# yvette256/nerfstudio-thermal

Hardware: AMD Instinct MI355X
Metric: train rays/sec (4096-ray batch, 96 samples/ray) (higher is better)
Workload: dtype f32; 1 GPU; thermal-nerfacto density_mode=shared train step (pixel sampling+raygen+fwd+losses+bwd+allreduce+Adam), 4096 rays/GPU, 256/96 proposal + 48 field samples, hash 16x2^19x2 + 2x(5x2^17x2), 8 cameras (4 RGB + 4 thermal); rays_per_gpu=4096, parallelism=dp1, grad_scaler=device-side (optim.DeviceGradScaler)

## Files before the change

### nerfstudio-thermal_amd/csrc/tn_common.h

```cpp
#pragma once
#include <hip/hip_runtime.h>
#include <stdint.h>
#include <math.h>
#include "../../include/thermal_nerf_hip.h"

#define TN_WAVE 64

void tn_set_error(const char* fmt, ...);
#define TN_REQUIRE(cond, ...)        \
  do {                               \
    if (!(cond)) {                   \
      tn_set_error(__VA_ARGS__);     \
      return TN_EINVAL;              \
    }                                \
  } while (0)
#define TN_CHECK_LAUNCH(name)                                         \
  do {                                                                \
    hipError_t e__ = hipGetLastError();                               \
    if (e__ != hipSuccess) {                                          \
      tn_set_error("%s: %s", name, hipGetErrorString(e__));           \
      return TN_ELAUNCH;                                              \
    }                                                                 \
  } while (0)

// ... 261 lines not shown
__device__ __forceinline__ float tn_wave_max(float v) {
#pragma unroll
  for (int o = 32; o > 0; o >>= 1) v = fmaxf(v, __shfl_xor(v, o, 64));
  return v;
}
__device__ __forceinline__ double tn_wave_incl_scan_d(double v, int lane) {
#pragma unroll
  for (int o = 1; o < 64; o <<= 1) {
    double t = __shfl_up(v, o, 64);
    if (lane >= o) v += t;
  }
  return v;
}
__device__ __forceinline__ double tn_excl_from_incl_d(double incl, int lane) {
  double t = __shfl_up(incl, 1, 64);
  return lane == 0 ? 0.0 : t;
}
__device__ __forceinline__ float tn_rexcl_from_incl(float incl, int lane) {
  float t = __shfl_down(incl, 1, 64);
  return lane == 63 ? 0.0f : t;
}
__device__ __forceinline__ float tn_wave_incl_rscan(float v, int lane) {
#pragma unroll
  for (int o = 1; o < 64; o <<= 1) {
    float t = __shfl_down(v, o, 64);
    if (lane + o < 64) v += t;
  }
  return v;
}

__device__ __forceinline__ void tn_patch_order(int64_t i, int64_t N, int S, int64_t& ray, int& s) {
  int64_t per = 4 * (int64_t)S;
  int64_t g = tn_div_index(i, per, N * (int64_t)S);
  int w = (int)(i - g * per);
  int64_t r0 = g * 4;
  int nr = (N - r0) < 4 ? (int)(N - r0) : 4;
  s = nr == 4 ? (w >> 2) : w / nr;
  ray = r0 + (w - s * nr);
}

#define TN_SCATTER_SCRATCH_BYTES (64ll << 20)
#ifndef TN_BIN_SLICE_LOG2
#define TN_BIN_SLICE_LOG2 12
#endif
#define TN_BIN_MAX_SLICES 256
#define TN_BIN_COUNT_STRIDE 16
static inline int64_t tn_bin_level_records(int64_t P) { return 16 * P + TN_BIN_MAX_SLICES * 1032; }
static inline int64_t tn_bin_bytes(int64_t P, int num_levels) {
  return 256 + (int64_t)num_levels * TN_BIN_MAX_SLICES * 4 * TN_BIN_COUNT_STRIDE + (int64_t)num_levels * tn_bin_level_records(P) * (2 + 8);
}
static inline int64_t tn_scatter_scratch_bytes(int64_t P, int num_levels) {
  int64_t b = tn_bin_bytes(P, num_levels);
  return ((b > TN_SCATTER_SCRATCH_BYTES ? b : TN_SCATTER_SCRATCH_BYTES) + 255) / 256 * 256;
}
enum { TN_REP_NONE = 0, TN_REP_DENSE = 1 };
struct ReplicaK {
  float2* rep;
  uint32_t total;
  uint32_t kinds;
  uint32_t n[TN_MAX_LEVELS];
  uint32_t off[TN_MAX_LEVELS];
  uint32_t first[TN_MAX_LEVELS];
  uint8_t R[TN_MAX_LEVELS];
};
#define TN_LD_LEVEL_MAJOR (-1)
struct TnNextSamplingHost {
  const TnPropNet *prop0, *prop1;
  const float* pose; const uint8_t* frozen; int num_cameras;
  const float *rays_o, *rays_d; const int64_t* cam;
  const float *nears, *fars, *jit0, *jit1, *jit2, *lin0, *lin1, *lin2;
  float anneal;
  int S0, S1, S2;
  int64_t N;
  float* out;
  int64_t off[16];
  int save_enc;
};
int tn_adam_step_ranges_amp_update_cw(float* params, const float* grads, float* exp_avg, float* exp_avg_sq, int32_t num_ranges, const int64_t* offsets,
                                      const int64_t* counts, const int32_t* steps, const double* lrs, const double* lr_finals,
                                      const int32_t* sched_max_steps, int32_t sched_step, double beta1, double beta2, double eps, const float* inv_scale,
                                      float* found_inf, const int32_t* flag_index, int32_t num_flags, int32_t* skipped, int32_t lag_index,
                                      int32_t count_skip, int32_t zero_grads, float* scale, int32_t* growth_tracker, uint32_t* done_counter,
                                      double growth_factor, double backoff_factor, int32_t growth_interval, const TnSampleRays* next, bool* next_taken,
                                      tn_stream_t stream, const TnNextSamplingHost* chain = nullptr, bool su_update = true);
static inline bool tn_next_sampling_supported(int S0, int S1, int S2) { return S0 > 128 && S0 <= 256 && S1 > 64 && S1 <= 128 && S2 >= 1 && S2 <= 256; }
int tn_render_fwd_ex(const float* e_bins, const float* density, const float* rgb, int64_t N, int32_t S, int32_t C, int32_t training, float* weights,
                     float* comp, float* accumulation, float* depth_median, float* depth_expected, float* scratch, bool launch_clip, int* clip_nblk,
                     tn_stream_t stream);
int tn_train_losses_clip(const float* s_bins_fine, const float* weights_fine, int32_t S_fine, int32_t num_props, const float* const* s_bins_prop,
                         const float* const* weights_prop, const int32_t* S_prop, float* const* d_weights_prop, int64_t N, float distortion_mult,
                         float interlevel_mult, float* d_weights_fine, const float* pred_rgb, int32_t rgb_stride, const float* pred_thermal,
                         int32_t thermal_stride, const float* image, const float* is_thermal, float thermal_mult, float tv_mult, float cross_mult,
                         float* d_pred_rgb, float* d_pred_thermal, float* loss_lines, float* depth_expected, const float* scratch, int clip_nblk,
                         tn_stream_t stream);
struct DposArgs;
struct PoseFinishArgs;
int tn_grid_scatter_launch(const TnGrid& grid, const float* origins, const float* directions, const float* e_bins, const float* g_enc, int ld,
                           int64_t N, int S, float* d_origins, float* d_directions, void* scratch, hipStream_t stream, float* dense_sum = nullptr,
                           bool counters_zeroed = false, const DposArgs* cowork = nullptr, const PoseFinishArgs* fold_cowork = nullptr);
bool tn_grid_scatter_takes_cowork(const TnGrid& grid, int64_t P, void* scratch);
int tn_field_bwd_phase_ex(const TnField* field, const float* origins, const float* directions, const int64_t* camera_indices, const float* e_bins,
                          const float* d_density, const float* d_rgb, int64_t N, int32_t S, void* workspace, int64_t workspace_bytes, float* d_origins,
                          float* d_directions, int32_t phases, int32_t level_begin, int32_t level_end, const PoseFinishArgs* fold_cowork,
                          bool* fold_cowork_taken, tn_stream_t stream);
int tn_pose_finish_args(const float* pose_adjustment, const uint8_t* frozen, const int64_t* camera_indices, const float* directions_in,
                        const float* d_origins, const float* d_directions, int64_t N, int32_t num_cameras, float* grad_pose, const float* loss_lines,
                        float* losses16, float trans_pen, float rot_pen, float scale, float* reg_out, const float* grads, int32_t num_ranges,
                        const int64_t* offsets, const int64_t* counts, const int32_t* flag_index, int32_t num_flags, float* found_inf, int32_t pose_flag,
                        PoseFinishArgs& a);
void tn_grid_scatter_counters(const TnGrid& grid, int64_t P, void* scratch, uint32_t** ptr, int* words);
__device__ __forceinline__ void tn_zero_words(uint32_t* __restrict__ p, int words) {
  if (blockIdx.x == 0 && blockIdx.y == 0)
    for (int i = threadIdx.x; i < words; i += blockDim.x) p[i] = 0u;
}
bool tn_grid_scatter_is_binned(const TnGrid& grid, int64_t P, const void* scratch);
int tn_grid_scatter_bin(const TnGrid& grid, const float* origins, const float* directions, const float* e_bins, const float* g_enc, int ld, int64_t N,
                        int S, float* d_origins, float* d_directions, void* scratch, hipStream_t stream, bool counters_zeroed = false,
                        const DposArgs* cowork = nullptr);
int tn_grid_scatter_fold(const TnGrid& grid, int64_t P, void* scratch, int level_begin, int level_end, hipStream_t stream,
                         const PoseFinishArgs* cowork = nullptr);
int64_t tn_grid_dense_count(const TnGrid& grid, int64_t P);
int tn_grid_dense_fold(const TnGrid& grid, int64_t P, const float* dense_sum, hipStream_t stream);
```

### nerfstudio-thermal_amd/csrc/tn_field.hip

```cpp
#include "tn_common.h"
#include "tn_field_dpos.h"
#include <stdlib.h>

typedef float f32x16 __attribute__((ext_vector_type(16)));
typedef float v4f_t __attribute__((ext_vector_type(4)));
#ifndef FRAG_NT
#define FRAG_NT 1
#endif

#define TILE 32
#define FRAG 64

__host__ __device__ __forceinline__ constexpr int RROW(int r, int h) { return (r & 3) + 8 * (r >> 2) + 4 * h; }

struct LayerGeom { int mo, ti; };
__host__ __device__ __forceinline__ constexpr int layer_mo(int l) { return (l == 0 || l == 2 || l == 3) ? 2 : 1; }
__host__ __device__ __forceinline__ constexpr int layer_ti(int l) { return l == 0 ? 1 : 2; }
__host__ __device__ __forceinline__ constexpr int layer_frags(int l) { return layer_mo(l) * layer_ti(l) * 16; }
__host__ __device__ __forceinline__ constexpr int fwd_off(int l) {
  int o = 0;
  for (int i = 0; i < l; ++i) o += layer_frags(i) * FRAG;
  return o;
}
#define PACK_FWD_FLOATS (fwd_off(5))
// ... 1162 lines not shown
                    int64_t zero_bytes, tn_stream_t stream) {
  if (N == 0) return TN_OK;
  int rc = check_field(field, "tn_field_fwd", false);
  if (rc) return rc;
  TN_REQUIRE(origins && directions && camera_indices && e_bins && workspace && density && rgb, "tn_field_fwd: null pointer");
  TN_REQUIRE(N >= 0 && S >= 1 && S <= TN_MAX_SAMPLES, "tn_field_fwd: bad N=%lld S=%d", (long long)N, S);
  if (N == 0) return TN_OK;
  int64_t P = N * (int64_t)S;
  FieldWs ws = ws_layout(workspace, P, training);
  TN_REQUIRE((2 * ws.PT + P) * 8 < (1ll << 32), "tn_field_fwd: batch too large for the 32-bit lane offsets of the level-major loads");
  TN_REQUIRE(workspace_bytes >= ws.bytes, "tn_field_fwd: workspace of %lld bytes, tn_field_workspace_bytes(%lld, %d) = %lld", (long long)workspace_bytes,
             (long long)P, training, (long long)ws.bytes);
  TN_REQUIRE(zero == nullptr || (((uintptr_t)zero % 16) == 0 && zero_bytes % 16 == 0), "tn_field_fwd: the buffer to clear must be 16-byte aligned and sized");
  TN_REQUIRE(!training || field->num_images <= FIELD_MAX_IMAGES, "tn_field_fwd: %d cameras, the per-camera tables of the training path are sized for %d",
             field->num_images, FIELD_MAX_IMAGES);
  rc = launch_encode(field, origins, directions, e_bins, N, S, ws, stream, FieldPrepExtra{pack_first != 0, zero, zero_bytes});
  if (rc) return rc;
  const size_t shmem = PACK_FWD_TOTAL * sizeof(float);
  const int grid = (int)std::max<int64_t>(1, std::min<int64_t>(tn_cdiv(tn_cdiv(P, TILE), FWD_THREADS / 64), 512));
  const int L = field->grid.num_levels;
#define FWD_LAUNCH(TRAIN_, BF3_, ...)                                                                                                          \
  {                                                                                                                                            \
    (void)hipFuncSetAttribute(reinterpret_cast<const void*>(&k_field_mlp_fwd<TRAIN_, BF3_>), hipFuncAttributeMaxDynamicSharedMemorySize, (int)shmem); \
    hipLaunchKernelGGL((k_field_mlp_fwd<TRAIN_, BF3_>), dim3(grid), dim3(FWD_THREADS), shmem, tn_s(stream), ws.pack, ws.enc, L, ws.PT, ws.sel, ws.sh, \
                       camera_indices, field->emb, field->num_images, TRAIN_ ? 1 : 0, N, S, field->num_channels, density, rgb, density_pre, __VA_ARGS__); \
  }
  const bool bf3 = tn_head_bf16x3();
  if (training) {
    if (bf3) FWD_LAUNCH(true, true, ws.h1, ws.hin, ws.hh1, ws.hh2, ws.y) else FWD_LAUNCH(true, false, ws.h1, ws.hin, ws.hh1, ws.hh2, ws.y)
  } else {
    if (bf3) FWD_LAUNCH(false, true, nullptr, nullptr, nullptr, nullptr, nullptr) else FWD_LAUNCH(false, false, nullptr, nullptr, nullptr, nullptr, nullptr)
  }
#undef FWD_LAUNCH
  TN_CHECK_LAUNCH("tn_field_fwd");
  return TN_OK;
}

extern "C" int tn_field_density_fwd(const TnField* field, const float* origins, const float* directions, const float* e_bins, int64_t N, int32_t S,
                                    int32_t training, void* workspace, int64_t workspace_bytes, float* density, tn_stream_t stream) {
  if (N == 0) return TN_OK;
  int rc = check_field(field, "tn_field_density_fwd", false);
  if (rc) return rc;
  TN_REQUIRE(origins && directions && e_bins && workspace && density, "tn_field_density_fwd: null pointer");
  TN_REQUIRE(N >= 0 && S >= 1 && S <= TN_MAX_SAMPLES, "tn_field_density_fwd: bad N=%lld S=%d", (long long)N, S);
  int64_t P = N * (int64_t)S;
  FieldWs ws = ws_layout(workspace, P, training ? 1 : 0);
  TN_REQUIRE((2 * ws.PT + P) * 8 < (1ll << 32), "tn_field_density_fwd: batch too large for the 32-bit lane offsets of the level-major loads");
  TN_REQUIRE(workspace_bytes >= ws.bytes, "tn_field_density_fwd: workspace of %lld bytes, tn_field_workspace_bytes(%lld, %d) = %lld", (long long)workspace_bytes,
             (long long)P, training ? 1 : 0, (long long)ws.bytes);
  rc = launch_encode(field, origins, directions, e_bins, N, S, ws, stream);
  if (rc) return rc;
  size_t shmem = PACK_FWD_TOTAL * sizeof(float);
  if (training) {
    (void)hipFuncSetAttribute(reinterpret_cast<const void*>(&k_field_density_only<true>), hipFuncAttributeMaxDynamicSharedMemorySize, (int)shmem);
    hipLaunchKernelGGL(k_field_density_only<true>, dim3(mlp_grid(P)), dim3(256), shmem, tn_s(stream), ws.pack, ws.enc, field->grid.num_levels, ws.PT, ws.sel, P, density, ws.h1, ws.hin);
  } else {
    (void)hipFuncSetAttribute(reinterpret_cast<const void*>(&k_field_density_only<false>), hipFuncAttributeMaxDynamicSharedMemorySize, (int)shmem);
    hipLaunchKernelGGL(k_field_density_only<false>, dim3(mlp_grid(P)), dim3(256), shmem, tn_s(stream), ws.pack, ws.enc, field->grid.num_levels, ws.PT, ws.sel, P, density, nullptr, nullptr);
  }
  TN_CHECK_LAUNCH("tn_field_density_fwd");
  return TN_OK;
}

static TnGrid level_range_grid(const TnGrid& g, int level_begin, int level_end) {
  TnGrid sub = g;
  const int64_t T2 = 2ll << g.log2_hashmap_size;
  sub.table = g.table + level_begin * T2;
  sub.table_grad = g.table_grad ? g.table_grad + level_begin * T2 : nullptr;
  sub.num_levels = level_end - level_begin;
  for (int i = 0; i < TN_MAX_LEVELS; ++i) sub.res[i] = (level_begin + i < g.num_levels) ? g.res[level_begin + i] : 0.0f;
  return sub;
}

extern "C" int tn_field_bwd_phase(const TnField* field, const float* origins, const float* directions, const int64_t* camera_indices,
                                  const float* e_bins, const float* d_density, const float* d_rgb, int64_t N, int32_t S, void* workspace,
                                  int64_t workspace_bytes, float* d_origins, float* d_directions, int32_t phases, int32_t level_begin, int32_t level_end,
                                  tn_stream_t stream) {
  return tn_field_bwd_phase_ex(field, origins, directions, camera_indices, e_bins, d_density, d_rgb, N, S, workspace, workspace_bytes, d_origins, d_directions,
                               phases, level_begin, level_end, nullptr, nullptr, stream);
}
int tn_field_bwd_phase_ex(const TnField* field, const float* origins, const float* directions, const int64_t* camera_indices, const float* e_bins,
                          const float* d_density, const float* d_rgb, int64_t N, int32_t S, void* workspace, int64_t workspace_bytes, float* d_origins,
                          float* d_directions, int32_t phases, int32_t level_begin, int32_t level_end, const PoseFinishArgs* fold_cowork,
                          bool* fold_cowork_taken, tn_stream_t stream) {
  if (fold_cowork_taken) *fold_cowork_taken = false;
  if (N == 0) return TN_OK;
  int rc = check_field(field, "tn_field_bwd", true);
  if (rc) return rc;
  TN_REQUIRE(origins && directions && camera_indices && e_bins && d_density && workspace, "tn_field_bwd: null pointer");
  const bool dens_only = d_rgb == nullptr;
  TN_REQUIRE((d_origins == nullptr) == (d_directions == nullptr), "tn_field_bwd: d_origins and d_directions must both be given or both NULL");
  TN_REQUIRE(N >= 0 && S >= 1 && S <= TN_MAX_SAMPLES, "tn_field_bwd: bad N=%lld S=%d", (long long)N, S);
  TN_REQUIRE((phases & ~(TN_BWD_MLP | TN_BWD_SCATTER | TN_BWD_JOIN | TN_BWD_SCATTER_BIN | TN_BWD_SCATTER_FOLD | TN_BWD_FORK_DPOS | TN_BWD_COUNTERS_CLEAN)) == 0 && phases != 0,
             "tn_field_bwd: bad phase set %d", phases);
  TN_REQUIRE(!((phases & TN_BWD_SCATTER) && (phases & (TN_BWD_SCATTER_BIN | TN_BWD_SCATTER_FOLD))), "tn_field_bwd: TN_BWD_SCATTER and its two halves exclude each other");
  if (phases & (TN_BWD_SCATTER | TN_BWD_SCATTER_FOLD))
    TN_REQUIRE(level_begin >= 0 && level_begin < level_end && level_end <= field->grid.num_levels, "tn_field_bwd: bad level range [%d, %d)", level_begin,
               level_end);
  int64_t P = N * (int64_t)S;
  FieldWs ws = ws_layout(workspace, P, 1);
  TN_REQUIRE(workspace_bytes >= ws.bytes, "tn_field_bwd: workspace of %lld bytes, tn_field_workspace_bytes(%lld, 1) = %lld", (long long)workspace_bytes, (long long)P,
             (long long)ws.bytes);
  TN_REQUIRE((2 * ws.PT + P) * 8 < (1ll << 32), "tn_field_bwd: batch too large for the 32-bit lane offsets of the level-major loads");
  hipStream_t st = tn_s(stream);
  const int C = field->num_channels;
  TN_REQUIRE(dens_only || !(phases & TN_BWD_MLP) || field->num_images <= FIELD_MAX_IMAGES,
             "tn_field_bwd: %d cameras, the per-camera sums of the appearance embedding's gradient are sized for %d", field->num_images, FIELD_MAX_IMAGES);
  DposArgs dpos_args{};
  bool dpos_cowork = false;
  if (phases & TN_BWD_MLP) {
    const size_t shmem = FB_LDS_FLOATS * sizeof(float);
    const int grid = (int)std::max<int64_t>(1, std::min<int64_t>(tn_cdiv(tn_cdiv(P, TILE), 4), 256));
    FusedGrads G{field->gw0, field->gb0, field->gw1, field->gb1, field->ghw0, field->ghb0, field->ghw1, field->ghb1, field->ghw2, field->ghb2, field->gemb};
    uint32_t* zp;
    int zw;
    tn_grid_scatter_counters(field->grid, P, ws.scatter, &zp, &zw);
    if (dens_only) {
      (void)hipFuncSetAttribute(reinterpret_cast<const void*>(&k_field_bwd_fused<true, false>), hipFuncAttributeMaxDynamicSharedMemorySize, (int)shmem);
      hipLaunchKernelGGL((k_field_bwd_fused<true, false>), dim3(grid), dim3(256), shmem, st, ws.pack, ws.sel, ws.y, d_rgb, d_density, camera_indices, field->num_images, P, S,
                         C, ws.sh, field->emb, ws.cam_bias, field->grid.num_levels, ws.PT, ws.enc, ws.h1, ws.hin, ws.hh1, ws.hh2, ws.g_enc, G, zp, zw);
    } else if (tn_head_bf16x3()) {
      (void)hipFuncSetAttribute(reinterpret_cast<const void*>(&k_field_bwd_fused<false, true>), hipFuncAttributeMaxDynamicSharedMemorySize, (int)shmem);
      hipLaunchKernelGGL((k_field_bwd_fused<false, true>), dim3(grid), dim3(256), shmem, st, ws.pack, ws.sel, ws.y, d_rgb, d_density, camera_indices, field->num_images, P,
                         S, C, ws.sh, field->emb, ws.cam_bias, field->grid.num_levels, ws.PT, ws.enc, ws.h1, ws.hin, ws.hh1, ws.hh2, ws.g_enc, G, zp, zw);
    } else {
      (void)hipFuncSetAttribute(reinterpret_cast<const void*>(&k_field_bwd_fused<false, false>), hipFuncAttributeMaxDynamicSharedMemorySize, (int)shmem);
      hipLaunchKernelGGL((k_field_bwd_fused<false, false>), dim3(grid), dim3(256), shmem, st, ws.pack, ws.sel, ws.y, d_rgb, d_density, camera_indices, field->num_images, P,
                         S, C, ws.sh, field->emb, ws.cam_bias, field->grid.num_levels, ws.PT, ws.enc, ws.h1, ws.hin, ws.hh1, ws.hh2, ws.g_enc, G, zp, zw);
    }
    if (!dens_only && d_origins == nullptr)
      hipLaunchKernelGGL(k_field_emb_finish, dim3(std::min(field->num_images + 8, 1024)), dim3(256), 0, st, ws.cam_bias,
                         reinterpret_cast<uint32_t*>(ws.cam_bias + (int64_t)FIELD_MAX_IMAGES * 64), field->hw0, field->emb, field->gemb, field->ghw0,
                         field->num_images);
    TN_CHECK_LAUNCH("tn_field_bwd(mlp + weight gradients)");
    if (d_origins != nullptr) {
      dpos_args = DposArgs{origins, directions, e_bins, ws.g_enc, ws.jac, N, S, field->grid.num_levels, ws.PT, d_origins, d_directions,
                           dens_only ? nullptr : ws.cam_bias, reinterpret_cast<uint32_t*>(ws.cam_bias + (int64_t)FIELD_MAX_IMAGES * 64), field->hw0, field->emb,
                           field->gemb, field->ghw0, field->num_images};
      const char* cwe = getenv("TN_DPOS_COWORK");
      dpos_cowork = (phases & TN_BWD_SCATTER) && level_begin == 0 && level_end == field->grid.num_levels && !(cwe && cwe[0] == '0') &&
                    tn_grid_scatter_takes_cowork(field->grid, P, ws.scatter);
      if (!dpos_cowork) {
        hipStream_t side = (phases & TN_BWD_FORK_DPOS) ? tn_fork(st) : nullptr;
        const int64_t tiles = tn_cdiv(P, 32);
        hipLaunchKernelGGL(k_field_dpos, dim3((unsigned)std::min<int64_t>(tn_cdiv(tiles, 4), 256 * 8)), dim3(256), 0, side ? side : st, dpos_args);
      }
      TN_CHECK_LAUNCH("tn_field_bwd(d position)");
    }
  }
  float* sc_do = nullptr;
  float* sc_dd = nullptr;
  if (phases & TN_BWD_SCATTER) {
    TnGrid sub = level_range_grid(field->grid, level_begin, level_end);
    const bool cz = (phases & (TN_BWD_MLP | TN_BWD_COUNTERS_CLEAN)) && level_begin == 0 && level_end == field->grid.num_levels;
    const PoseFinishArgs* fcw = (fold_cowork != nullptr && dpos_cowork) ? fold_cowork : nullptr;
    rc = tn_grid_scatter_launch(sub, origins, directions, e_bins, ws.g_enc + (int64_t)level_begin * 2 * P, TN_LD_LEVEL_MAJOR, N, S, sc_do, sc_dd, ws.scatter, st,
                                nullptr, cz, dpos_cowork ? &dpos_args : nullptr, fcw);
    if (fold_cowork_taken && rc == TN_OK) *fold_cowork_taken = fcw != nullptr;
  }
  if (phases & (TN_BWD_SCATTER_BIN | TN_BWD_SCATTER_FOLD)) {
    TN_REQUIRE(tn_grid_scatter_is_binned(field->grid, P, ws.scatter), "tn_field_bwd: the two-step scatter needs a record-based path (TN_SCATTER_MODE=2 or 1 -- not 0 --, a scatter workspace, table <= 2^20 slots)");
    if (phases & TN_BWD_SCATTER_BIN)
      rc = tn_grid_scatter_bin(field->grid, origins, directions, e_bins, ws.g_enc, TN_LD_LEVEL_MAJOR, N, S, sc_do, sc_dd, ws.scatter, st,
                               (phases & (TN_BWD_MLP | TN_BWD_COUNTERS_CLEAN)) != 0);
    if (rc == TN_OK && (phases & TN_BWD_SCATTER_FOLD)) rc = tn_grid_scatter_fold(field->grid, P, ws.scatter, level_begin, level_end, st);
  }
  if (phases & TN_BWD_JOIN) tn_join_all(st);
  return rc;
}

extern "C" int tn_field_bwd(const TnField* field, const float* origins, const float* directions, const int64_t* camera_indices, const float* e_bins,
                            const float* d_density, const float* d_rgb, int64_t N, int32_t S, void* workspace, int64_t workspace_bytes, float* d_origins,
                            float* d_directions, tn_stream_t stream) {
  if (field == nullptr) return check_field(field, "tn_field_bwd", true);
  return tn_field_bwd_phase(field, origins, directions, camera_indices, e_bins, d_density, d_rgb, N, S, workspace, workspace_bytes, d_origins, d_directions,
                            TN_BWD_MLP | TN_BWD_SCATTER | TN_BWD_JOIN, 0, field->grid.num_levels, stream);
}

extern "C" int64_t tn_field_dense_count(const TnField* field, int64_t num_points, int32_t level_begin, int32_t level_end) {
  if (field == nullptr || level_begin < 0 || level_begin >= level_end || level_end > field->grid.num_levels) return 0;
  return tn_grid_dense_count(level_range_grid(field->grid, level_begin, level_end), num_points);
}

extern "C" int tn_field_bwd_scatter_dense(const TnField* field, const float* origins, const float* directions, const float* e_bins, int64_t N, int32_t S,
                                          void* workspace, int64_t workspace_bytes, float* d_origins, float* d_directions, int32_t level_begin,
                                          int32_t level_end, float* dense_sum, tn_stream_t stream) {
  if (N == 0) return TN_OK;
  int rc = check_field(field, "tn_field_bwd_scatter_dense", true);
  if (rc) return rc;
  TN_REQUIRE(origins && directions && e_bins && workspace && dense_sum, "tn_field_bwd_scatter_dense: null pointer");
  TN_REQUIRE((d_origins == nullptr) == (d_directions == nullptr), "tn_field_bwd_scatter_dense: d_origins and d_directions must both be given or both NULL");
  TN_REQUIRE(N > 0 && S >= 1 && S <= TN_MAX_SAMPLES, "tn_field_bwd_scatter_dense: bad N=%lld S=%d", (long long)N, S);
  TN_REQUIRE(level_begin >= 0 && level_begin < level_end && level_end <= field->grid.num_levels, "tn_field_bwd_scatter_dense: bad level range [%d, %d)",
             level_begin, level_end);
  FieldWs ws = ws_layout(workspace, N * (int64_t)S, 1);
  TN_REQUIRE(workspace_bytes >= ws.bytes, "tn_field_bwd_scatter_dense: workspace of %lld bytes, needs %lld", (long long)workspace_bytes, (long long)ws.bytes);
  return tn_grid_scatter_launch(level_range_grid(field->grid, level_begin, level_end), origins, directions, e_bins,
                                ws.g_enc + (int64_t)level_begin * 2 * N * S, TN_LD_LEVEL_MAJOR, N, S, nullptr, nullptr, ws.scatter, tn_s(stream), dense_sum);
}

extern "C" int tn_field_dense_fold(const TnField* field, int64_t num_points, int32_t level_begin, int32_t level_end, const float* dense_sum,
                                   tn_stream_t stream) {
  int rc = check_field(field, "tn_field_dense_fold", true);
  if (rc) return rc;
  TN_REQUIRE(level_begin >= 0 && level_begin < level_end && level_end <= field->grid.num_levels && num_points > 0, "tn_field_dense_fold: bad arguments");
  return tn_grid_dense_fold(level_range_grid(field->grid, level_begin, level_end), num_points, dense_sum, tn_s(stream));
}
```

### nerfstudio-thermal_amd/csrc/tn_misc.hip

```cpp
#include "tn_common.h"
#include "tn_pose_finish.h"
#include <algorithm>
#include "tn_pixel_loss.h"
#include <stdlib.h>
#include <stdarg.h>
#include <stdio.h>
#include <string.h>

static thread_local char g_err[512] = "";
void tn_set_error(const char* fmt, ...) {
  va_list ap;
  va_start(ap, fmt);
  vsnprintf(g_err, sizeof(g_err), fmt, ap);
  va_end(ap);
}
extern "C" const char* tn_last_error(void) { return g_err; }
#include <map>
#include <mutex>
namespace {
struct Companion {
  hipStream_t side = nullptr;
  hipEvent_t fork_ev = nullptr, join_ev = nullptr;
  bool forked = false;
};
// ... 738 lines not shown
    r.bc2_sqrt[n] = (float)sqrt(bc2);
    max_n4 = std::max<int64_t>(max_n4, counts[k] / 4);
    ++n;
  }
  if (n == 0) return TN_OK;
  int grid = (int)std::max<int64_t>(1, std::min<int64_t>(tn_cdiv(max_n4, 256), 256 * 16));
  hipLaunchKernelGGL(k_adam_ranges, dim3(grid, n), dim3(256), 0, tn_s(stream), params, grads, exp_avg, exp_avg_sq, r, (float)beta1, (float)beta2,
                     (float)(1.0 - beta1), (float)(1.0 - beta2), (float)eps);
  TN_CHECK_LAUNCH("tn_adam_step_ranges");
  return TN_OK;
}

__global__ void __launch_bounds__(256) k_grad_nonfinite(const float4* __restrict__ g, int64_t n4, const float* __restrict__ gt, int tail,
                                                         float* __restrict__ found_inf) {
  typedef float v4f __attribute__((ext_vector_type(4)));
  bool bad = false;
  for (int64_t i = blockIdx.x * (int64_t)blockDim.x + threadIdx.x; i < n4; i += (int64_t)gridDim.x * blockDim.x) {
    const v4f v = reinterpret_cast<const v4f*>(g)[i];
    const float t = (v.x - v.x) + (v.y - v.y) + (v.z - v.z) + (v.w - v.w);
    bad = bad || (t != 0.0f);
  }
  if (blockIdx.x == 0 && (int)threadIdx.x < tail) { const float x = gt[threadIdx.x]; bad = bad || ((x - x) != 0.0f); }
  if (__any(bad) && (threadIdx.x & 63) == 0) *found_inf = 1.0f;
}
extern "C" int tn_grad_nonfinite(const float* grads, int64_t count, float* found_inf, tn_stream_t stream) {
  if (count == 0) return TN_OK;
  TN_REQUIRE(grads && found_inf && count > 0, "tn_grad_nonfinite: bad argument");
  TN_REQUIRE(((uintptr_t)grads % 16) == 0, "tn_grad_nonfinite: grads must be 16-byte aligned");
  const int64_t n4 = count / 4;
  const int grid = (int)std::max<int64_t>(1, std::min<int64_t>(tn_cdiv(n4, 256 * 4), 256 * 8));
  hipLaunchKernelGGL(k_grad_nonfinite, dim3(grid), dim3(256), 0, tn_s(stream), reinterpret_cast<const float4*>(grads), n4, grads + n4 * 4, (int)(count - n4 * 4),
                     found_inf);
  TN_CHECK_LAUNCH("tn_grad_nonfinite");
  return TN_OK;
}
struct NonfiniteRanges { int64_t off[TN_ADAM_MAX_RANGES], cnt[TN_ADAM_MAX_RANGES]; int32_t flag[TN_ADAM_MAX_RANGES]; };
__global__ void __launch_bounds__(256) k_grad_nonfinite_ranges(const float* __restrict__ g, NonfiniteRanges r, float* __restrict__ found_inf) {
  typedef float v4f __attribute__((ext_vector_type(4)));
  const int k = blockIdx.y;
  const int64_t n = r.cnt[k], n4 = n / 4;
  if ((int64_t)blockIdx.x * blockDim.x >= n4 && blockIdx.x != 0) return;
  const float* base = g + r.off[k];
  bool bad = false;
  for (int64_t i = blockIdx.x * (int64_t)blockDim.x + threadIdx.x; i < n4; i += (int64_t)gridDim.x * blockDim.x) {
    const v4f v = reinterpret_cast<const v4f*>(base)[i];
    const float t = (v.x - v.x) + (v.y - v.y) + (v.z - v.z) + (v.w - v.w);
    bad = bad || (t != 0.0f);
  }
  if (blockIdx.x == 0 && (int64_t)threadIdx.x < n - n4 * 4) { const float x = base[n4 * 4 + threadIdx.x]; bad = bad || ((x - x) != 0.0f); }
  if (__any(bad) && (threadIdx.x & 63) == 0) found_inf[r.flag[k]] = 1.0f;
}
extern "C" int tn_grad_nonfinite_ranges(const float* grads, int32_t num_ranges, const int64_t* offsets, const int64_t* counts, const int32_t* flag_index,
                                        int32_t num_flags, float* found_inf, tn_stream_t stream) {
  if (num_ranges == 0) return TN_OK;
  TN_REQUIRE(grads && offsets && counts && found_inf && num_ranges > 0 && num_ranges <= TN_ADAM_MAX_RANGES && num_flags >= 1,
             "tn_grad_nonfinite_ranges: bad argument");
  TN_REQUIRE(((uintptr_t)grads % 16) == 0, "tn_grad_nonfinite_ranges: grads must be 16-byte aligned");
  NonfiniteRanges r{};
  int64_t max_n4 = 0;
  int n = 0;
  for (int k = 0; k < num_ranges; ++k) {
    const int fl = flag_index ? flag_index[k] : 0;
    TN_REQUIRE(offsets[k] >= 0 && offsets[k] % 4 == 0 && counts[k] >= 0 && fl >= 0 && fl < num_flags, "tn_grad_nonfinite_ranges: bad range %d", k);
    if (counts[k] == 0) continue;
    r.off[n] = offsets[k]; r.cnt[n] = counts[k]; r.flag[n] = fl;
    max_n4 = std::max<int64_t>(max_n4, counts[k] / 4);
    ++n;
  }
  if (n == 0) return TN_OK;
  const int grid = (int)std::max<int64_t>(1, std::min<int64_t>(tn_cdiv(max_n4, 256 * 4), 256 * 8));
  hipLaunchKernelGGL(k_grad_nonfinite_ranges, dim3(grid, n), dim3(256), 0, tn_s(stream), grads, r, found_inf);
  TN_CHECK_LAUNCH("tn_grad_nonfinite_ranges");
  return TN_OK;
}

struct AdamRangesAmp {
  int64_t off[TN_ADAM_MAX_RANGES], cnt[TN_ADAM_MAX_RANGES];
  int32_t step[TN_ADAM_MAX_RANGES], flag[TN_ADAM_MAX_RANGES];
  double lr[TN_ADAM_MAX_RANGES];
  double lr_final[TN_ADAM_MAX_RANGES];
  int32_t max_steps[TN_ADAM_MAX_RANGES];
  int32_t sched_step;
  int32_t num_flags, lag_index;
};
struct ScalerUpdate {
  float* scale;
  int32_t* growth_tracker;
  uint32_t* done;
  float growth_factor, backoff_factor;
  int32_t growth_interval;
};
__device__ __forceinline__ void scaler_update_body(float* scale, int32_t* growth_tracker, float* found_inf, int num_flags, int32_t* lag, float growth_factor,
                                                   float backoff_factor, int growth_interval, int clear) {
  bool any = false;
  for (int i = 0; i < num_flags; ++i) {
    any = any || (found_inf[i] != 0.0f);
    if (clear) found_inf[i] = 0.0f;
  }
  if (any) {
    *scale = *scale * backoff_factor;
    *growth_tracker = 0;
    if (lag != nullptr) *lag += 1;
  } else {
    const int successful = *growth_tracker + 1;
    if (successful == growth_interval) {
      const float ns = *scale * growth_factor;
      if ((ns - ns) == 0.0f) *scale = ns;
      *growth_tracker = 0;
    } else {
      *growth_tracker = successful;
    }
  }
}
#define TN_DONE_WORDS (65 * 16)
__device__ __forceinline__ void adam_block_done(const ScalerUpdate& su, float* found_inf, int num_flags, int32_t* skipped, int lag_index) {
  if (su.scale == nullptr) return;
  __syncthreads();
  if (threadIdx.x == 0) {
    const uint32_t total = gridDim.x * gridDim.y, lb = blockIdx.y * gridDim.x + blockIdx.x, line = lb & 63u;
    const uint32_t expect = total / 64u + ((line < (total & 63u)) ? 1u : 0u);
    if (__hip_atomic_fetch_add(su.done + line * 16u, 1u, __ATOMIC_RELAXED, __HIP_MEMORY_SCOPE_AGENT) + 1u == expect) {
      __hip_atomic_store(su.done + line * 16u, 0u, __ATOMIC_RELAXED, __HIP_MEMORY_SCOPE_AGENT);
      const uint32_t lines = total < 64u ? total : 64u;
      if (__hip_atomic_fetch_add(su.done + 64u * 16u, 1u, __ATOMIC_RELAXED, __HIP_MEMORY_SCOPE_AGENT) + 1u == lines) {
        __hip_atomic_store(su.done + 64u * 16u, 0u, __ATOMIC_RELAXED, __HIP_MEMORY_SCOPE_AGENT);
        scaler_update_body(su.scale, su.growth_tracker, found_inf, num_flags, (skipped != nullptr && lag_index >= 0) ? skipped + lag_index : nullptr,
                           su.growth_factor, su.backoff_factor, su.growth_interval, 1);
      }
    }
  }
}
struct SampleCoWork { SamplePixelsArgs a; RaygenArgs g; int blocks; };
#include "tn_next_sampling.h"
__device__ __forceinline__ void adam_range_body(float* __restrict__ p, const float* __restrict__ g, float* __restrict__ m, float* __restrict__ v,
                                                const AdamRangesAmp& r, double beta1, double beta2, float eps, const float* __restrict__ inv_scale,
                                                float* __restrict__ found_inf, int32_t* __restrict__ skipped, int count_skip, int zero_g, int k, int bid,
                                                int nblk) {
  const int fl = r.flag[k];
  float* gz = const_cast<float*>(g);
  const int lag = (skipped != nullptr && r.lag_index >= 0) ? skipped[r.lag_index] : 0;
  const int64_t off = r.off[k], n = r.cnt[k], n4 = n / 4;
  const int64_t stride = (int64_t)nblk * blockDim.x;
  if (found_inf != nullptr && found_inf[fl] != 0.0f) {
    if (count_skip && skipped != nullptr && bid == 0 && threadIdx.x == 0) {
      bool first = true;
      for (int j = 0; j < k; ++j) first = first && r.flag[j] != fl;
      if (first) atomicAdd(&skipped[fl], 1);
    }
    if (zero_g) {
      for (int64_t i = bid * (int64_t)blockDim.x + threadIdx.x; i < n4; i += stride)
        reinterpret_cast<float4*>(gz + off)[i] = make_float4(0.f, 0.f, 0.f, 0.f);
      if (bid == 0 && (int64_t)threadIdx.x < n - n4 * 4) gz[off + n4 * 4 + threadIdx.x] = 0.0f;
    }
    return;
  }
  if ((int64_t)bid * blockDim.x >= n4 && bid != 0) return;
  __shared__ float s_ns, s_bc;
  __syncthreads();
  if (threadIdx.x == 0) {
    const int sk = skipped ? skipped[fl] : 0;
    const int eff = r.step[k] - sk;
    const double bc1 = 1.0 - pow(beta1, (double)(eff < 1 ? 1 : eff)), bc2 = 1.0 - pow(beta2, (double)(eff < 1 ? 1 : eff));
    double lr = r.lr[k];
    if (r.max_steps[k] > 0) {
      double t = (double)(r.sched_step - lag) / (double)r.max_steps[k];
      t = t < 0.0 ? 0.0 : (t > 1.0 ? 1.0 : t);
      lr = exp(log(r.lr[k]) * (1.0 - t) + log(r.lr_final[k]) * t);
    }
    s_ns = (float)(-(lr / bc1));
    s_bc = (float)sqrt(bc2);
  }
  __syncthreads();
  const float neg_step = s_ns, bc2_sqrt = s_bc, b1 = (float)beta1, b2 = (float)beta2, omb1 = (float)(1.0 - beta1), omb2 = (float)(1.0 - beta2);
  const float is = inv_scale ? *inv_scale : 1.0f;
  float4* p4 = reinterpret_cast<float4*>(p + off);
  const float4* g4 = reinterpret_cast<const float4*>(g + off);
  float4* m4 = reinterpret_cast<float4*>(m + off);
  float4* v4 = reinterpret_cast<float4*>(v + off);
#define ADAM1(P, G, M, V)                         \
  {                                               \
    float g_ = inv_scale ? (G) * is : (G);        \
    float m_new_ = M * b1 + g_ * omb1;            \
    float v_new_ = V * b2 + (omb2 * g_) * g_;     \
    float den_ = sqrtf(v_new_) / bc2_sqrt + eps;  \
    P = P + neg_step * (m_new_ / den_);           \
    M = m_new_;                                   \
    V = v_new_;                                   \
  }
  typedef float v4f __attribute__((ext_vector_type(4)));
  typedef uint32_t v4u __attribute__((ext_vector_type(4)));
#define ADAM4(I, GG, MM, VV)                                                                                           \
  {                                                                                                                    \
    const v4u zb = __builtin_bit_cast(v4u, GG) | __builtin_bit_cast(v4u, MM) | __builtin_bit_cast(v4u, VV);          \
    if ((zb.x | zb.y | zb.z | zb.w) != 0u) {                                                                           \
      float4 pp = p4[I];                                                                                               \
      ADAM1(pp.x, GG.x, MM.x, VV.x)                                                                                    \
      ADAM1(pp.y, GG.y, MM.y, VV.y)                                                                                    \
      ADAM1(pp.z, GG.z, MM.z, VV.z)                                                                                    \
      ADAM1(pp.w, GG.w, MM.w, VV.w)                                                                                    \
      p4[I] = pp;                                                                                                      \
      __builtin_nontemporal_store(MM, reinterpret_cast<v4f*>(m4) + (I));                                               \
      __builtin_nontemporal_store(VV, reinterpret_cast<v4f*>(v4) + (I));                                               \
      if (zero_g) { const v4f z = {0.f, 0.f, 0.f, 0.f}; __builtin_nontemporal_store(z, reinterpret_cast<v4f*>(gz + off) + (I)); } \
    }                                                                                                                  \
  }
  int64_t i0 = bid * (int64_t)blockDim.x + threadIdx.x;
  for (; i0 < n4; i0 += stride) {
    v4f gg = __builtin_nontemporal_load(reinterpret_cast<const v4f*>(g4) + i0);
    v4f mm4 = __builtin_nontemporal_load(reinterpret_cast<const v4f*>(m4) + i0);
    v4f vv4 = __builtin_nontemporal_load(reinterpret_cast<const v4f*>(v4) + i0);
    ADAM4(i0, gg, mm4, vv4)
  }
#undef ADAM4
  const int tail = (int)(n - n4 * 4);
  if (bid == 0 && (int)threadIdx.x < tail) {
    const int64_t i = off + n4 * 4 + threadIdx.x;
    float pp = p[i], gg = g[i], mm = m[i], vv = v[i];
    ADAM1(pp, gg, mm, vv)
    p[i] = pp; m[i] = mm; v[i] = vv;
    if (zero_g) gz[i] = 0.0f;
  }
#undef ADAM1
}
__global__ void k_adam_ranges_amp(float* __restrict__ p, const float* __restrict__ g, float* __restrict__ m, float* __restrict__ v, AdamRangesAmp r,
                                  double beta1, double beta2, float eps, const float* __restrict__ inv_scale, float* __restrict__ found_inf,
                                  int32_t* __restrict__ skipped, int count_skip, int zero_g, ScalerUpdate su, SampleCoWork cw) {
  int k = blockIdx.y;
  if (cw.blocks > 0) {
    if (k == 0) {
      if (blockIdx.x < (unsigned)cw.blocks) sample_rays_body(cw.a, cw.g, blockIdx.x, (unsigned)cw.blocks);
      adam_block_done(su, found_inf, r.num_flags, skipped, r.lag_index);
      return;
    }
    --k;
  }
  adam_range_body(p, g, m, v, r, beta1, beta2, eps, inv_scale, found_inf, skipped, count_skip, zero_g, k, (int)blockIdx.x, (int)gridDim.x);
  adam_block_done(su, found_inf, r.num_flags, skipped, r.lag_index);
}
template <bool FUSED>
__global__ void __launch_bounds__(256, 4) k_adam_ranges_amp_next(float* __restrict__ p, const float* __restrict__ g, float* __restrict__ m, float* __restrict__ v,
                                                                 AdamRangesAmp r, double beta1, double beta2, float eps, const float* __restrict__ inv_scale,
                                                                 float* __restrict__ found_inf, int32_t* __restrict__ skipped, int count_skip, int zero_g,
                                                                 ScalerUpdate su, NextSamplingArgs ns, FusedAdam fa) {
  __shared__ __attribute__((aligned(16))) float ns_lds[NS_LDS_FLOATS];
  __shared__ __attribute__((aligned(16))) float fa_stage[FUSED ? 4 * FA_STAGE_FLOATS : 4];
  __shared__ float fa_scal[4];
  if (blockIdx.y == 0) {
    if (blockIdx.x < (unsigned)ns.blocks) next_sampling_body<FUSED>(ns, blockIdx.x, (unsigned)ns.blocks, ns_lds, &fa, fa_stage, fa_scal);
  } else {
    adam_range_body(p, g, m, v, r, beta1, beta2, eps, inv_scale, found_inf, skipped, count_skip, zero_g, (int)blockIdx.y - 1, (int)blockIdx.x, (int)gridDim.x);
  }
  adam_block_done(su, found_inf, r.num_flags, skipped, r.lag_index);
}
__global__ void __launch_bounds__(256, 4) k_next_sampling(NextSamplingArgs ns) {
  __shared__ __attribute__((aligned(16))) float ns_lds[NS_LDS_FLOATS];
  next_sampling_body(ns, blockIdx.x, gridDim.x, ns_lds);
}
static int adam_ranges_amp_impl(float* params, const float* grads, float* exp_avg, float* exp_avg_sq, int32_t num_ranges, const int64_t* offsets,
                               const int64_t* counts, const int32_t* steps, const double* lrs, const double* lr_finals,
                               const int32_t* sched_max_steps, int32_t sched_step, double beta1, double beta2, double eps,
                               const float* inv_scale, const float* found_inf, const int32_t* flag_index, int32_t num_flags, int32_t* skipped,
                               int32_t lag_index, int32_t count_skip, int32_t zero_grads, ScalerUpdate su, tn_stream_t stream,
                               const TnSampleRays* next = nullptr, bool* next_taken = nullptr, const TnNextSamplingHost* chain = nullptr) {
  if (next_taken) *next_taken = false;
  if (num_ranges == 0) return TN_OK;
  TN_REQUIRE(params && grads && exp_avg && exp_avg_sq && offsets && counts && steps && lrs, "tn_adam_step_ranges_amp: null pointer");
  TN_REQUIRE(num_ranges > 0 && num_ranges <= TN_ADAM_MAX_RANGES, "tn_adam_step_ranges_amp: %d ranges (at most %d)", num_ranges, TN_ADAM_MAX_RANGES);
  TN_REQUIRE(((uintptr_t)params % 16 == 0) && ((uintptr_t)grads % 16 == 0) && ((uintptr_t)exp_avg % 16 == 0) && ((uintptr_t)exp_avg_sq % 16 == 0),
             "tn_adam_step_ranges_amp: arena pointers must be 16-byte aligned");
  TN_REQUIRE(num_flags >= 1 && num_flags <= 64 && lag_index >= -1 && lag_index <= 64, "tn_adam_step_ranges_amp: bad num_flags / lag_index");
  AdamRangesAmp r{};
  int64_t max_n4 = 0;
  int n = 0;
  for (int k = 0; k < num_ranges; ++k) {
    TN_REQUIRE(offsets[k] >= 0 && offsets[k] % 4 == 0 && counts[k] >= 0 && steps[k] >= 1, "tn_adam_step_ranges_amp: bad range %d (offset %lld count %lld step %d)",
               k, (long long)offsets[k], (long long)counts[k], steps[k]);
    const int fl = flag_index ? flag_index[k] : 0;
    TN_REQUIRE(fl >= 0 && fl < num_flags, "tn_adam_step_ranges_amp: flag index %d of range %d outside [0, %d)", fl, k, num_flags);
    if (counts[k] == 0) continue;
    r.off[n] = offsets[k]; r.cnt[n] = counts[k]; r.step[n] = steps[k]; r.lr[n] = lrs[k]; r.flag[n] = fl;
    r.lr_final[n] = lr_finals ? lr_finals[k] : lrs[k];
    r.max_steps[n] = (lr_finals && sched_max_steps) ? sched_max_steps[k] : 0;
    max_n4 = std::max<int64_t>(max_n4, counts[k] / 4);
    ++n;
  }
  if (n == 0) return TN_OK;
  r.sched_step = sched_step;
  r.num_flags = num_flags;
  r.lag_index = lag_index;
  int grid = (int)std::max<int64_t>(1, std::min<int64_t>(tn_cdiv(max_n4, 256), 256 * 16));
  SampleCoWork cw{};
  if (next != nullptr && next->num_rays > 0) {
    int rc = sample_rays_build("tn_train_step(next_sample)", next, cw.a, cw.g);
    if (rc) return rc;
    grid = std::max(grid, (int)std::min<int64_t>(tn_cdiv(next->num_rays * 4, 256), 256));
    cw.blocks = (int)std::min<int64_t>(tn_cdiv(next->num_rays * 4, 256), grid);
    if (next_taken) *next_taken = true;
  }
  if (chain != nullptr) {
    TN_REQUIRE(next == nullptr, "tn_train_step(next_sampling): the launch that carries the chain does not sample the batch");
    TN_REQUIRE(chain->N > 0 && chain->N % 4 == 0 && chain->N < (1ll << 30), "tn_train_step(next_sampling): %lld rays (a multiple of 4 is needed)", (long long)chain->N);
    TN_REQUIRE(tn_next_sampling_supported(chain->S0, chain->S1, chain->S2), "tn_train_step(next_sampling): unsupported sample counts (%d, %d, %d)", chain->S0,
               chain->S1, chain->S2);
    TN_REQUIRE(chain->prop0 && chain->prop1 && chain->pose && chain->nears && chain->fars && chain->lin0 && chain->lin1 && chain->lin2 && chain->out &&
                   chain->rays_o && chain->rays_d && chain->cam && chain->num_cameras >= 1,
               "tn_train_step(next_sampling): null pointer");
    TN_REQUIRE(chain->prop0->grid.num_levels == PL && chain->prop1->grid.num_levels == PL && chain->prop0->grid.log2_hashmap_size >= 1 &&
                   chain->prop0->grid.log2_hashmap_size <= 24 && chain->prop1->grid.log2_hashmap_size >= 1 && chain->prop1->grid.log2_hashmap_size <= 24,
               "tn_train_step(next_sampling): proposal grids are built for %d levels", PL);
    NextSamplingArgs ns{};
    auto prop = [](const TnPropNet* q) {
      NsProp o{};
      o.table = reinterpret_cast<const float2*>(q->grid.table);
      o.tsize = 1u << q->grid.log2_hashmap_size; o.mask = o.tsize - 1u;
      for (int l = 0; l < PL; ++l) o.res[l] = q->grid.res[l];
      o.w0 = q->w0; o.b0 = q->b0; o.w1 = q->w1; o.b1 = q->b1;
      return o;
    };
    TN_REQUIRE(chain->prop0->grid.table && chain->prop0->w0 && chain->prop0->b0 && chain->prop0->w1 && chain->prop0->b1 && chain->prop1->grid.table &&
                   chain->prop1->w0 && chain->prop1->b0 && chain->prop1->w1 && chain->prop1->b1, "tn_train_step(next_sampling): null parameter pointer");
    ns.p0 = prop(chain->prop0); ns.p1 = prop(chain->prop1);
    ns.pose = chain->pose; ns.frozen = chain->frozen; ns.num_cameras = chain->num_cameras;
    ns.rays_o = chain->rays_o; ns.rays_d = chain->rays_d; ns.cam = chain->cam;
    ns.nears = chain->nears; ns.fars = chain->fars;
    ns.jit0 = chain->jit0; ns.jit1 = chain->jit1; ns.jit2 = chain->jit2;
    ns.lin0 = chain->lin0; ns.lin1 = chain->lin1; ns.lin2 = chain->lin2;
    ns.anneal = chain->anneal;
    ns.S0 = chain->S0; ns.S1 = chain->S1; ns.S2 = chain->S2; ns.N = (int)chain->N;
    ns.out = chain->out;
    for (int k = 0; k < NS_SLOTS; ++k) {
      TN_REQUIRE(chain->off[k] >= 0 && chain->off[k] < (1ll << 32), "tn_train_step(next_sampling): forward buffer region %d out of range", k);
      ns.off[k] = (uint32_t)chain->off[k];
    }
    ns.save_enc = chain->save_enc;
    grid = std::max(grid, (int)std::min<int64_t>(chain->N / 4, 1024));
    ns.blocks = (int)std::min<int64_t>(chain->N / 4, grid);
    const char* mode = getenv("TN_NEXT_SAMPLING");
    if (mode && mode[0] == '3') {
      hipStream_t side = tn_fork_n(tn_s(stream), 3);
      hipLaunchKernelGGL(k_next_sampling, dim3(ns.blocks), dim3(256), 0, side ? side : tn_s(stream), ns);
      TN_CHECK_LAUNCH("tn_next_sampling");
      SampleCoWork none{};
      hipLaunchKernelGGL(k_adam_ranges_amp, dim3(grid, n), dim3(256), 0, tn_s(stream), params, grads, exp_avg, exp_avg_sq, r, beta1, beta2, (float)eps, inv_scale,
                         const_cast<float*>(found_inf), skipped, (int)count_skip, (int)zero_grads, su, none);
      TN_CHECK_LAUNCH("tn_adam_step_ranges_amp");
      return TN_OK;
    }
    if (mode && mode[0] == '2') {
      SampleCoWork none{};
      hipLaunchKernelGGL(k_adam_ranges_amp, dim3(grid, n), dim3(256), 0, tn_s(stream), params, grads, exp_avg, exp_avg_sq, r, beta1, beta2, (float)eps, inv_scale,
                         const_cast<float*>(found_inf), skipped, (int)count_skip, (int)zero_grads, su, none);
      TN_CHECK_LAUNCH("tn_adam_step_ranges_amp");
      hipLaunchKernelGGL(k_next_sampling, dim3(ns.blocks), dim3(256), 0, tn_s(stream), ns);
      TN_CHECK_LAUNCH("tn_next_sampling");
      return TN_OK;
    }
    FusedAdam fa{};
    if (mode && mode[0] == '4' && n == 1 && inv_scale == nullptr) {
      const int64_t nb = r.cnt[0] / 256, W = (int64_t)ns.blocks * 4, trips = tn_cdiv(chain->N, W);
      const char* fs = getenv("TN_FUSED_SITES");
      const int64_t per_ray = fs ? std::max(1, atoi(fs)) : FA_SITES_PER_RAY;
      const int64_t take = std::min<int64_t>(nb - 1, per_ray * trips * W);
      if (take >= W) {
        fa.p = params + r.off[0]; fa.g = grads + r.off[0]; fa.m = exp_avg + r.off[0]; fa.v = exp_avg_sq + r.off[0];
        fa.batches = (uint32_t)take;
        fa.flag = r.flag[0]; fa.step = r.step[0]; fa.max_steps = r.max_steps[0]; fa.sched_step = r.sched_step; fa.lag_index = r.lag_index;
        fa.zero_g = (int)zero_grads;
        fa.beta1 = beta1; fa.beta2 = beta2; fa.lr = r.lr[0]; fa.lr_final = r.lr_final[0]; fa.eps = (float)eps;
        fa.found_inf = found_inf; fa.skipped = skipped;
        r.off[0] += take * 256; r.cnt[0] -= take * 256;
      }
    }
    if (fa.batches > 0)
      hipLaunchKernelGGL(k_adam_ranges_amp_next<true>, dim3(grid, n + 1), dim3(256), 0, tn_s(stream), params, grads, exp_avg, exp_avg_sq, r, beta1, beta2, (float)eps,
                         inv_scale, const_cast<float*>(found_inf), skipped, (int)count_skip, (int)zero_grads, su, ns, fa);
    else
      hipLaunchKernelGGL(k_adam_ranges_amp_next<false>, dim3(grid, n + 1), dim3(256), 0, tn_s(stream), params, grads, exp_avg, exp_avg_sq, r, beta1, beta2, (float)eps,
                         inv_scale, const_cast<float*>(found_inf), skipped, (int)count_skip, (int)zero_grads, su, ns, fa);
    TN_CHECK_LAUNCH("tn_adam_step_ranges_amp(next_sampling)");
    return TN_OK;
  }
  hipLaunchKernelGGL(k_adam_ranges_amp, dim3(grid, n + (cw.blocks > 0 ? 1 : 0)), dim3(256), 0, tn_s(stream), params, grads, exp_avg, exp_avg_sq, r, beta1, beta2,
                     (float)eps, inv_scale, const_cast<float*>(found_inf), skipped, (int)count_skip, (int)zero_grads, su, cw);
  TN_CHECK_LAUNCH("tn_adam_step_ranges_amp");
  return TN_OK;
}
extern "C" int tn_adam_step_ranges_amp(float* params, const float* grads, float* exp_avg, float* exp_avg_sq, int32_t num_ranges, const int64_t* offsets,
                                       const int64_t* counts, const int32_t* steps, const double* lrs, const double* lr_finals,
                                       const int32_t* sched_max_steps, int32_t sched_step, double beta1, double beta2, double eps,
                                       const float* inv_scale, const float* found_inf, const int32_t* flag_index, int32_t num_flags, int32_t* skipped,
                                       int32_t lag_index, int32_t count_skip, int32_t zero_grads, tn_stream_t stream) {
  return adam_ranges_amp_impl(params, grads, exp_avg, exp_avg_sq, num_ranges, offsets, counts, steps, lrs, lr_finals, sched_max_steps, sched_step, beta1, beta2,
                              eps, inv_scale, found_inf, flag_index, num_flags, skipped, lag_index, count_skip, zero_grads, ScalerUpdate{}, stream);
}
extern "C" int tn_adam_step_ranges_amp_update(float* params, const float* grads, float* exp_avg, float* exp_avg_sq, int32_t num_ranges, const int64_t* offsets,
                                              const int64_t* counts, const int32_t* steps, const double* lrs, const double* lr_finals,
                                              const int32_t* sched_max_steps, int32_t sched_step, double beta1, double beta2, double eps,
                                              const float* inv_scale, float* found_inf, const int32_t* flag_index, int32_t num_flags, int32_t* skipped,
                                              int32_t lag_index, int32_t count_skip, int32_t zero_grads, float* scale, int32_t* growth_tracker,
                                              uint32_t* done_counter, double growth_factor, double backoff_factor, int32_t growth_interval,
                                              tn_stream_t stream) {
  TN_REQUIRE(found_inf && scale && growth_tracker && done_counter && growth_interval >= 1, "tn_adam_step_ranges_amp_update: bad scaler arguments");
  TN_REQUIRE(num_ranges > 0, "tn_adam_step_ranges_amp_update: the fused scale update needs at least one range (use tn_grad_scaler_update otherwise)");
  ScalerUpdate su{scale, growth_tracker, done_counter, (float)growth_factor, (float)backoff_factor, (int32_t)growth_interval};
  return adam_ranges_amp_impl(params, grads, exp_avg, exp_avg_sq, num_ranges, offsets, counts, steps, lrs, lr_finals, sched_max_steps, sched_step, beta1, beta2,
                              eps, inv_scale, found_inf, flag_index, num_flags, skipped, lag_index, count_skip, zero_grads, su, stream);
}

int tn_adam_step_ranges_amp_update_cw(float* params, const float* grads, float* exp_avg, float* exp_avg_sq, int32_t num_ranges, const int64_t* offsets,
                                      const int64_t* counts, const int32_t* steps, const double* lrs, const double* lr_finals,
                                      const int32_t* sched_max_steps, int32_t sched_step, double beta1, double beta2, double eps, const float* inv_scale,
                                      float* found_inf, const int32_t* flag_index, int32_t num_flags, int32_t* skipped, int32_t lag_index,
                                      int32_t count_skip, int32_t zero_grads, float* scale, int32_t* growth_tracker, uint32_t* done_counter,
                                      double growth_factor, double backoff_factor, int32_t growth_interval, const TnSampleRays* next, bool* next_taken,
                                      tn_stream_t stream, const TnNextSamplingHost* chain, bool su_update) {
  TN_REQUIRE(found_inf && scale && growth_tracker && done_counter && growth_interval >= 1, "tn_adam_step_ranges_amp_update: bad scaler arguments");
  TN_REQUIRE(num_ranges > 0, "tn_adam_step_ranges_amp_update: the fused scale update needs at least one range (use tn_grad_scaler_update otherwise)");
  ScalerUpdate su{scale, growth_tracker, done_counter, (float)growth_factor, (float)backoff_factor, (int32_t)growth_interval};
  return adam_ranges_amp_impl(params, grads, exp_avg, exp_avg_sq, num_ranges, offsets, counts, steps, lrs, lr_finals, sched_max_steps, sched_step, beta1, beta2,
                              eps, inv_scale, found_inf, flag_index, num_flags, skipped, lag_index, count_skip, zero_grads, su_update ? su : ScalerUpdate{}, stream,
                              next, next_taken, chain);
}

__global__ void k_grad_scaler_update(float* scale, int32_t* growth_tracker, float* found_inf, int num_flags, int32_t* lag, float growth_factor,
                                     float backoff_factor, int growth_interval, int clear) {
  scaler_update_body(scale, growth_tracker, found_inf, num_flags, lag, growth_factor, backoff_factor, growth_interval, clear);
}
extern "C" int tn_grad_scaler_update(float* scale, int32_t* growth_tracker, float* found_inf, int32_t num_flags, int32_t* lag,
                                     double growth_factor, double backoff_factor, int32_t growth_interval, int32_t clear_found_inf, tn_stream_t stream) {
  TN_REQUIRE(scale && growth_tracker && found_inf && num_flags >= 1 && growth_interval >= 1, "tn_grad_scaler_update: bad argument");
  hipLaunchKernelGGL(k_grad_scaler_update, dim3(1), dim3(1), 0, tn_s(stream), scale, growth_tracker, found_inf, (int)num_flags, lag, (float)growth_factor,
                     (float)backoff_factor, (int)growth_interval, (int)clear_found_inf);
  TN_CHECK_LAUNCH("tn_grad_scaler_update");
  return TN_OK;
}
```

### nerfstudio-thermal_amd/csrc/tn_pipeline.hip

```cpp
#include "tn_common.h"
#include "tn_pose_finish.h"

namespace {
struct EvalWs {
  float *s0, *e0, *d0, *w0, *s1, *e1, *d1, *w1, *s2, *e2, *w2, *rgb_s, *scratch;
  void* field_ws;
  int64_t bytes;
};
EvalWs eval_layout(void* base, int64_t N, int S0, int S1, int S2, int C) {
  EvalWs w;
  char* p = reinterpret_cast<char*>(base);
  int64_t off = 0;
  auto take = [&](int64_t floats) {
    float* r = reinterpret_cast<float*>(p + off);
    off += ((floats * 4 + 255) / 256) * 256;
    return r;
  };
  w.s0 = take(N * (S0 + 1)); w.e0 = take(N * (S0 + 1)); w.d0 = take(N * S0); w.w0 = take(N * S0);
  w.s1 = take(N * (S1 + 1)); w.e1 = take(N * (S1 + 1)); w.d1 = take(N * S1); w.w1 = take(N * S1);
  w.s2 = take(N * (S2 + 1)); w.e2 = take(N * (S2 + 1)); w.w2 = take(N * S2);
  w.rgb_s = take(N * (int64_t)S2 * C);
  w.scratch = take(TN_RENDER_SCRATCH_FLOATS);
  w.field_ws = p + off;
  off += tn_field_workspace_bytes(N * (int64_t)S2, 0);
  w.bytes = off;
  return w;
}
}

extern "C" int64_t tn_render_rays_eval_workspace_bytes(int64_t num_rays, int32_t S0, int32_t S1, int32_t S2, int32_t C) {
  if (num_rays < 0 || S0 < 1 || S1 < 1 || S2 < 1 || S0 > TN_MAX_SAMPLES || S1 > TN_MAX_SAMPLES || S2 > TN_MAX_SAMPLES || C < 1 || C > 4) return TN_EINVAL;
  return eval_layout(nullptr, num_rays, S0, S1, S2, C).bytes;
}

extern "C" int tn_render_rays_eval(const TnPropNet* prop0, const TnPropNet* prop1, const TnField* field, const float* origins,
                                   const float* directions, const int64_t* camera_indices, const float* nears, const float* fars, int64_t N,
                                   int32_t S0, int32_t S1, int32_t S2, float anneal, const float* lin_spaced0, const float* lin_pdf1,
                                   const float* lin_pdf2, void* workspace, int64_t workspace_bytes, float* rgb, float* accumulation, float* depth_median,
                                   float* depth_expected, float* prop_depth0, float* prop_depth1, float* density, float* e_bins_out,
                                   float* rgb_samples_out, tn_stream_t stream) {
  if (N == 0) return TN_OK;
  TN_REQUIRE(prop0 && prop1 && field && origins && directions && camera_indices && nears && fars && lin_spaced0 && lin_pdf1 && lin_pdf2 &&
                 workspace && rgb && density,
             "tn_render_rays_eval: null pointer");
  TN_REQUIRE(N > 0 && S0 >= 1 && S1 >= 1 && S2 >= 1 && S0 <= TN_MAX_SAMPLES && S1 <= TN_MAX_SAMPLES && S2 <= TN_MAX_SAMPLES,
             "tn_render_rays_eval: bad N=%lld S=(%d, %d, %d)", (long long)N, S0, S1, S2);
  TN_REQUIRE(((uintptr_t)workspace % 256) == 0, "tn_render_rays_eval: workspace must be 256-byte aligned");
  const int C = field->num_channels;
  EvalWs w = eval_layout(workspace, N, S0, S1, S2, C);
  TN_REQUIRE(workspace_bytes >= w.bytes, "tn_render_rays_eval: workspace of %lld bytes, tn_render_rays_eval_workspace_bytes = %lld", (long long)workspace_bytes,
             (long long)w.bytes);
  const int64_t field_ws_bytes = tn_field_workspace_bytes(N * (int64_t)S2, 0);
  float* e2 = e_bins_out ? e_bins_out : w.e2;
  float* rgb_s = rgb_samples_out ? rgb_samples_out : w.rgb_s;
  int rc;
  if ((rc = tn_spaced_bins(lin_spaced0, nullptr, nears, fars, N, S0, w.s0, w.e0, stream))) return rc;
  if ((rc = tn_prop_density_fwd(prop0, origins, directions, w.e0, N, S0, w.d0, stream))) return rc;
  if ((rc = tn_weights_resample(w.e0, w.d0, w.s0, S0, anneal, lin_pdf1, nullptr, nears, fars, N, S1, w.w0, prop_depth0, w.s1, w.e1, stream))) return rc;
  if ((rc = tn_prop_density_fwd(prop1, origins, directions, w.e1, N, S1, w.d1, stream))) return rc;
  if ((rc = tn_weights_resample(w.e1, w.d1, w.s1, S1, anneal, lin_pdf2, nullptr, nears, fars, N, S2, w.w1, prop_depth1, w.s2, e2, stream))) return rc;
  if ((rc = tn_field_fwd_ex(field, origins, directions, camera_indices, e2, N, S2, 0, w.field_ws, field_ws_bytes, density, rgb_s, nullptr, 1, nullptr, 0, stream)))
    return rc;
  return tn_render_fwd(e2, density, rgb_s, N, S2, C, 0, w.w2, rgb, accumulation, depth_median, depth_expected, w.scratch, stream);
}

enum {
  TRO_ORIGINS = 0, TRO_DIRECTIONS,
  TRO_S0, TRO_E0, TRO_D0, TRO_W0, TRO_M0,
  TRO_S1, TRO_E1, TRO_D1, TRO_W1, TRO_M1,
  TRO_S2, TRO_E2, TRO_D2, TRO_W2,
  TRO_RGB_SAMPLES, TRO_COMP, TRO_ACC, TRO_DEPTH, TRO_EXPECTED, TRO_SCRATCH,
  TRO_PENC0, TRO_PENC1,
  TRO_END,
  TRO_COUNT
};
static void train_layout(int64_t N, int S0, int S1, int S2, int C, int64_t* off) {
  int64_t o = 0;
  auto take = [&](int slot, int64_t floats) { off[slot] = o; o += (floats + 63) / 64 * 64; };
  take(TRO_ORIGINS, N * 3); take(TRO_DIRECTIONS, N * 3);
  take(TRO_S0, N * (S0 + 1)); take(TRO_E0, N * (S0 + 1)); take(TRO_D0, N * S0); take(TRO_W0, N * S0); take(TRO_M0, N);
  take(TRO_S1, N * (S1 + 1)); take(TRO_E1, N * (S1 + 1)); take(TRO_D1, N * S1); take(TRO_W1, N * S1); take(TRO_M1, N);
  take(TRO_S2, N * (S2 + 1)); take(TRO_E2, N * (S2 + 1)); take(TRO_D2, N * S2); take(TRO_W2, N * S2);
  take(TRO_RGB_SAMPLES, N * (int64_t)S2 * C); take(TRO_COMP, N * C); take(TRO_ACC, N); take(TRO_DEPTH, N); take(TRO_EXPECTED, N);
  take(TRO_SCRATCH, TN_RENDER_SCRATCH_FLOATS);
// ... 10 lines not shown
}

static int render_rays_train_impl(const TnPropNet* prop0, const TnPropNet* prop1, const TnField* field, const float* pose_adjustment,
                                  const uint8_t* frozen, int32_t num_cameras, const float* origins_in, const float* directions_in,
                                  const int64_t* camera_indices, const float* nears, const float* fars, int64_t N, int32_t S0, int32_t S1,
                                  int32_t S2, float anneal, const float* jitter0, const float* jitter1, const float* jitter2,
                                  const float* lin_spaced0, const float* lin_pdf1, const float* lin_pdf2, void* field_workspace,
                                  int64_t field_workspace_bytes, float* out, void* wait_event_before_field, void* zero_fill, int64_t zero_fill_bytes,
                                  int32_t save_prop_enc, int with_render, int* clip_nblk, tn_stream_t stream, bool sampling_done = false) {
  if (clip_nblk) *clip_nblk = 0;
  if (N == 0) return TN_OK;
  TN_REQUIRE(prop0 && prop1 && field && origins_in && directions_in && camera_indices && nears && fars && lin_spaced0 && lin_pdf1 && lin_pdf2 &&
                 field_workspace && out,
             "tn_render_rays_train: null pointer");
  TN_REQUIRE(N > 0 && S0 >= 1 && S1 >= 1 && S2 >= 1 && S0 <= TN_MAX_SAMPLES && S1 <= TN_MAX_SAMPLES && S2 <= TN_MAX_SAMPLES,
             "tn_render_rays_train: bad N=%lld S=(%d, %d, %d)", (long long)N, S0, S1, S2);
  TN_REQUIRE(((uintptr_t)out % 256) == 0, "tn_render_rays_train: the output buffer must be 256-byte aligned");
  const int C = field->num_channels;
  int64_t off[TRO_COUNT];
  train_layout(N, S0, S1, S2, C, off);
  auto at = [&](int slot) { return out + off[slot]; };
  const float* o = origins_in;
  const float* d = directions_in;
  int rc;
  if (sampling_done) {
    if (pose_adjustment != nullptr) { o = at(TRO_ORIGINS); d = at(TRO_DIRECTIONS); }
  } else {
    if (pose_adjustment != nullptr) {
      TN_REQUIRE(num_cameras >= 1, "tn_render_rays_train: bad num_cameras=%d", num_cameras);
      if ((rc = tn_pose_spaced_bins(pose_adjustment, frozen, camera_indices, origins_in, directions_in, N, num_cameras, at(TRO_ORIGINS), at(TRO_DIRECTIONS),
                                    lin_spaced0, jitter0, nears, fars, S0, at(TRO_S0), at(TRO_E0), stream)))
        return rc;
      o = at(TRO_ORIGINS);
      d = at(TRO_DIRECTIONS);
    } else if ((rc = tn_spaced_bins(lin_spaced0, jitter0, nears, fars, N, S0, at(TRO_S0), at(TRO_E0), stream))) {
      return rc;
    }
    if ((rc = tn_prop_density_fwd_ex(prop0, o, d, at(TRO_E0), N, S0, at(TRO_D0), save_prop_enc ? at(TRO_PENC0) : nullptr, stream))) return rc;
    if ((rc = tn_weights_resample(at(TRO_E0), at(TRO_D0), at(TRO_S0), S0, anneal, lin_pdf1, jitter1, nears, fars, N, S1, at(TRO_W0), at(TRO_M0), at(TRO_S1),
                                  at(TRO_E1), stream)))
      return rc;
    if ((rc = tn_prop_density_fwd_ex(prop1, o, d, at(TRO_E1), N, S1, at(TRO_D1), save_prop_enc ? at(TRO_PENC1) : nullptr, stream))) return rc;
    if ((rc = tn_weights_resample(at(TRO_E1), at(TRO_D1), at(TRO_S1), S1, anneal, lin_pdf2, jitter2, nears, fars, N, S2, at(TRO_W1), at(TRO_M1), at(TRO_S2),
                                  at(TRO_E2), stream)))
      return rc;
  }
  if (wait_event_before_field != nullptr) {
    hipError_t e = hipStreamWaitEvent(tn_s(stream), reinterpret_cast<hipEvent_t>(wait_event_before_field), 0);
    TN_REQUIRE(e == hipSuccess, "tn_render_rays_train: hipStreamWaitEvent failed: %s", hipGetErrorString(e));
  }
  if ((rc = tn_field_fwd_ex(field, o, d, camera_indices, at(TRO_E2), N, S2, 1, field_workspace, field_workspace_bytes, at(TRO_D2), at(TRO_RGB_SAMPLES), nullptr, 1,
                            zero_fill, zero_fill_bytes, stream)))
    return rc;
  if (!with_render) return TN_OK;
  return tn_render_fwd_ex(at(TRO_E2), at(TRO_D2), at(TRO_RGB_SAMPLES), N, S2, C, 1, at(TRO_W2), at(TRO_COMP), at(TRO_ACC), at(TRO_DEPTH), at(TRO_EXPECTED),
                          at(TRO_SCRATCH), with_render == 1, clip_nblk, stream);
}
extern "C" int tn_render_rays_train(const TnPropNet* prop0, const TnPropNet* prop1, const TnField* field, const float* pose_adjustment,
                                    const uint8_t* frozen, int32_t num_cameras, const float* origins_in, const float* directions_in,
                                    const int64_t* camera_indices, const float* nears, const float* fars, int64_t N, int32_t S0, int32_t S1,
                                    int32_t S2, float anneal, const float* jitter0, const float* jitter1, const float* jitter2,
                                    const float* lin_spaced0, const float* lin_pdf1, const float* lin_pdf2, void* field_workspace,
                                    int64_t field_workspace_bytes, float* out, void* wait_event_before_field, void* zero_fill, int64_t zero_fill_bytes,
                                    int32_t save_prop_enc, tn_stream_t stream) {
  return render_rays_train_impl(prop0, prop1, field, pose_adjustment, frozen, num_cameras, origins_in, directions_in, camera_indices, nears, fars, N, S0, S1, S2,
                                anneal, jitter0, jitter1, jitter2, lin_spaced0, lin_pdf1, lin_pdf2, field_workspace, field_workspace_bytes, out,
                                wait_event_before_field, zero_fill, zero_fill_bytes, save_prop_enc, 1, nullptr, stream);
}

__global__ void k_add_inplace(float* __restrict__ a, const float* __restrict__ b, int64_t n) {
  for (int64_t i = blockIdx.x * (int64_t)blockDim.x + threadIdx.x; i < n; i += (int64_t)gridDim.x * blockDim.x) a[i] += b[i];
}
extern "C" int64_t tn_render_rays_train_bwd_tmp_floats(int64_t N, int32_t S0, int32_t S1, int32_t S2, int32_t C) {
  if (N < 0 || S0 < 1 || S1 < 1 || S2 < 1 || C < 1 || C > 4) return TN_EINVAL;
  auto up = [](int64_t x) { return (x + 63) / 64 * 64; };
  return up(N * (int64_t)S2 * C) + up(N * (int64_t)S2) + up(N * (int64_t)S0) + up(N * (int64_t)S1);
}
static int render_rays_train_bwd_impl(const TnPropNet* prop0, const TnPropNet* prop1, const TnField* field, const float* origins,
                                      const float* directions, const int64_t* camera_indices, int64_t N, int32_t S0, int32_t S1, int32_t S2,
                                      const float* fwd_out, const float* d_comp, const float* d_weights0,
                                      const float* d_weights1, const float* d_weights2, const float* d_density_extra, void* field_workspace,
                                      int64_t field_workspace_bytes, void* prop_workspace0, int64_t prop_workspace_bytes0, void* prop_workspace1,
                                      int64_t prop_workspace_bytes1, float* tmp, float* d_origins, float* d_directions, int32_t prop_enc_saved,
                                      bool render_bwd_done, const PoseFinishArgs* fold_cowork, bool* fold_cowork_taken, tn_stream_t stream) {
  if (fold_cowork_taken) *fold_cowork_taken = false;
  if (N == 0) return TN_OK;
  TN_REQUIRE(field && origins && directions && camera_indices && fwd_out && d_comp && d_weights2 && field_workspace && tmp,
             "tn_render_rays_train_bwd: null pointer");
  TN_REQUIRE((d_weights0 == nullptr) == (d_weights1 == nullptr), "tn_render_rays_train_bwd: d_weights0 and d_weights1 come together (or not at all)");
  const bool prop_grad = d_weights0 != nullptr;
  if (prop_grad) TN_REQUIRE(prop0 && prop1 && prop_workspace0 && prop_workspace1, "tn_render_rays_train_bwd: proposal networks / workspaces missing");
  TN_REQUIRE(N > 0 && S0 >= 1 && S1 >= 1 && S2 >= 1 && S0 <= TN_MAX_SAMPLES && S1 <= TN_MAX_SAMPLES && S2 <= TN_MAX_SAMPLES,
             "tn_render_rays_train_bwd: bad N=%lld S=(%d, %d, %d)", (long long)N, S0, S1, S2);
  TN_REQUIRE((d_origins == nullptr) == (d_directions == nullptr), "tn_render_rays_train_bwd: d_origins and d_directions must both be given or both NULL");
  const int C = field->num_channels;
  int64_t off[TRO_COUNT];
  train_layout(N, S0, S1, S2, C, off);
  auto at = [&](int slot) { return fwd_out + off[slot]; };
  auto up = [](int64_t x) { return (x + 63) / 64 * 64; };
  float* d_rgb = tmp;
  float* d_dens = d_rgb + up(N * (int64_t)S2 * C);
  float* dd0 = d_dens + up(N * (int64_t)S2);
  float* dd1 = dd0 + up(N * (int64_t)S0);
  const float* o = origins;
  const float* d = directions;
  hipStream_t st = tn_s(stream);
  int rc;
  if (!render_bwd_done && (rc = tn_render_bwd(at(TRO_E2), at(TRO_D2), at(TRO_RGB_SAMPLES), at(TRO_W2), d_comp, d_weights2, N, S2, C, d_rgb, d_dens, stream)))
    return rc;
  if (d_density_extra != nullptr) {
    const int64_t n = N * (int64_t)S2;
    hipLaunchKernelGGL(k_add_inplace, dim3((unsigned)std::min<int64_t>(tn_cdiv(n, 256), 4096)), dim3(256), 0, st, d_dens, d_density_extra, n);
    TN_CHECK_LAUNCH("tn_render_rays_train_bwd(add)");
  }
  int rc0 = TN_OK, rc1 = TN_OK;
  if (prop_grad) {
    hipStream_t s0 = tn_fork_n(st, 1), s1 = tn_fork_n(st, 2);
    tn_stream_t t0 = s0 ? (tn_stream_t)s0 : stream, t1 = s1 ? (tn_stream_t)s1 : stream;
    rc0 = tn_weights_bwd(at(TRO_E0), at(TRO_D0), at(TRO_W0), d_weights0, N, S0, dd0, t0);
    if (!rc0)
      rc0 = tn_prop_density_bwd_ex(prop0, o, d, at(TRO_E0), dd0, N, S0, prop_workspace0, prop_workspace_bytes0, d_origins, d_directions,
                                   prop_enc_saved ? at(TRO_PENC0) : nullptr, t0);
    rc1 = tn_weights_bwd(at(TRO_E1), at(TRO_D1), at(TRO_W1), d_weights1, N, S1, dd1, t1);
    if (!rc1)
      rc1 = tn_prop_density_bwd_ex(prop1, o, d, at(TRO_E1), dd1, N, S1, prop_workspace1, prop_workspace_bytes1, d_origins, d_directions,
                                   prop_enc_saved ? at(TRO_PENC1) : nullptr, t1);
  }
  rc = tn_field_bwd_phase_ex(field, o, d, camera_indices, at(TRO_E2), d_dens, d_rgb, N, S2, field_workspace, field_workspace_bytes, d_origins, d_directions,
                             TN_BWD_MLP | TN_BWD_SCATTER | TN_BWD_JOIN | (prop_grad ? TN_BWD_FORK_DPOS : 0), 0, field->grid.num_levels,
                             prop_grad ? nullptr : fold_cowork, fold_cowork_taken, stream);
  if (prop_grad) { tn_join_n(st, 1); tn_join_n(st, 2); }
  return rc ? rc : (rc0 ? rc0 : rc1);
}
extern "C" int tn_render_rays_train_bwd(const TnPropNet* prop0, const TnPropNet* prop1, const TnField* field, const float* origins,
                                        const float* directions, const int64_t* camera_indices, int64_t N, int32_t S0, int32_t S1, int32_t S2,
                                        const float* fwd_out, const float* d_comp, const float* d_weights0,
                                        const float* d_weights1, const float* d_weights2, const float* d_density_extra, void* field_workspace,
                                        int64_t field_workspace_bytes, void* prop_workspace0, int64_t prop_workspace_bytes0, void* prop_workspace1,
                                        int64_t prop_workspace_bytes1, float* tmp, float* d_origins, float* d_directions, int32_t prop_enc_saved,
                                        tn_stream_t stream) {
  return render_rays_train_bwd_impl(prop0, prop1, field, origins, directions, camera_indices, N, S0, S1, S2, fwd_out, d_comp, d_weights0, d_weights1, d_weights2,
                                    d_density_extra, field_workspace, field_workspace_bytes, prop_workspace0, prop_workspace_bytes0, prop_workspace1,
                                    prop_workspace_bytes1, tmp, d_origins, d_directions, prop_enc_saved, false, nullptr, nullptr, stream);
}


extern "C" int tn_train_step(const TnTrainStep* a, tn_stream_t stream) {
  TN_REQUIRE(a != nullptr, "tn_train_step: null argument block");
  tn_join_n(tn_s(stream), 3);
  if (a->next_sample_taken) *a->next_sample_taken = 0;
  if (a->N == 0) return TN_OK;
  TN_REQUIRE(a->prop0 && a->prop1 && a->field && a->origins_in && a->directions_in && a->camera_indices && a->image && a->is_thermal && a->nears &&
                 a->fars && a->fwd_out && a->bwd_tmp && a->acc && a->losses16 && a->loss_lines && a->d_comp && a->d_weights2,
             "tn_train_step: null pointer");
  TN_REQUIRE(a->pose_adjustment && a->grad_pose && a->d_origins && a->d_directions && a->num_cameras >= 1,
             "tn_train_step: this entry point is the iteration WITH a camera optimiser (pose_adjustment, grad_pose, d_origins, d_directions)");
  TN_REQUIRE(a->prop_grad == 0 || (a->d_weights0 && a->d_weights1 && a->prop_workspace0 && a->prop_workspace1),
             "tn_train_step: prop_grad needs d_weights0 / d_weights1 and both proposal workspaces");
  TN_REQUIRE(a->num_check >= 0 && a->num_check <= TN_TRAIN_STEP_MAX_RANGES && a->num_ranges >= 0 && a->num_ranges <= TN_TRAIN_STEP_MAX_RANGES,
             "tn_train_step: at most %d ranges", TN_TRAIN_STEP_MAX_RANGES);
  TN_REQUIRE(a->found_inf && a->num_flags >= 1 && a->scale && a->growth_tracker && a->done_counter && a->skipped,
             "tn_train_step: the GradScaler state is part of the iteration (found_inf, scale, growth_tracker, done_counter, skipped)");
  TN_REQUIRE(a->num_ranges == 0 || (a->params && a->grads && a->exp_avg && a->exp_avg_sq), "tn_train_step: null arena pointer");
  const int C = a->field->num_channels;
  TN_REQUIRE(C == 4, "tn_train_step: the shared-density model renders RGB + thermal from one field (4 channels), got %d", C);
  TN_REQUIRE(a->N > 0 && a->S0 >= 1 && a->S1 >= 1 && a->S2 >= 1 && a->S0 <= TN_MAX_SAMPLES && a->S1 <= TN_MAX_SAMPLES && a->S2 <= TN_MAX_SAMPLES,
             "tn_train_step: bad N=%lld S=(%d, %d, %d)", (long long)a->N, a->S0, a->S1, a->S2);
  TN_REQUIRE(((uintptr_t)a->fwd_out % 256) == 0, "tn_train_step: the forward's buffer must be 256-byte aligned");
  TN_REQUIRE(((uintptr_t)a->acc % 16) == 0 && a->acc_bytes >= 0 && a->acc_bytes % 16 == 0, "tn_train_step: the accumulator block must be 16-byte aligned and sized");
  TN_REQUIRE(a->lin_spaced0 && a->lin_pdf1 && a->lin_pdf2 && a->field_workspace, "tn_train_step: null sampler table / field workspace");
  {
    const int64_t need_f = tn_field_workspace_bytes(a->N * (int64_t)a->S2, 1);
    TN_REQUIRE(a->field_workspace_bytes >= need_f, "tn_train_step: field workspace of %lld bytes, tn_field_workspace_bytes(%lld, 1) = %lld",
               (long long)a->field_workspace_bytes, (long long)(a->N * (int64_t)a->S2), (long long)need_f);
    if (a->prop_grad) {
      const int64_t need0 = tn_prop_workspace_bytes(a->N * (int64_t)a->S0), need1 = tn_prop_workspace_bytes(a->N * (int64_t)a->S1);
      TN_REQUIRE(a->prop_workspace_bytes0 >= need0 && a->prop_workspace_bytes1 >= need1,
                 "tn_train_step: proposal workspaces of %lld / %lld bytes, tn_prop_workspace_bytes = %lld / %lld", (long long)a->prop_workspace_bytes0,
                 (long long)a->prop_workspace_bytes1, (long long)need0, (long long)need1);
    }
  }
  if (a->next_sampling_taken) *a->next_sampling_taken = 0;
  if (a->next_sample != nullptr && a->num_ranges > 0) {
    const TnSampleRays* s = a->next_sample;
    TN_REQUIRE(s->num_rays >= 0 && s->num_images >= 1 && s->patch_size >= 1 && s->patch_size <= 8, "tn_train_step(next_sample): bad num_rays=%lld num_images=%d patch_size=%d",
               (long long)s->num_rays, s->num_images, s->patch_size);
    if (s->num_rays > 0) {
      const int64_t pp = (int64_t)s->patch_size * s->patch_size, per = ((s->num_rays / s->num_images) / pp) * pp, last = s->num_rays - (int64_t)(s->num_images - 1) * per;
      TN_REQUIRE(last > 0 && last % pp == 0, "tn_train_step(next_sample): %lld rays over %d images do not split into whole patches", (long long)s->num_rays, s->num_images);
      TN_REQUIRE(s->images && s->image_offsets && s->heights && s->widths && s->is_thermal && s->image_idx && s->u && s->ray_indices && s->image &&
                     s->is_thermal_out && s->c2w && s->fx && s->fy && s->cx && s->cy && s->origins && s->directions && s->num_cameras >= 1,
                 "tn_train_step(next_sample): null pointer / bad camera arguments");
    }
  }
  if (a->next_sampling != nullptr) TN_REQUIRE(a->next_sampling->fwd_out != nullptr && ((uintptr_t)a->next_sampling->fwd_out % 256) == 0,
                                              "tn_train_step(next_sampling): the next forward buffer must be given and 256-byte aligned");
  int64_t off[TRO_COUNT];
  train_layout(a->N, a->S0, a->S1, a->S2, C, off);
  int rc;
  const char* fr = getenv("TN_FUSE_RENDER");
  const bool fuse_render = fr && fr[0] == '1' && a->N % 4 == 0;
  int clip_nblk = 0;
  if ((rc = render_rays_train_impl(a->prop0, a->prop1, a->field, a->pose_adjustment, a->frozen, a->num_cameras, a->origins_in, a->directions_in,
                                   a->camera_indices, a->nears, a->fars, a->N, a->S0, a->S1, a->S2, a->anneal, a->jitter0, a->jitter1, a->jitter2,
                                   a->lin_spaced0, a->lin_pdf1, a->lin_pdf2, a->field_workspace, a->field_workspace_bytes, a->fwd_out, nullptr, a->acc,
                                   a->acc_bytes, a->prop_grad ? 1 : 0, fuse_render ? 0 : 2, &clip_nblk, stream, a->sampling_done != 0)))
    return rc;
  float* out = a->fwd_out;
  const float* sprop[2] = {out + off[TRO_S0], out + off[TRO_S1]};
  const float* wprop[2] = {out + off[TRO_W0], out + off[TRO_W1]};
  const int32_t Sprop[2] = {a->S0, a->S1};
  float* dwprop[2] = {a->prop_grad ? a->d_weights0 : nullptr, a->prop_grad ? a->d_weights1 : nullptr};
  const float* comp = out + off[TRO_COMP];
  if (fuse_render) {
    float* d_rgb = a->bwd_tmp;
    float* d_dens = d_rgb + (a->N * (int64_t)a->S2 * C + 63) / 64 * 64;
    if ((rc = tn_render_losses_bwd(out + off[TRO_E2], out + off[TRO_D2], out + off[TRO_RGB_SAMPLES], a->N, a->S2, C, out + off[TRO_W2], out + off[TRO_COMP],
                                   out + off[TRO_ACC], out + off[TRO_DEPTH], out + off[TRO_EXPECTED], out + off[TRO_SCRATCH], out + off[TRO_S2], 2, sprop, wprop,
                                   Sprop, dwprop, a->distortion_mult, a->interlevel_mult, a->d_weights2, a->image, a->is_thermal, a->thermal_mult, a->tv_mult,
                                   a->cross_mult, a->d_comp, a->loss_lines, d_rgb, d_dens, 1, stream)))
      return rc;
  } else if ((rc = tn_train_losses_clip(out + off[TRO_S2], out + off[TRO_W2], a->S2, 2, sprop, wprop, Sprop, dwprop, a->N, a->distortion_mult,
                                        a->interlevel_mult, a->d_weights2, comp, C, comp + 3, C, a->image, a->is_thermal, a->thermal_mult, a->tv_mult,
                                        a->cross_mult, a->d_comp, a->d_comp + 3, a->loss_lines, out + off[TRO_EXPECTED], out + off[TRO_SCRATCH], clip_nblk,
                                        stream))) {
    return rc;
  }
  PoseFinishArgs pf;
  bool pf_taken = false;
  const char* pfe = getenv("TN_POSE_FINISH_COWORK");
  const bool pf_cowork = !a->prop_grad && !(pfe && pfe[0] == '0');
  if (pf_cowork &&
      (rc = tn_pose_finish_args(a->pose_adjustment, a->frozen, a->camera_indices, a->directions_in, a->d_origins, a->d_directions, a->N, a->num_cameras,
                                a->grad_pose, a->loss_lines, a->losses16, a->trans_pen, a->rot_pen, a->pen_scale, a->losses16 + 11, a->grads, a->num_check,
                                a->check_offsets, a->check_counts, a->check_flags, a->num_flags, a->found_inf, a->pose_flag, pf)))
    return rc;
  if ((rc = render_rays_train_bwd_impl(a->prop_grad ? a->prop0 : nullptr, a->prop_grad ? a->prop1 : nullptr, a->field, out + off[TRO_ORIGINS],
                                       out + off[TRO_DIRECTIONS], a->camera_indices, a->N, a->S0, a->S1, a->S2, out, a->d_comp,
                                       a->prop_grad ? a->d_weights0 : nullptr, a->prop_grad ? a->d_weights1 : nullptr, a->d_weights2, nullptr,
                                       a->field_workspace, a->field_workspace_bytes, a->prop_grad ? a->prop_workspace0 : nullptr,
                                       a->prop_grad ? a->prop_workspace_bytes0 : 0, a->prop_grad ? a->prop_workspace1 : nullptr,
                                       a->prop_grad ? a->prop_workspace_bytes1 : 0, a->bwd_tmp, a->d_origins, a->d_directions, a->prop_grad ? 1 : 0,
                                       fuse_render, pf_cowork ? &pf : nullptr, &pf_taken, stream)))
    return rc;
  if (!pf_taken) {
    if ((rc = tn_pose_bwd_finish_check(a->pose_adjustment, a->frozen, a->camera_indices, a->directions_in, a->d_origins, a->d_directions, a->N,
                                       a->num_cameras, a->grad_pose, a->loss_lines, a->losses16, a->trans_pen, a->rot_pen, a->pen_scale, a->losses16 + 11,
                                       a->grads, a->num_check, a->check_offsets, a->check_counts, a->check_flags, a->num_flags, a->found_inf, a->pose_flag,
                                       stream)))
      return rc;
  }
  if (a->num_ranges == 0) return TN_OK;
  bool taken = false;
  const TnNextSampling* nx = a->next_sampling;
  const char* nse = getenv("TN_NEXT_SAMPLING");
  bool chain = nx != nullptr && a->next_sample != nullptr && a->next_sample->num_rays == a->N && a->next_sample->camera_indices != nullptr && a->N % 4 == 0 &&
               tn_next_sampling_supported(a->S0, a->S1, a->S2) && !(nse && nse[0] == '0');
  int first[TN_TRAIN_STEP_MAX_RANGES], nfirst = 0, rest[TN_TRAIN_STEP_MAX_RANGES], nrest = 0;
  if (chain) {
    const float* reads[] = {a->prop0->grid.table, a->prop0->w0, a->prop0->b0, a->prop0->w1, a->prop0->b1, a->prop1->grid.table, a->prop1->w0,
                            a->prop1->b0, a->prop1->w1, a->prop1->b1, a->pose_adjustment};
    for (int k = 0; k < a->num_ranges; ++k) {
      const float *lo = a->params + a->offsets[k], *hi = lo + a->counts[k];
      bool hit = false;
      for (const float* q : reads) hit = hit || (q >= lo && q < hi);
      if (hit) first[nfirst++] = k; else if (a->counts[k] > 0) rest[nrest++] = k;
    }
    chain = nrest > 0 && nfirst > 0;
  }
  if (!chain) {
    rc = tn_adam_step_ranges_amp_update_cw(a->params, a->grads, a->exp_avg, a->exp_avg_sq, a->num_ranges, a->offsets, a->counts, a->steps, a->lrs, a->lr_finals,
                                           a->sched_max_steps, a->sched_step, a->beta1, a->beta2, a->eps, nullptr, a->found_inf, a->flag_index, a->num_flags,
                                           a->skipped, a->lag_index, 1, 1, a->scale, a->growth_tracker, a->done_counter, a->growth_factor, a->backoff_factor,
                                           a->growth_interval, a->next_sample, &taken, stream);
  } else {
    auto sub = [&](const int* idx, int n, int64_t* o, int64_t* c, int32_t* s, double* l, double* lf, int32_t* ms, int32_t* fl) {
      for (int i = 0; i < n; ++i) {
        const int k = idx[i];
        o[i] = a->offsets[k]; c[i] = a->counts[k]; s[i] = a->steps[k]; l[i] = a->lrs[k]; lf[i] = a->lr_finals[k]; ms[i] = a->sched_max_steps[k]; fl[i] = a->flag_index[k];
      }
    };
    int64_t o[TN_TRAIN_STEP_MAX_RANGES], c[TN_TRAIN_STEP_MAX_RANGES];
    int32_t s[TN_TRAIN_STEP_MAX_RANGES], ms[TN_TRAIN_STEP_MAX_RANGES], fl[TN_TRAIN_STEP_MAX_RANGES];
    double l[TN_TRAIN_STEP_MAX_RANGES], lf[TN_TRAIN_STEP_MAX_RANGES];
    rc = TN_OK;
    sub(first, nfirst, o, c, s, l, lf, ms, fl);
    rc = tn_adam_step_ranges_amp_update_cw(a->params, a->grads, a->exp_avg, a->exp_avg_sq, nfirst, o, c, s, l, lf, ms, a->sched_step, a->beta1, a->beta2, a->eps,
                                           nullptr, a->found_inf, fl, a->num_flags, a->skipped, a->lag_index, 1, 1, a->scale, a->growth_tracker, a->done_counter,
                                           a->growth_factor, a->backoff_factor, a->growth_interval, a->next_sample, &taken, stream, nullptr, false);
    if (!rc && !taken) rc = tn_sample_rays_args(a->next_sample, stream);
    if (!rc) {
      taken = true;
      TnNextSamplingHost h{};
      h.prop0 = a->prop0; h.prop1 = a->prop1; h.pose = a->pose_adjustment; h.frozen = a->frozen; h.num_cameras = a->num_cameras;
      h.rays_o = a->next_sample->origins; h.rays_d = a->next_sample->directions; h.cam = a->next_sample->camera_indices;
      h.nears = a->nears; h.fars = a->fars; h.jit0 = nx->jitter0; h.jit1 = nx->jitter1; h.jit2 = nx->jitter2;
      h.lin0 = a->lin_spaced0; h.lin1 = a->lin_pdf1; h.lin2 = a->lin_pdf2; h.anneal = nx->anneal;
      h.S0 = a->S0; h.S1 = a->S1; h.S2 = a->S2; h.N = a->N;
      h.out = nx->fwd_out;
      const int slots[16] = {TRO_ORIGINS, TRO_DIRECTIONS, TRO_S0, TRO_E0, TRO_D0, TRO_W0, TRO_M0, TRO_S1, TRO_E1, TRO_D1, TRO_W1, TRO_M1, TRO_S2, TRO_E2, TRO_PENC0,
                             TRO_PENC1};
      for (int k = 0; k < 16; ++k) h.off[k] = off[slots[k]];
      h.save_enc = nx->prop_grad ? 1 : 0;
      sub(rest, nrest, o, c, s, l, lf, ms, fl);
      rc = tn_adam_step_ranges_amp_update_cw(a->params, a->grads, a->exp_avg, a->exp_avg_sq, nrest, o, c, s, l, lf, ms, a->sched_step, a->beta1, a->beta2, a->eps,
                                             nullptr, a->found_inf, fl, a->num_flags, a->skipped, a->lag_index, 1, 1, a->scale, a->growth_tracker, a->done_counter,
                                             a->growth_factor, a->backoff_factor, a->growth_interval, nullptr, nullptr, stream, &h, true);
      if (!rc && a->next_sampling_taken) *a->next_sampling_taken = 1;
    }
  }
  if (a->next_sample_taken) *a->next_sample_taken = taken ? 1 : 0;
  return rc;
}
```

### nerfstudio-thermal_amd/csrc/tn_scatter.hip

```cpp
#include "tn_common.h"
#include "tn_field_dpos.h"
#include "tn_pose_finish.h"
#include <stdlib.h>
#include <stdio.h>
#include <vector>
#include <algorithm>

__device__ __forceinline__ float seg_sum4(float v, int start, int lane) {
  int sl = lane >> 2;
#pragma unroll
  for (int o = 1; o < 16; o <<= 1) {
    float t = __shfl_up(v, 4 * o, 64);
    if (sl - o >= start) v += t;
  }
  return v;
}

__global__ void __launch_bounds__(256) k_grid_scatter(GridK g, const float* __restrict__ origins, const float* __restrict__ directions,
                                                      const float* __restrict__ e_bins, const float* __restrict__ g_enc, int ld, int64_t N, int S,
                                                      float* __restrict__ d_origins, float* __restrict__ d_directions, int level_groups, ReplicaK rk) {
  const bool want_dpos = d_origins != nullptr;
  const int lane = tn_lane();
  const int q = lane & 3, xc = q >> 1, ft = q & 1;
  const int64_t P = N * (int64_t)S;
  const int64_t stride = (int64_t)gridDim.x * (blockDim.x >> 2);
  const int64_t iters = tn_cdiv(P, stride);
  for (int64_t it = 0; it < iters; ++it) {
    int64_t i = it * stride + (int64_t)blockIdx.x * (blockDim.x >> 2) + (threadIdx.x >> 2);
    const bool live = i < P;
    if (!live) i = P - 1;
    int64_t ray;
    int s;
    tn_patch_order(i, N, S, ray, s);
    const int64_t p = ray * S + s;
    const float* o = origins + ray * 3;
    const float* d = directions + ray * 3;
    const float* eb = e_bins + ray * (S + 1) + s;
    const float st = eb[0], en = eb[1];
    const Contracted c = tn_contract(o[0], o[1], o[2], d[0], d[1], d[2], st, en);
    float dpx = 0.f, dpy = 0.f, dpz = 0.f;
    float gvs[TN_MAX_LEVELS];
#pragma unroll
    for (int li = 0; li < TN_MAX_LEVELS; ++li) {
      int l = blockIdx.y + li * level_groups;
      gvs[li] = (live && l < g.L) ? g_enc[ld > 0 ? p * ld + 2 * l + ft : (int64_t)l * 2 * P + 2 * p + ft] : 0.0f;
    }
    if (want_dpos) {
#pragma unroll 1
      for (int li = 0; li < TN_MAX_LEVELS; ++li) {
        int l = blockIdx.y + li * level_groups;
        if (l >= g.L) break;
        float gv = gvs[li];
        const float res = g.res[l];
        const uint32_t level_off = (uint32_t)l * g.tsize;
        float sx = c.px * res, sy = c.py * res, sz = c.pz * res;
        float fxf = floorf(sx), fyf = floorf(sy), fzf = floorf(sz);
        uint32_t fx = (uint32_t)(int)fxf, fy = (uint32_t)(int)fyf, fz = (uint32_t)(int)fzf;
        uint32_t cx = (uint32_t)(int)ceilf(sx), cy = (uint32_t)(int)ceilf(sy), cz = (uint32_t)(int)ceilf(sz);
        float ox = sx - fxf, oy = sy - fyf, oz = sz - fzf;
        float ux = 1.0f - ox, uy = 1.0f - oy, uz = 1.0f - oz;
        uint32_t xi = xc ? cx : fx;
        float wxv = xc ? ox : ux;
        uint32_t hcy = cy * TN_PRIME_Y, hfy = fy * TN_PRIME_Y, hcz = cz * TN_PRIME_Z, hfz = fz * TN_PRIME_Z;
        const uint32_t hy[4] = {hcy, hfy, hcy, hfy};
        const uint32_t hz[4] = {hcz, hcz, hfz, hfz};
        const float wy[4] = {oy, uy, oy, uy};
        const float wz[4] = {oz, oz, uz, uz};
        float a = 0.f, b = 0.f, cc = 0.f;
#pragma unroll
        for (int k = 0; k < 4; ++k) {
          uint32_t idx = ((xi ^ hy[k] ^ hz[k]) & g.mask) + level_off;
          float2 t = g.table[idx];
          float tv = ft ? t.y : t.x;
          a += wy[k] * wz[k] * tv;
          b += ((k & 1) ? -1.0f : 1.0f) * wz[k] * tv;
          cc += wy[k] * ((k & 2) ? -1.0f : 1.0f) * tv;
        }
        dpx += (xc ? 1.0f : -1.0f) * a * gv * res;
        dpy += wxv * b * gv * res;
        dpz += wxv * cc * gv * res;
      }
    }
#pragma unroll 1
    for (int li = 0; li < TN_MAX_LEVELS; ++li) {
      int l = blockIdx.y + li * level_groups;
// ... 461 lines not shown
  const bool store = g.grad_zero && raw_count <= bk.cap;
  const uint32_t begin = ch * chunk;
  if (begin >= count) return;
  if (bk.trace && threadIdx.x == 0) bk.trace[16 * blk] = wall_clock64();
  const uint32_t end = min(count, begin + chunk);
  const bool split = count > chunk;
  const int tid = threadIdx.x, lane = tid & 63, wave = tid >> 6;
  const uint32_t slots = 1u << bk.slice_log2;
  const size_t base = (size_t)l * bk.level_stride + (size_t)sl * bk.cap;
  const uint16_t* ip = bk.idx + base;
  const float2* vp = bk.val + base;
  const uint32_t mine = wave * 512 + 2 * lane;
  double* ax = reinterpret_cast<double*>(s_mem);
  double* ay = ax + slots;
#define FOLD_FIRE(REC)                                                                      \
  _Pragma("unroll") for (int j = 0; j < 8; ++j) {                                             \
    if (((REC).ok >> j) & 1u) {                                                               \
      const uint32_t id = (REC).id(j);                                                        \
      if ((REC).vals[j].x != 0.0f) unsafeAtomicAdd(&ax[id], (double)(REC).vals[j].x);         \
      if ((REC).vals[j].y != 0.0f) unsafeAtomicAdd(&ay[id], (double)(REC).vals[j].y);         \
    }                                                                                         \
  }
  FoldRecs cur, nxt;
  fold_load(ip, vp, begin + mine, end, cur);
  {
    float4* z = reinterpret_cast<float4*>(s_mem);
    for (uint32_t t = tid; t < slots; t += FOLD_THREADS) z[t] = make_float4(0.f, 0.f, 0.f, 0.f);
  }
  __syncthreads();
  if (bk.trace && threadIdx.x == 0) bk.trace[16 * blk + 1] = wall_clock64();
  for (uint32_t blk = begin + wave * 512; blk < end; blk += FOLD_THREADS * 8) {
    nxt.ok = 0;
    if (blk + FOLD_THREADS * 8 < end) fold_load(ip, vp, blk + FOLD_THREADS * 8 + 2 * lane, end, nxt);
    FOLD_FIRE(cur)
    cur = nxt;
  }
#undef FOLD_FIRE
  __syncthreads();
  if (bk.trace && threadIdx.x == 0) bk.trace[16 * blk + 2] = wall_clock64();
  float2* dst = g.grad + (size_t)l * g.tsize + ((size_t)sl << bk.slice_log2);
  for (uint32_t t0 = 0; t0 < slots; t0 += FOLD_THREADS * 8) {
    float2 v[8], cv[8];
    bool nz[8];
#pragma unroll
    for (int u = 0; u < 8; ++u) {
      const uint32_t t = t0 + u * FOLD_THREADS + tid;
      nz[u] = false;
      if (t < slots) {
        v[u] = make_float2((float)ax[t], (float)ay[t]);
        nz[u] = v[u].x != 0.0f || v[u].y != 0.0f;
        if (nz[u] && !split) cv[u] = store ? make_float2(0.f, 0.f) : dst[t];
      }
    }
#pragma unroll
    for (int u = 0; u < 8; ++u) {
      const uint32_t t = t0 + u * FOLD_THREADS + tid;
      if (!nz[u]) continue;
      if (!split) {
        const float2 r = make_float2(cv[u].x + v[u].x, cv[u].y + v[u].y);
        dst[t] = r;
        if (g.nonfinite != nullptr && ((r.x - r.x) + (r.y - r.y)) != 0.0f) *g.nonfinite = 1.0f;
      } else {
        if (v[u].x != 0.0f) unsafeAtomicAdd(reinterpret_cast<float*>(dst + t), v[u].x);
        if (v[u].y != 0.0f) unsafeAtomicAdd(reinterpret_cast<float*>(dst + t) + 1, v[u].y);
        if (g.nonfinite != nullptr && ((v[u].x - v[u].x) + (v[u].y - v[u].y)) != 0.0f) *g.nonfinite = 1.0f;
      }
    }
  }
  if (bk.trace) {
    __syncthreads();
    if (threadIdx.x == 0) bk.trace[16 * blk + 3] = wall_clock64();
  }
}

struct SegK {
  uint16_t* idx;
  float2* val;
  uint32_t* hdr;
  uint32_t NB;
  int slice_log2, nslices;
  uint32_t merge_mask;
  uint32_t segc;
  uint32_t chunks;
};
#define SEG_CAP (BIN_THREADS * 8)
#define SEG_REGION (SEG_CAP + TN_BIN_MAX_SLICES)
#ifndef SEG_FOLD_ABLATE
#define SEG_FOLD_ABLATE 0
#endif

template <bool WANT_DPOS>
__global__ void __launch_bounds__(BIN_THREADS, 4) k_seg_bin(GridK g, const float* __restrict__ origins, const float* __restrict__ directions,
                                                         const float* __restrict__ e_bins, const float* __restrict__ g_enc, int ld, int64_t N, int S,
                                                         float* __restrict__ d_origins, float* __restrict__ d_directions, int level_groups, SegK sk,
                                                         DposArgs cw, int cw_blocks) {
  __shared__ uint32_t s_cnt[TN_BIN_MAX_SLICES];
  __shared__ uint32_t s_off[TN_BIN_MAX_SLICES + 1];
  __shared__ __attribute__((aligned(16))) uint16_t s_i16[SEG_REGION];
  __shared__ __attribute__((aligned(16))) float2 s_val[SEG_REGION];
  const unsigned bx = blockIdx.x;
  if (!WANT_DPOS && bx >= sk.NB) {
    field_dpos_body(cw, blockIdx.y * (unsigned)cw_blocks + (bx - sk.NB), (unsigned)cw_blocks * gridDim.y, reinterpret_cast<float*>(s_val),
                    reinterpret_cast<int*>(s_cnt));
    return;
  }
  const int lane = tn_lane();
  const int tid = threadIdx.x, wv = tid >> 6;
  const int ns = sk.nslices;
  const int64_t P = N * (int64_t)S;
  int64_t i = (int64_t)bx * BIN_THREADS + tid;
  const bool live = i < P;
  if (!live) i = P - 1;
  int64_t ray;
  int s;
  tn_patch_order(i, N, S, ray, s);
  const int64_t p = ray * S + s;
  const float* o = origins + ray * 3;
  const float* d = directions + ray * 3;
  const float* eb = e_bins + ray * (S + 1) + s;
  const float st = eb[0], en = eb[1];
  const Contracted c = tn_contract(o[0], o[1], o[2], d[0], d[1], d[2], st, en);
  const int nlev = (g.L - (int)blockIdx.y + level_groups - 1) / level_groups;
  constexpr int GVP = WANT_DPOS ? 0 : 5;
  float2 gvp[GVP + 1];
#pragma unroll
  for (int li = 0; li < GVP; ++li) {
    const int l = blockIdx.y + li * level_groups;
    gvp[li] = (live && li < nlev) ? *reinterpret_cast<const float2*>(ld > 0 ? g_enc + p * ld + 2 * l : g_enc + (int64_t)l * 2 * P + 2 * p) : make_float2(0.f, 0.f);
  }
  for (int t = tid; t < ns; t += BIN_THREADS) s_cnt[t] = 0;
  __syncthreads();
  const uint32_t smask = (1u << sk.slice_log2) - 1u;
  float dpx = 0.f, dpy = 0.f, dpz = 0.f;
#pragma unroll 1
  for (int li = 0; li < nlev; ++li) {
    const int l = blockIdx.y + li * level_groups;
    const float res = g.res[l];
    const bool merge = (sk.merge_mask >> l) & 1u;
    BinLevel b;
    bin_level(c, res, g.mask, merge, live, lane, b);
    if (b.emit) {
#pragma unroll
      for (int k = 0; k < 8; ++k) b.idx[k] |= atomicAdd(&s_cnt[b.idx[k] >> sk.slice_log2], 1u) << 20;
    }
    __syncthreads();
    if (wv == (li & (BIN_THREADS / 64 - 1))) {
      uint32_t run = 0;
      uint32_t* hdr = sk.hdr + ((size_t)l * ns) * sk.NB + bx;
      for (int base = 0; base < ns; base += 64) {
        const int sl = base + lane;
        const uint32_t cnt = sl < ns ? s_cnt[sl] : 0u;
        const uint32_t ce = (cnt + 1u) & ~1u;
        uint32_t inc = ce;
#pragma unroll
        for (int o2 = 1; o2 < 64; o2 <<= 1) {
          const uint32_t t = __shfl_up(inc, o2, 64);
          if (lane >= o2) inc += t;
        }
        if (sl < ns) {
          const uint32_t off = run + inc - ce;
          s_off[sl] = off;
          s_cnt[sl] = 0u;
          hdr[(size_t)sl * sk.NB] = off | (cnt << 16);
        }
        run += __shfl(inc, 63, 64);
      }
      if (lane == 0) s_off[ns] = run;
    }
    float2 gv = make_float2(0.f, 0.f);
    if (li < GVP) {
#pragma unroll
      for (int q = 0; q < GVP; ++q)
        if (q == li) gv = gvp[q];
    } else if (live) {
      gv = *reinterpret_cast<const float2*>(ld > 0 ? g_enc + p * ld + 2 * l : g_enc + (int64_t)l * 2 * P + 2 * p);
    }
    if (WANT_DPOS) {
      const float2* tb = g.table + (size_t)l * g.tsize;
      float sk8[8];
#pragma unroll
      for (int k = 0; k < 8; ++k) {
        const float2 t = tb[b.idx[k] & 0xfffffu];
        sk8[k] = gv.x * t.x + gv.y * t.y;
      }
      float ax = 0.f, ay = 0.f, az = 0.f;
#pragma unroll
      for (int v = 0; v < 2; ++v)
#pragma unroll
        for (int u = 0; u < 2; ++u) {
          ax += b.wy[u] * b.wz[v] * (sk8[1 + 2 * u + 4 * v] - sk8[0 + 2 * u + 4 * v]);
          ay += b.wx[u] * b.wz[v] * (sk8[u + 2 + 4 * v] - sk8[u + 0 + 4 * v]);
          az += b.wx[u] * b.wy[v] * (sk8[u + 2 * v + 4] - sk8[u + 2 * v + 0]);
        }
      dpx += ax * res;
      dpy += ay * res;
      dpz += az * res;
    }
    float vx[8], vy[8];
#pragma unroll
    for (int k = 0; k < 8; ++k) {
      const float w = b.wx[k & 1] * b.wy[(k >> 1) & 1] * b.wz[k >> 2];
      vx[k] = w * gv.x;
      vy[k] = w * gv.y;
    }
    if (merge && b.maxlen > 1) bin_run_sums(vx, vy, lane, b);
    __syncthreads();
    if (b.emit) {
#pragma unroll
      for (int k = 0; k < 8; ++k) {
        const uint32_t pos = s_off[(b.idx[k] & 0xfffffu) >> sk.slice_log2] + (b.idx[k] >> 20);
        s_i16[pos] = (uint16_t)(b.idx[k] & smask);
        s_val[pos] = make_float2(vx[k], vy[k]);
      }
    }
    __syncthreads();
    const uint32_t total = s_off[ns];
    const size_t reg = ((size_t)l * sk.NB + bx) * SEG_REGION;
    {
      float4* __restrict__ dv = reinterpret_cast<float4*>(sk.val + reg);
      const float4* sv = reinterpret_cast<const float4*>(s_val);
      for (uint32_t j = tid; j < (total + 1) / 2; j += BIN_THREADS) dv[j] = sv[j];
      uint4* __restrict__ di = reinterpret_cast<uint4*>(sk.idx + reg);
      const uint4* si = reinterpret_cast<const uint4*>(s_i16);
      for (uint32_t j = tid; j < (total + 7) / 8; j += BIN_THREADS) di[j] = si[j];
    }
  }
  if (WANT_DPOS) {
    float wxg, wyg, wzg;
    tn_contract_bwd(c, dpx, dpy, dpz, wxg, wyg, wzg);
    if (!live) { wxg = wyg = wzg = 0.0f; }
    const float tm = (st + en) / 2.0f;
    float v[6] = {wxg, wyg, wzg, wxg * tm, wyg * tm, wzg * tm};
    const int r32 = (int)ray;
    const int lead = __shfl(r32, lane & 3, 64);
    if (__all(r32 == lead)) {
#pragma unroll
      for (int k = 0; k < 6; ++k) {
        float r = v[k];
        r += __shfl_xor(r, 4, 64);
        r += __shfl_xor(r, 8, 64);
        r += __shfl_xor(r, 16, 64);
        r += __shfl_xor(r, 32, 64);
        if (lane < 4 && r != 0.0f) atomicAdd((k < 3 ? d_origins : d_directions) + ray * 3 + (k % 3), r);
      }
    } else {
#pragma unroll
      for (int k = 0; k < 6; ++k)
        if (v[k] != 0.0f) atomicAdd((k < 3 ? d_origins : d_directions) + ray * 3 + (k % 3), v[k]);
    }
  }
}

__global__ void __launch_bounds__(FOLD_THREADS, 8) k_seg_fold(GridK g, SegK sk, uint32_t level_begin, uint32_t grad_zero_promise, PoseFinishArgs pf,
                                                           uint32_t pf_blocks) {
  extern __shared__ __attribute__((aligned(16))) float s_mem[];
  if (blockIdx.x < pf_blocks) {
    if ((int)blockIdx.x < pf.total_blocks) pose_finish_body(pf, (int)blockIdx.x);
    return;
  }
  const uint32_t fb = blockIdx.x - pf_blocks;
  const int tid = threadIdx.x, lane = tid & 63, wave = tid >> 6;
  const uint32_t ns = (uint32_t)sk.nslices, per_level = ns * sk.chunks;
  const uint32_t l = level_begin + fb / per_level, rel = fb % per_level;
  const uint32_t ch = rel / ns, p = rel % ns;
  const uint32_t sl = (ns % 32u == 0u) ? ((p >> 5) << 5) + ((p & 7u) << 2) + ((p >> 3) & 3u) : p;
  const uint32_t slots = 1u << sk.slice_log2;
  double* ax = reinterpret_cast<double*>(s_mem);
  double* ay = ax + slots;
  uint32_t* s_h = reinterpret_cast<uint32_t*>(s_mem + 4 * slots);
  uint32_t* s_pre = s_h + sk.segc;
  uint32_t* s_tot = s_pre + sk.segc;
  const uint32_t b0 = ch * sk.segc, nseg = min(sk.segc, sk.NB - b0);
  const uint32_t my_h = (uint32_t)tid < nseg ? sk.hdr[((size_t)l * ns + sl) * sk.NB + b0 + tid] : 0u;
  {
    float4* z = reinterpret_cast<float4*>(s_mem);
    for (uint32_t t = tid; t < slots; t += FOLD_THREADS) z[t] = make_float4(0.f, 0.f, 0.f, 0.f);
  }
  {
    const uint32_t c = ((my_h >> 16) + 1u) >> 1;
    uint32_t inc = c;
#pragma unroll
    for (int o = 1; o < 64; o <<= 1) {
      const uint32_t up = __shfl_up(inc, o, 64);
      if (lane >= o) inc += up;
    }
    if ((uint32_t)tid < nseg) { s_h[tid] = my_h; s_pre[tid] = inc - c; }
    if (lane == 63) s_tot[wave] = inc;
  }
  __syncthreads();
  uint32_t total = 0;
#pragma unroll
  for (int w = 0; w < FOLD_THREADS / 64; ++w) total += s_tot[w];
  if (total == 0) return;
  const bool split = sk.chunks > 1;
  const bool store = grad_zero_promise && !split;
  const uint32_t avg = 2u * total / nseg;
  const int gw_log2 = avg >= 256 ? 6 : (avg >= 96 ? 5 : 4);
  const uint32_t gw = 1u << gw_log2, ngroups = FOLD_THREADS >> gw_log2;
  const uint32_t share = (((total + ngroups - 1) / ngroups) + gw - 1) & ~(gw - 1);
  const uint32_t r_begin = ((uint32_t)tid >> gw_log2) * share, r_end = min(total, r_begin + share);
  uint32_t rr = r_begin + ((uint32_t)tid & (gw - 1));
  const size_t lvl_base = (size_t)l * sk.NB + b0;
  uint32_t sg = 0, t = 0, cnt = 0, cnt_rec = 0;
  size_t base = 0;
  auto open_seg = [&]() {
    const uint32_t h = s_h[sg];
    cnt_rec = h >> 16;
    cnt = (cnt_rec + 1u) >> 1;
    base = (lvl_base + sg) * SEG_REGION + (h & 0xffffu);
  };
  if (r_begin < total) {
    uint32_t before = 0, w = 0;
#pragma unroll
    for (int i = 0; i < FOLD_THREADS / 64; ++i) {
      const uint32_t c = s_tot[i];
      if (i == (int)w && r_begin >= before + c) { before += c; ++w; }
    }
    const uint32_t want = r_begin - before;
    uint32_t lo = w * 64, hi = min(nseg, lo + 64);
    while (hi - lo > 1) {
      const uint32_t mid = (lo + hi) >> 1;
      if (s_pre[mid] <= want) lo = mid; else hi = mid;
    }
    sg = lo;
    open_seg();
    t = want - s_pre[sg] + ((uint32_t)tid & (gw - 1));
  }
  struct FoldRec { uint32_t idp; float4 v; bool ok; };
  auto fetch = [&](FoldRec& r) {
    r.ok = rr < r_end;
    r.idp = 0;
    r.v = make_float4(0.f, 0.f, 0.f, 0.f);
    if (r.ok) {
      while (t >= cnt) {
        t -= cnt;
        ++sg;
        open_seg();
      }
#if SEG_FOLD_ABLATE & 2
      r.idp = ((uint32_t)(base + 2 * t) & (slots - 1)) * 0x10001u;
      r.v = make_float4(1.0f, 1.0f, 1.0f, 1.0f);
#else
      r.idp = *reinterpret_cast<const uint32_t*>(sk.idx + base + 2 * (size_t)t);
      r.v = *reinterpret_cast<const float4*>(sk.val + base + 2 * (size_t)t);
#endif
      if (2u * t + 1u >= cnt_rec) { r.idp &= 0xffffu; r.v.z = 0.0f; r.v.w = 0.0f; }
    }
    t += gw;
    rr += gw;
  };
#ifndef SEG_FOLD_D
#define SEG_FOLD_D 4
#endif
  constexpr int FOLD_D = SEG_FOLD_D;
  FoldRec q[FOLD_D];
#pragma unroll
  for (int d = 0; d < FOLD_D; ++d) fetch(q[d]);
  while (__any(q[0].ok)) {
#pragma unroll
    for (int d = 0; d < FOLD_D; ++d) {
      const FoldRec c = q[d];
      fetch(q[d]);
#if SEG_FOLD_ABLATE & 1
      if (c.ok && c.v.x == 123.456f && c.idp == 77u) ax[c.idp & 0xffffu] = (double)c.v.y;
#else
      if (c.ok && ((c.v.x != 0.0f) | (c.v.y != 0.0f) | (c.v.z != 0.0f) | (c.v.w != 0.0f))) {
        const uint32_t i0 = c.idp & 0xffffu, i1 = c.idp >> 16;
        unsafeAtomicAdd(&ax[i0], (double)c.v.x);
        unsafeAtomicAdd(&ay[i0], (double)c.v.y);
        unsafeAtomicAdd(&ax[i1], (double)c.v.z);
        unsafeAtomicAdd(&ay[i1], (double)c.v.w);
      }
#endif
    }
  }
  __syncthreads();
#if SEG_FOLD_ABLATE & 4
  if (total != 0xffffffffu) return;
#endif
  float2* dst = g.grad + (size_t)l * g.tsize + ((size_t)sl << sk.slice_log2);
  for (uint32_t tt = 0; tt < slots; tt += FOLD_THREADS * 8) {
    float2 w[8], cv[8];
    bool nz[8];
#pragma unroll
    for (int u = 0; u < 8; ++u) {
      const uint32_t t = tt + u * FOLD_THREADS + tid;
      nz[u] = false;
      if (t < slots) {
        w[u] = make_float2((float)ax[t], (float)ay[t]);
        nz[u] = w[u].x != 0.0f || w[u].y != 0.0f;
        if (nz[u] && !split) cv[u] = store ? make_float2(0.f, 0.f) : dst[t];
      }
    }
#pragma unroll
    for (int u = 0; u < 8; ++u) {
      const uint32_t t = tt + u * FOLD_THREADS + tid;
      if (!nz[u]) continue;
      if (!split) {
        const float2 r = make_float2(cv[u].x + w[u].x, cv[u].y + w[u].y);
        dst[t] = r;
        if (g.nonfinite != nullptr && ((r.x - r.x) + (r.y - r.y)) != 0.0f) *g.nonfinite = 1.0f;
      } else {
        if (w[u].x != 0.0f) unsafeAtomicAdd(reinterpret_cast<float*>(dst + t), w[u].x);
        if (w[u].y != 0.0f) unsafeAtomicAdd(reinterpret_cast<float*>(dst + t) + 1, w[u].y);
        if (g.nonfinite != nullptr && ((w[u].x - w[u].x) + (w[u].y - w[u].y)) != 0.0f) *g.nonfinite = 1.0f;
      }
    }
  }
}

static int env_int(const char* name, int dflt, int lo, int hi) {
  const char* e = getenv(name);
  int v = e ? atoi(e) : dflt;
  return v < lo ? lo : (v > hi ? hi : v);
}
static int dense_replicas() { static int r = env_int("TN_SCATTER_REPLICAS", 16, 0, 64); return r; }

static int64_t plan_replicas(const TnGrid& grid, int64_t P, ReplicaK& rk) {
  const int64_t cap = TN_SCATTER_SCRATCH_BYTES / (int64_t)sizeof(float2);
  const int64_t T = 1ll << grid.log2_hashmap_size;
  int64_t used = 0, total = 0;
  if (dense_replicas() <= 0) return 0;
  for (int l = 0; l < grid.num_levels; ++l) {
    float r = grid.res[l];
    int64_t n = 0;
    int kind = TN_REP_NONE, R = 0;
    if (r >= 1.0f && r <= 62.0f) {
      int64_t r1 = (int64_t)ceilf(r) + 1;
      n = r1 * r1 * r1;
      R = dense_replicas();
      if (n <= T && n <= 4 * P && used + n * R <= cap) kind = TN_REP_DENSE;
    }
    if (kind == TN_REP_NONE) break;
    rk.kinds |= (uint32_t)kind << (2 * l);
    rk.n[l] = (uint32_t)n;
    rk.off[l] = (uint32_t)used;
    rk.first[l] = (uint32_t)total;
    rk.R[l] = (uint8_t)R;
    used += n * R;
    total += n;
  }
  rk.total = (uint32_t)total;
  return used;
}

static int scatter_mode() { return env_int("TN_SCATTER_MODE", 2, 0, 2); }
static bool seg_mode() { return scatter_mode() == 2; }
static int merge_res();

static int seg_plan(const TnGrid& grid, int64_t P, void* scratch, SegK& sk) {
  const int L = grid.num_levels;
  sk = SegK{};
  sk.slice_log2 = std::min(TN_BIN_SLICE_LOG2, grid.log2_hashmap_size);
  sk.nslices = 1 << (grid.log2_hashmap_size - sk.slice_log2);
  TN_REQUIRE(sk.nslices <= TN_BIN_MAX_SLICES, "tn_grid_scatter: table too large for the segmented path");
  const int64_t NB = tn_cdiv(P, BIN_THREADS);
  sk.NB = (uint32_t)NB;
  const int64_t recs = (int64_t)L * NB * SEG_REGION;
  char* base = reinterpret_cast<char*>(scratch) + 256;
  sk.val = reinterpret_cast<float2*>(base);
  sk.idx = reinterpret_cast<uint16_t*>(base + recs * 8);
  sk.hdr = reinterpret_cast<uint32_t*>(base + recs * 10);
  TN_REQUIRE(256 + recs * 10 + (int64_t)L * sk.nslices * NB * 4 <= tn_scatter_scratch_bytes(P, L), "tn_grid_scatter: segmented layout exceeds the scatter scratch");
  for (int l = 0; l < L; ++l)
    if (grid.res[l] <= (float)merge_res()) sk.merge_mask |= 1u << l;
  int64_t segc = (int64_t)L * sk.nslices >= 1024 ? 1024 : std::max<int64_t>(64, std::min<int64_t>(1024, 8 * sk.nslices));
  segc = std::min<int64_t>(segc, NB);
  segc = tn_cdiv(NB, tn_cdiv(NB, segc));
  sk.segc = (uint32_t)segc;
  sk.chunks = (uint32_t)tn_cdiv(NB, segc);
  return TN_OK;
}
static int fold_chunk_sparse() { static int r = env_int("TN_SCATTER_SPARSE_CHUNK", 16384, 1024, 32768) & ~1023; return r; }
static int merge_res() { static int r = env_int("TN_SCATTER_MERGE_RES", 1 << 20, 0, 1 << 20); return r; }

static int bin_plan(const TnGrid& grid, int64_t P, void* scratch, BinK& bk, uint32_t& nblk) {
  const int L = grid.num_levels;
  bk = BinK{};
  bk.slice_log2 = std::min(TN_BIN_SLICE_LOG2, grid.log2_hashmap_size);
  bk.nslices = 1 << (grid.log2_hashmap_size - bk.slice_log2);
  TN_REQUIRE(bk.nslices <= TN_BIN_MAX_SLICES, "tn_grid_scatter: table too large for the binned path");
  const int64_t cap = (tn_bin_level_records(P) / bk.nslices) & ~7ll;
  TN_REQUIRE(cap * bk.nslices < (1ll << 32), "tn_grid_scatter: batch too large for the binned path");
  bk.cap = (uint32_t)cap;
  bk.level_stride = (uint32_t)(cap * bk.nslices);
  char* base = reinterpret_cast<char*>(scratch);
  bk.count = reinterpret_cast<uint32_t*>(base);
  bk.cstride = 1;
  const int64_t cnt_bytes = 256 + (int64_t)L * TN_BIN_MAX_SLICES * 4 * TN_BIN_COUNT_STRIDE;
  bk.val = reinterpret_cast<float2*>(base + cnt_bytes);
  bk.idx = reinterpret_cast<uint16_t*>(base + cnt_bytes + (int64_t)L * tn_bin_level_records(P) * 8);
  nblk = 0;
  for (int l = 0; l < L; ++l) {
    if (grid.res[l] <= (float)merge_res()) bk.merge_mask |= 1u << l;
    const double r1 = ceil((double)grid.res[l]) + 1.0;
    const double T = (double)(1ll << grid.log2_hashmap_size), live = std::min(r1 * r1 * r1, T);
    const bool sparse = r1 * r1 * r1 < 0.5 * T || 8.0 * (double)P > 16.0 * live;
    bk.chunk[l] = sparse ? (uint32_t)fold_chunk_sparse() : 32768u;
    bk.blk0[l] = nblk;
    nblk += (uint32_t)(bk.nslices * tn_cdiv(bk.cap, bk.chunk[l]));
  }
  bk.blk0[L] = nblk;
  return TN_OK;
}

void tn_grid_scatter_counters(const TnGrid& grid, int64_t P, void* scratch, uint32_t** ptr, int* words) {
  *ptr = nullptr;
  *words = 0;
  if (P <= 0 || !tn_grid_scatter_is_binned(grid, P, scratch)) return;
  if (seg_mode()) return;
  BinK bk;
  uint32_t nblk;
  if (bin_plan(grid, P, scratch, bk, nblk) != TN_OK) return;
  *ptr = bk.count;
  *words = grid.num_levels * bk.nslices * (int)bk.cstride;
}

int tn_grid_scatter_bin(const TnGrid& grid, const float* origins, const float* directions, const float* e_bins, const float* g_enc, int ld, int64_t N,
                        int S, float* d_origins, float* d_directions, void* scratch, hipStream_t stream, bool counters_zeroed, const DposArgs* cowork) {
  const int64_t P = N * (int64_t)S;
  const int L = grid.num_levels;
  if (seg_mode()) {
    SegK sk;
    int rc = seg_plan(grid, P, scratch, sk);
    if (rc) return rc;
    GridK gk = make_gridk(grid);
    const int blocks = (int)sk.NB;
    int level_groups = 1;
    while (level_groups < L && (int64_t)blocks * level_groups < 256 * 6) level_groups *= 2;
    level_groups = std::min(level_groups, L);
    TN_REQUIRE(cowork == nullptr || d_origins == nullptr, "tn_grid_scatter: co-work only beside a bin pass without a d position path of its own");
    if (d_origins != nullptr) {
      hipLaunchKernelGGL(k_seg_bin<true>, dim3(blocks, level_groups), dim3(BIN_THREADS), 0, stream, gk, origins, directions, e_bins, g_enc, ld, N, S, d_origins,
                         d_directions, level_groups, sk, DposArgs{}, 0);
    } else {
      int cw_blocks = 0;
      if (cowork != nullptr) {
        const int64_t tiles = tn_cdiv(cowork->N * (int64_t)cowork->S, 32);
        cw_blocks = (int)std::min<int64_t>(tn_cdiv(tn_cdiv(tiles, BIN_THREADS / 64), level_groups), 2048);
      }
      hipLaunchKernelGGL(k_seg_bin<false>, dim3(blocks + cw_blocks, level_groups), dim3(BIN_THREADS), 0, stream, gk, origins, directions, e_bins, g_enc, ld, N, S,
                         d_origins, d_directions, level_groups, sk, cowork ? *cowork : DposArgs{}, cw_blocks);
    }
    TN_CHECK_LAUNCH("tn_grid_scatter(bin, segmented)");
    return TN_OK;
  }
  TN_REQUIRE(cowork == nullptr, "tn_grid_scatter: co-work needs the segmented path (tn_grid_scatter_takes_cowork)");
  BinK bk;
  uint32_t nblk;
  int rc = bin_plan(grid, P, scratch, bk, nblk);
  if (rc) return rc;
  if (!counters_zeroed) {
    hipError_t e = hipMemsetAsync(bk.count, 0, (size_t)L * bk.nslices * 4 * bk.cstride, stream);
    TN_REQUIRE(e == hipSuccess, "tn_grid_scatter: memset failed: %s", hipGetErrorString(e));
  }
  GridK gk = make_gridk(grid);
  const int blocks = (int)tn_cdiv(P, BIN_THREADS);
  int level_groups = 1;
  while (level_groups < L && ((int64_t)blocks * level_groups < 256 * 6 || tn_cdiv(L, level_groups) * bk.nslices > BIN_MAX_COUNTERS)) level_groups *= 2;
  level_groups = std::min(level_groups, L);
  {
    static const int forced = env_int("TN_BIN_LEVEL_GROUPS", 0, 0, TN_MAX_LEVELS);
    if (forced > 0 && tn_cdiv(L, std::min(forced, L)) * bk.nslices <= BIN_MAX_COUNTERS) level_groups = std::min(forced, L);
  }
  if (d_origins != nullptr)
    hipLaunchKernelGGL(k_grid_bin<true>, dim3(blocks, level_groups), dim3(BIN_THREADS), 0, stream, gk, origins, directions, e_bins, g_enc, ld, N, S,
                       d_origins, d_directions, level_groups, bk);
  else
    hipLaunchKernelGGL(k_grid_bin<false>, dim3(blocks, level_groups), dim3(BIN_THREADS), 0, stream, gk, origins, directions, e_bins, g_enc, ld, N, S,
                       d_origins, d_directions, level_groups, bk);
  TN_CHECK_LAUNCH("tn_grid_scatter(bin)");
  return TN_OK;
}

int tn_grid_scatter_fold(const TnGrid& grid, int64_t P, void* scratch, int level_begin, int level_end, hipStream_t stream, const PoseFinishArgs* cowork) {
  const int L = grid.num_levels;
  TN_REQUIRE(level_begin >= 0 && level_begin < level_end && level_end <= L, "tn_grid_scatter_fold: bad level range");
  TN_REQUIRE(cowork == nullptr || seg_mode(), "tn_grid_scatter_fold: co-work needs the segmented path (tn_grid_scatter_takes_cowork)");
  if (seg_mode()) {
    SegK sk;
    int rc = seg_plan(grid, P, scratch, sk);
    if (rc) return rc;
    GridK gk = make_gridk(grid);
    const size_t shmem = (size_t)(2u << sk.slice_log2) * sizeof(double) + (size_t)sk.segc * 8 + (FOLD_THREADS / 64) * 4;
    (void)hipFuncSetAttribute(reinterpret_cast<const void*>(&k_seg_fold), hipFuncAttributeMaxDynamicSharedMemorySize,
                              (int)((2u << TN_BIN_SLICE_LOG2) * sizeof(double) + 1024 * 8 + (FOLD_THREADS / 64) * 4));
    const uint32_t nblk = (uint32_t)(level_end - level_begin) * (uint32_t)sk.nslices * sk.chunks;
    const uint32_t pfb = cowork ? ((uint32_t)cowork->total_blocks + 7u) & ~7u : 0u;
    hipLaunchKernelGGL(k_seg_fold, dim3(nblk + pfb), dim3(FOLD_THREADS), shmem, stream, gk, sk, (uint32_t)level_begin, (uint32_t)(gk.grad_zero ? 1 : 0),
                       cowork ? *cowork : PoseFinishArgs{}, pfb);
    TN_CHECK_LAUNCH("tn_grid_scatter(fold, segmented)");
    return TN_OK;
  }
  BinK bk;
  uint32_t nblk_all;
  int rc = bin_plan(grid, P, scratch, bk, nblk_all);
  if (rc) return rc;
  GridK gk = make_gridk(grid);
  const uint32_t first_block = bk.blk0[level_begin], nblk = bk.blk0[level_end] - bk.blk0[level_begin];
  const size_t shmem = (size_t)(2u << bk.slice_log2) * sizeof(double);
  (void)hipFuncSetAttribute(reinterpret_cast<const void*>(&k_grid_fold), hipFuncAttributeMaxDynamicSharedMemorySize,
                            (int)((2u << TN_BIN_SLICE_LOG2) * sizeof(double)));
  static int trace_on = env_int("TN_FOLD_TRACE", 0, 0, 1);
  static unsigned long long* trace_buf = nullptr;
  if (trace_on) {
    if (!trace_buf) (void)hipMalloc(&trace_buf, (size_t)1 << 22);
    (void)hipMemsetAsync(trace_buf, 0, (size_t)nblk_all * 128, stream);
    bk.trace = trace_buf;
  }
  hipLaunchKernelGGL(k_grid_fold, dim3(nblk), dim3(FOLD_THREADS), shmem, stream, gk, bk, first_block);
  if (trace_on) {
    std::vector<unsigned long long> h((size_t)nblk_all * 16);
    (void)hipStreamSynchronize(stream);
    (void)hipMemcpy(h.data(), trace_buf, h.size() * 8, hipMemcpyDeviceToHost);
    unsigned long long t0 = ~0ull, t1 = 0;
    for (uint32_t b = 0; b < nblk_all; ++b)
      if (h[16 * b]) { t0 = std::min(t0, h[16 * b]); t1 = std::max(t1, h[16 * b + 3]); }
    fprintf(stderr, "[fold trace] %u blocks, span %.1f us (wall clock 100 MHz)\n", nblk, (t1 - t0) / 100.0);
    if (const char* dump = getenv("TN_FOLD_TRACE_FILE")) {
      if (FILE* f = fopen(dump, "wb")) { fwrite(h.data(), 8, h.size(), f); fclose(f); }
    }
    for (int l = 0; l < L; ++l) {
      double a = 0, b2 = 0, c = 0, first = 1e30, last = 0; int n = 0;
      double st[9] = {0};
      for (uint32_t b = bk.blk0[l]; b < bk.blk0[l + 1]; ++b) {
        const unsigned long long* q = &h[16 * b];
        if (!q[0]) continue;
        ++n; a += (q[1] - q[0]) / 100.0; b2 += (q[2] - q[1]) / 100.0; c += (q[3] - q[2]) / 100.0;
        first = std::min(first, (q[0] - t0) / 100.0); last = std::max(last, (q[3] - t0) / 100.0);
        unsigned long long prev = q[1];
        for (int k = 0; k < 9; ++k) { if (q[4 + k]) { st[k] += (q[4 + k] - prev) / 100.0; prev = q[4 + k]; } }
      }
      if (n) fprintf(stderr, "  level %2d: %4d active blocks, mean us: setup %.1f passes %.1f flush %.1f; first start %.1f last end %.1f | 1st iteration: passes %.2f %.2f %.2f %.2f retries %.2f %.2f %.2f sync %.2f float-atomics %.2f\n", l, n, a / n, b2 / n, c / n, first, last,
                     st[0] / n, st[1] / n, st[2] / n, st[3] / n, st[4] / n, st[5] / n, st[6] / n, st[7] / n, st[8] / n);
    }
  }
  TN_CHECK_LAUNCH("tn_grid_scatter(fold)");
  return TN_OK;
}

bool tn_grid_scatter_is_binned(const TnGrid& grid, int64_t P, const void* scratch) {
  return scratch != nullptr && scatter_mode() >= 1 && grid.log2_hashmap_size - TN_BIN_SLICE_LOG2 <= 8 && P * 8 < (1ll << 31);
}

bool tn_grid_scatter_takes_cowork(const TnGrid& grid, int64_t P, void* scratch) { return seg_mode() && tn_grid_scatter_is_binned(grid, P, scratch); }

static int grid_scatter_binned(const TnGrid& grid, const float* origins, const float* directions, const float* e_bins, const float* g_enc, int ld,
                               int64_t N, int S, float* d_origins, float* d_directions, void* scratch, hipStream_t stream, bool counters_zeroed,
                               const DposArgs* cowork, const PoseFinishArgs* fold_cowork) {
  int rc = tn_grid_scatter_bin(grid, origins, directions, e_bins, g_enc, ld, N, S, d_origins, d_directions, scratch, stream, counters_zeroed, cowork);
  if (rc) return rc;
  return tn_grid_scatter_fold(grid, N * (int64_t)S, scratch, 0, grid.num_levels, stream, fold_cowork);
}

int tn_grid_scatter_launch(const TnGrid& grid, const float* origins, const float* directions, const float* e_bins, const float* g_enc, int ld,
                           int64_t N, int S, float* d_origins, float* d_directions, void* scratch, hipStream_t stream, float* dense_sum,
                           bool counters_zeroed, const DposArgs* cowork, const PoseFinishArgs* fold_cowork) {
  TN_REQUIRE(grid.table && grid.table_grad && origins && directions && e_bins && g_enc, "tn_grid_scatter: null pointer");
  TN_REQUIRE(grid.num_levels >= 1 && grid.num_levels <= TN_MAX_LEVELS && (ld >= 2 * grid.num_levels || ld == TN_LD_LEVEL_MAJOR),
             "tn_grid_scatter: bad level count / row stride");
  int64_t P = N * (int64_t)S;
  if (P == 0) return TN_OK;
  if (dense_sum == nullptr && tn_grid_scatter_is_binned(grid, P, scratch))
    return grid_scatter_binned(grid, origins, directions, e_bins, g_enc, ld, N, S, d_origins, d_directions, scratch, stream, counters_zeroed, cowork, fold_cowork);
  TN_REQUIRE(cowork == nullptr && fold_cowork == nullptr, "tn_grid_scatter: co-work needs the segmented path (tn_grid_scatter_takes_cowork)");
  int grid_dim = (int)std::min<int64_t>(tn_cdiv(P, 64), 256 * 32);
  int level_groups = 1;
  if (grid.num_levels >= 8) {
    double rounds = (double)grid_dim / 2048.0;
    if (rounds < 4.0 && (rounds - floor(rounds)) > 0.0 && (rounds - floor(rounds)) < 0.75) level_groups = 2;
  }
  ReplicaK rk{};
  int64_t used = 0;
  if (scratch != nullptr) {
    used = plan_replicas(grid, P, rk);
    rk.rep = reinterpret_cast<float2*>(scratch);
    if (rk.kinds) {
      hipError_t e = hipMemsetAsync(scratch, 0, (size_t)used * sizeof(float2), stream);
      TN_REQUIRE(e == hipSuccess, "tn_grid_scatter: memset failed: %s", hipGetErrorString(e));
    }
  }
  if (dense_sum != nullptr) {
    bool all_dense = scratch != nullptr;
    for (int l = 0; l < grid.num_levels; ++l) all_dense = all_dense && (((rk.kinds >> (2 * l)) & 3u) == TN_REP_DENSE);
    TN_REQUIRE(all_dense, "tn_grid_scatter: dense_sum wanted but not every level of the range is accumulated densely");
  }
  GridK gk = make_gridk(grid);
  hipLaunchKernelGGL(k_grid_scatter, dim3(grid_dim, level_groups), dim3(256), 0, stream, gk, origins, directions, e_bins, g_enc, ld, N, S, d_origins,
                     d_directions, level_groups, rk);
  TN_CHECK_LAUNCH("tn_grid_scatter");
  if (rk.kinds) {
    hipLaunchKernelGGL(k_replica_reduce, dim3((unsigned)tn_cdiv(rk.total, 256)), dim3(256), 0, stream, gk, rk, reinterpret_cast<float2*>(dense_sum));
    TN_CHECK_LAUNCH("tn_grid_scatter(reduce)");
  }
  return TN_OK;
}

int64_t tn_grid_dense_count(const TnGrid& grid, int64_t P) {
  if (P <= 0 || grid.num_levels < 1 || grid.num_levels > TN_MAX_LEVELS) return 0;
  ReplicaK rk{};
  (void)plan_replicas(grid, P, rk);
  for (int l = 0; l < grid.num_levels; ++l)
    if (((rk.kinds >> (2 * l)) & 3u) != TN_REP_DENSE) return 0;
  return (int64_t)rk.total;
}

__global__ void __launch_bounds__(256) k_dense_fold(GridK g, ReplicaK rk, const float2* __restrict__ dense_sum) {
  uint32_t e = blockIdx.x * blockDim.x + threadIdx.x;
  if (e >= rk.total) return;
  float2 v = dense_sum[e];
  if (v.x == 0.0f && v.y == 0.0f) return;
  int l = 0;
#pragma unroll 1
  for (int i = 0; i < g.L; ++i)
    if (rk.first[i] <= e) l = i;
  const uint32_t t = e - rk.first[l];
  const uint32_t r1 = (uint32_t)(int)ceilf(g.res[l]) + 1u;
  uint32_t x = t % r1, y = (t / r1) % r1, z = t / (r1 * r1);
  uint32_t idx = ((x ^ (y * TN_PRIME_Y) ^ (z * TN_PRIME_Z)) & g.mask) + (uint32_t)l * g.tsize;
  float* dst = reinterpret_cast<float*>(g.grad + idx);
  if (v.x != 0.0f) unsafeAtomicAdd(dst, v.x);
  if (v.y != 0.0f) unsafeAtomicAdd(dst + 1, v.y);
  if (g.nonfinite != nullptr && ((v.x - v.x) + (v.y - v.y)) != 0.0f) *g.nonfinite = 1.0f;
}
int tn_grid_dense_fold(const TnGrid& grid, int64_t P, const float* dense_sum, hipStream_t stream) {
  TN_REQUIRE(grid.table_grad && dense_sum, "tn_grid_dense_fold: null pointer");
  ReplicaK rk{};
  (void)plan_replicas(grid, P, rk);
  for (int l = 0; l < grid.num_levels; ++l)
    TN_REQUIRE(((rk.kinds >> (2 * l)) & 3u) == TN_REP_DENSE, "tn_grid_dense_fold: level %d of the range is not accumulated densely", l);
  hipLaunchKernelGGL(k_dense_fold, dim3((unsigned)tn_cdiv(rk.total, 256)), dim3(256), 0, stream, make_gridk(grid), rk, reinterpret_cast<const float2*>(dense_sum));
  TN_CHECK_LAUNCH("tn_grid_dense_fold");
  return TN_OK;
}

extern "C" int64_t tn_hash_scatter_workspace_bytes(int64_t num_points, int32_t num_levels) {
  if (num_points < 0 || num_levels < 1 || num_levels > TN_MAX_LEVELS) return TN_EINVAL;
  return tn_scatter_scratch_bytes(num_points, num_levels);
}

extern "C" int tn_hash_scatter(const TnGrid* grid, const float* origins, const float* directions, const float* e_bins, const float* g_enc, int32_t ld,
                               int64_t N, int32_t S, float* d_origins, float* d_directions, void* workspace, int64_t workspace_bytes, tn_stream_t stream) {
  if (N == 0) return TN_OK;
  TN_REQUIRE(grid != nullptr, "tn_hash_scatter: null grid");
  TN_REQUIRE(((uintptr_t)workspace % 256) == 0, "tn_hash_scatter: workspace must be 256-byte aligned");
  TN_REQUIRE((d_origins == nullptr) == (d_directions == nullptr), "tn_hash_scatter: d_origins and d_directions must both be given or both NULL");
  TN_REQUIRE(N >= 0 && S >= 1 && S <= TN_MAX_SAMPLES, "tn_hash_scatter: bad N=%lld S=%d", (long long)N, S);
  TN_REQUIRE(grid->log2_hashmap_size >= 1 && grid->log2_hashmap_size <= 24, "tn_hash_scatter: bad log2_hashmap_size");
// ... 7 lines not shown
```

Measured before the change: 5.980 million rays/s.

## Fuse Adam step for the hash table into the segmented scatter fold

Adds a path where the segmented grid-scatter fold kernel applies the Adam update directly to the hash-table parameters as it folds gradients. A prepare kernel checks the other gradient ranges for inf/nan first, and a state word records whether the fused step happened. The later range-based Adam kernel then skips that range when the word says fused. This avoids a separate pass that re-reads the large table gradient and Adam moments, at the cost of an extra small prepare launch and more complex fallback logic.

```diff
diff --git a/nerfstudio-thermal_amd/csrc/tn_adam.h b/nerfstudio-thermal_amd/csrc/tn_adam.h
--- /dev/null
+++ b/nerfstudio-thermal_amd/csrc/tn_adam.h
@@ -0,0 +1,60 @@
+#pragma once
+#include "tn_common.h"
+
+struct AdamCoef {
+  float neg_step, bc2_sqrt;
+  float b1, b2, omb1, omb2, eps;
+};
+__host__ __device__ __forceinline__ AdamCoef adam_coef(float neg_step, float bc2_sqrt, double beta1, double beta2, float eps) {
+  return AdamCoef{neg_step, bc2_sqrt, (float)beta1, (float)beta2, (float)(1.0 - beta1), (float)(1.0 - beta2), eps};
+}
+__device__ __forceinline__ void adam1(float& p, float g, float& m, float& v, const AdamCoef& c) {
+  const float m_new = m * c.b1 + g * c.omb1;
+  const float v_new = v * c.b2 + (c.omb2 * g) * g;
+  const float den = sqrtf(v_new) / c.bc2_sqrt + c.eps;
+  p = p + c.neg_step * (m_new / den);
+  m = m_new;
+  v = v_new;
+}
+#pragma clang fp contract(off)
+__device__ __forceinline__ double adam_bias_correction(double beta, int step, int skipped) {
+  const int eff = step - skipped;
+  return 1.0 - pow(beta, (double)(eff < 1 ? 1 : eff));
+}
+__device__ __forceinline__ double adam_sched_t(int max_steps, int sched_step, int lag) {
+  const double t = (double)(sched_step - lag) / (double)max_steps;
+  return t < 0.0 ? 0.0 : (t > 1.0 ? 1.0 : t);
+}
+__device__ __forceinline__ double adam_log_lr_term(double lr, double weight) { return log(lr) * weight; }
+__device__ __forceinline__ void adam_scalars_finish(double bc1, double bc2, double lr, float& neg_step, float& bc2_sqrt) {
+  neg_step = (float)(-(lr / bc1));
+  bc2_sqrt = (float)sqrt(bc2);
+}
+__device__ __forceinline__ void adam_step_scalars(int step, int skipped, double lr, double lr_final, int max_steps, int sched_step, int lag, double beta1,
+                                                  double beta2, float& neg_step, float& bc2_sqrt) {
+  const double bc1 = adam_bias_correction(beta1, step, skipped), bc2 = adam_bias_correction(beta2, step, skipped);
+  if (max_steps > 0) {
+    const double t = adam_sched_t(max_steps, sched_step, lag);
+    lr = exp(adam_log_lr_term(lr, 1.0 - t) + adam_log_lr_term(lr_final, t));
+  }
+  adam_scalars_finish(bc1, bc2, lr, neg_step, bc2_sqrt);
+}
+
+#define TN_FOLD_ADAM_STATE_SLOT 12
+#define TN_FOLD_ADAM_NONE 0.0f
+#define TN_FOLD_ADAM_FUSED 1.0f
+#define TN_FOLD_ADAM_FELL_BACK 2.0f
+struct FoldAdamHost {
+  float *p, *m, *v;
+  float* state;
+  float* found_inf;
+  int flag;
+  const int32_t* skipped;
+  int lag_index;
+  int step, max_steps, sched_step;
+  double lr, lr_final, beta1, beta2;
+  float eps;
+  const float* grads;
+  int ncheck;
+  int64_t check_off[TN_TRAIN_STEP_MAX_RANGES], check_cnt[TN_TRAIN_STEP_MAX_RANGES];
+};
diff --git a/nerfstudio-thermal_amd/csrc/tn_common.h b/nerfstudio-thermal_amd/csrc/tn_common.h
--- a/nerfstudio-thermal_amd/csrc/tn_common.h
+++ b/nerfstudio-thermal_amd/csrc/tn_common.h
@@ -367,7 +367,8 @@
                                       float* found_inf, const int32_t* flag_index, int32_t num_flags, int32_t* skipped, int32_t lag_index,
                                       int32_t count_skip, int32_t zero_grads, float* scale, int32_t* growth_tracker, uint32_t* done_counter,
                                       double growth_factor, double backoff_factor, int32_t growth_interval, const TnSampleRays* next, bool* next_taken,
-                                      tn_stream_t stream, const TnNextSamplingHost* chain = nullptr, bool su_update = true);
+                                      tn_stream_t stream, const TnNextSamplingHost* chain = nullptr, bool su_update = true,
+                                      const float* cond_word = nullptr, int cond_range = -1);
 static inline bool tn_next_sampling_supported(int S0, int S1, int S2) { return S0 > 128 && S0 <= 256 && S1 > 64 && S1 <= 128 && S2 >= 1 && S2 <= 256; }
 int tn_render_fwd_ex(const float* e_bins, const float* density, const float* rgb, int64_t N, int32_t S, int32_t C, int32_t training, float* weights,
                      float* comp, float* accumulation, float* depth_median, float* depth_expected, float* scratch, bool launch_clip, int* clip_nblk,
@@ -380,14 +381,17 @@
                          tn_stream_t stream);
 struct DposArgs;
 struct PoseFinishArgs;
+struct FoldAdamHost;
 int tn_grid_scatter_launch(const TnGrid& grid, const float* origins, const float* directions, const float* e_bins, const float* g_enc, int ld,
                            int64_t N, int S, float* d_origins, float* d_directions, void* scratch, hipStream_t stream, float* dense_sum = nullptr,
-                           bool counters_zeroed = false, const DposArgs* cowork = nullptr, const PoseFinishArgs* fold_cowork = nullptr);
+                           bool counters_zeroed = false, const DposArgs* cowork = nullptr, const PoseFinishArgs* fold_cowork = nullptr,
+                           const FoldAdamHost* fold_adam = nullptr);
 bool tn_grid_scatter_takes_cowork(const TnGrid& grid, int64_t P, void* scratch);
+bool tn_fold_adam_takes(const TnGrid& grid, int64_t P, void* scratch);
 int tn_field_bwd_phase_ex(const TnField* field, const float* origins, const float* directions, const int64_t* camera_indices, const float* e_bins,
                           const float* d_density, const float* d_rgb, int64_t N, int32_t S, void* workspace, int64_t workspace_bytes, float* d_origins,
                           float* d_directions, int32_t phases, int32_t level_begin, int32_t level_end, const PoseFinishArgs* fold_cowork,
-                          bool* fold_cowork_taken, tn_stream_t stream);
+                          bool* fold_cowork_taken, tn_stream_t stream, const FoldAdamHost* fold_adam = nullptr);
 int tn_pose_finish_args(const float* pose_adjustment, const uint8_t* frozen, const int64_t* camera_indices, const float* directions_in,
                         const float* d_origins, const float* d_directions, int64_t N, int32_t num_cameras, float* grad_pose, const float* loss_lines,
                         float* losses16, float trans_pen, float rot_pen, float scale, float* reg_out, const float* grads, int32_t num_ranges,
@@ -401,8 +405,8 @@
 bool tn_grid_scatter_is_binned(const TnGrid& grid, int64_t P, const void* scratch);
 int tn_grid_scatter_bin(const TnGrid& grid, const float* origins, const float* directions, const float* e_bins, const float* g_enc, int ld, int64_t N,
                         int S, float* d_origins, float* d_directions, void* scratch, hipStream_t stream, bool counters_zeroed = false,
-                        const DposArgs* cowork = nullptr);
+                        const DposArgs* cowork = nullptr, const FoldAdamHost* fold_adam = nullptr);
 int tn_grid_scatter_fold(const TnGrid& grid, int64_t P, void* scratch, int level_begin, int level_end, hipStream_t stream,
-                         const PoseFinishArgs* cowork = nullptr);
+                         const PoseFinishArgs* cowork = nullptr, const FoldAdamHost* fold_adam = nullptr);
 int64_t tn_grid_dense_count(const TnGrid& grid, int64_t P);
 int tn_grid_dense_fold(const TnGrid& grid, int64_t P, const float* dense_sum, hipStream_t stream);
diff --git a/nerfstudio-thermal_amd/csrc/tn_field.hip b/nerfstudio-thermal_amd/csrc/tn_field.hip
--- a/nerfstudio-thermal_amd/csrc/tn_field.hip
+++ b/nerfstudio-thermal_amd/csrc/tn_field.hip
@@ -1268,7 +1268,7 @@
 int tn_field_bwd_phase_ex(const TnField* field, const float* origins, const float* directions, const int64_t* camera_indices, const float* e_bins,
                           const float* d_density, const float* d_rgb, int64_t N, int32_t S, void* workspace, int64_t workspace_bytes, float* d_origins,
                           float* d_directions, int32_t phases, int32_t level_begin, int32_t level_end, const PoseFinishArgs* fold_cowork,
-                          bool* fold_cowork_taken, tn_stream_t stream) {
+                          bool* fold_cowork_taken, tn_stream_t stream, const FoldAdamHost* fold_adam) {
   if (fold_cowork_taken) *fold_cowork_taken = false;
   if (N == 0) return TN_OK;
   int rc = check_field(field, "tn_field_bwd", true);
@@ -1340,8 +1340,9 @@
     TnGrid sub = level_range_grid(field->grid, level_begin, level_end);
     const bool cz = (phases & (TN_BWD_MLP | TN_BWD_COUNTERS_CLEAN)) && level_begin == 0 && level_end == field->grid.num_levels;
     const PoseFinishArgs* fcw = (fold_cowork != nullptr && dpos_cowork) ? fold_cowork : nullptr;
+    const FoldAdamHost* fad = (fold_adam != nullptr && dpos_cowork) ? fold_adam : nullptr;
     rc = tn_grid_scatter_launch(sub, origins, directions, e_bins, ws.g_enc + (int64_t)level_begin * 2 * P, TN_LD_LEVEL_MAJOR, N, S, sc_do, sc_dd, ws.scatter, st,
-                                nullptr, cz, dpos_cowork ? &dpos_args : nullptr, fcw);
+                                nullptr, cz, dpos_cowork ? &dpos_args : nullptr, fcw, fad);
     if (fold_cowork_taken && rc == TN_OK) *fold_cowork_taken = fcw != nullptr;
   }
   if (phases & (TN_BWD_SCATTER_BIN | TN_BWD_SCATTER_FOLD)) {
diff --git a/nerfstudio-thermal_amd/csrc/tn_misc.hip b/nerfstudio-thermal_amd/csrc/tn_misc.hip
--- a/nerfstudio-thermal_amd/csrc/tn_misc.hip
+++ b/nerfstudio-thermal_amd/csrc/tn_misc.hip
@@ -844,6 +844,8 @@
   int32_t max_steps[TN_ADAM_MAX_RANGES];
   int32_t sched_step;
   int32_t num_flags, lag_index;
+  const float* cond_word;
+  int32_t cond_range;
 };
 struct ScalerUpdate {
   float* scale;
@@ -894,6 +896,7 @@
 }
 struct SampleCoWork { SamplePixelsArgs a; RaygenArgs g; int blocks; };
 #include "tn_next_sampling.h"
+#include "tn_adam.h"
 __device__ __forceinline__ void adam_range_body(float* __restrict__ p, const float* __restrict__ g, float* __restrict__ m, float* __restrict__ v,
                                                 const AdamRangesAmp& r, double beta1, double beta2, float eps, const float* __restrict__ inv_scale,
                                                 float* __restrict__ found_inf, int32_t* __restrict__ skipped, int count_skip, int zero_g, int k, int bid,
@@ -903,51 +906,37 @@
   const int lag = (skipped != nullptr && r.lag_index >= 0) ? skipped[r.lag_index] : 0;
   const int64_t off = r.off[k], n = r.cnt[k], n4 = n / 4;
   const int64_t stride = (int64_t)nblk * blockDim.x;
+  const bool stepped_by_fold = r.cond_word != nullptr && k == r.cond_range && *r.cond_word == TN_FOLD_ADAM_FUSED;
   if (found_inf != nullptr && found_inf[fl] != 0.0f) {
     if (count_skip && skipped != nullptr && bid == 0 && threadIdx.x == 0) {
       bool first = true;
       for (int j = 0; j < k; ++j) first = first && r.flag[j] != fl;
       if (first) atomicAdd(&skipped[fl], 1);
     }
-    if (zero_g) {
+    if (zero_g && !stepped_by_fold) {
       for (int64_t i = bid * (int64_t)blockDim.x + threadIdx.x; i < n4; i += stride)
         reinterpret_cast<float4*>(gz + off)[i] = make_float4(0.f, 0.f, 0.f, 0.f);
       if (bid == 0 && (int64_t)threadIdx.x < n - n4 * 4) gz[off + n4 * 4 + threadIdx.x] = 0.0f;
     }
     return;
   }
+  if (stepped_by_fold) return;
   if ((int64_t)bid * blockDim.x >= n4 && bid != 0) return;
   __shared__ float s_ns, s_bc;
   __syncthreads();
-  if (threadIdx.x == 0) {
-    const int sk = skipped ? skipped[fl] : 0;
-    const int eff = r.step[k] - sk;
-    const double bc1 = 1.0 - pow(beta1, (double)(eff < 1 ? 1 : eff)), bc2 = 1.0 - pow(beta2, (double)(eff < 1 ? 1 : eff));
-    double lr = r.lr[k];
-    if (r.max_steps[k] > 0) {
-      double t = (double)(r.sched_step - lag) / (double)r.max_steps[k];
-      t = t < 0.0 ? 0.0 : (t > 1.0 ? 1.0 : t);
-      lr = exp(log(r.lr[k]) * (1.0 - t) + log(r.lr_final[k]) * t);
-    }
-    s_ns = (float)(-(lr / bc1));
-    s_bc = (float)sqrt(bc2);
-  }
+  if (threadIdx.x == 0) adam_step_scalars(r.step[k], skipped ? skipped[fl] : 0, r.lr[k], r.lr_final[k], r.max_steps[k], r.sched_step, lag, beta1, beta2, s_ns, s_bc);
   __syncthreads();
-  const float neg_step = s_ns, bc2_sqrt = s_bc, b1 = (float)beta1, b2 = (float)beta2, omb1 = (float)(1.0 - beta1), omb2 = (float)(1.0 - beta2);
+  const AdamCoef coef = adam_coef(s_ns, s_bc, beta1, beta2, eps);
   const float is = inv_scale ? *inv_scale : 1.0f;
   float4* p4 = reinterpret_cast<float4*>(p + off);
   const float4* g4 = reinterpret_cast<const float4*>(g + off);
   float4* m4 = reinterpret_cast<float4*>(m + off);
   float4* v4 = reinterpret_cast<float4*>(v + off);
-#define ADAM1(P, G, M, V)                         \
-  {                                               \
-    float g_ = inv_scale ? (G) * is : (G);        \
-    float m_new_ = M * b1 + g_ * omb1;            \
-    float v_new_ = V * b2 + (omb2 * g_) * g_;     \
-    float den_ = sqrtf(v_new_) / bc2_sqrt + eps;  \
-    P = P + neg_step * (m_new_ / den_);           \
-    M = m_new_;                                   \
-    V = v_new_;                                   \
+#define ADAM1(P, G, M, V)                               \
+  {                                                     \
+    float p_ = P, m_ = M, v_ = V;                       \
+    adam1(p_, inv_scale ? (G) * is : (G), m_, v_, coef); \
+    P = p_; M = m_; V = v_;                             \
   }
   typedef float v4f __attribute__((ext_vector_type(4)));
   typedef uint32_t v4u __attribute__((ext_vector_type(4)));
@@ -1023,7 +1012,8 @@
                                const int32_t* sched_max_steps, int32_t sched_step, double beta1, double beta2, double eps,
                                const float* inv_scale, const float* found_inf, const int32_t* flag_index, int32_t num_flags, int32_t* skipped,
                                int32_t lag_index, int32_t count_skip, int32_t zero_grads, ScalerUpdate su, tn_stream_t stream,
-                               const TnSampleRays* next = nullptr, bool* next_taken = nullptr, const TnNextSamplingHost* chain = nullptr) {
+                               const TnSampleRays* next = nullptr, bool* next_taken = nullptr, const TnNextSamplingHost* chain = nullptr,
+                               const float* cond_word = nullptr, int cond_range = -1) {
   if (next_taken) *next_taken = false;
   if (num_ranges == 0) return TN_OK;
   TN_REQUIRE(params && grads && exp_avg && exp_avg_sq && offsets && counts && steps && lrs, "tn_adam_step_ranges_amp: null pointer");
@@ -1040,6 +1030,7 @@
     const int fl = flag_index ? flag_index[k] : 0;
     TN_REQUIRE(fl >= 0 && fl < num_flags, "tn_adam_step_ranges_amp: flag index %d of range %d outside [0, %d)", fl, k, num_flags);
     if (counts[k] == 0) continue;
+    if (cond_word != nullptr && k == cond_range) { r.cond_word = cond_word; r.cond_range = n; }
     r.off[n] = offsets[k]; r.cnt[n] = counts[k]; r.step[n] = steps[k]; r.lr[n] = lrs[k]; r.flag[n] = fl;
     r.lr_final[n] = lr_finals ? lr_finals[k] : lrs[k];
     r.max_steps[n] = (lr_finals && sched_max_steps) ? sched_max_steps[k] : 0;
@@ -1118,7 +1109,7 @@
       return TN_OK;
     }
     FusedAdam fa{};
-    if (mode && mode[0] == '4' && n == 1 && inv_scale == nullptr) {
+    if (mode && mode[0] == '4' && n == 1 && inv_scale == nullptr && r.cond_word == nullptr) {
       const int64_t nb = r.cnt[0] / 256, W = (int64_t)ns.blocks * 4, trips = tn_cdiv(chain->N, W);
       const char* fs = getenv("TN_FUSED_SITES");
       const int64_t per_ray = fs ? std::max(1, atoi(fs)) : FA_SITES_PER_RAY;
@@ -1175,13 +1166,13 @@
                                       float* found_inf, const int32_t* flag_index, int32_t num_flags, int32_t* skipped, int32_t lag_index,
                                       int32_t count_skip, int32_t zero_grads, float* scale, int32_t* growth_tracker, uint32_t* done_counter,
                                       double growth_factor, double backoff_factor, int32_t growth_interval, const TnSampleRays* next, bool* next_taken,
-                                      tn_stream_t stream, const TnNextSamplingHost* chain, bool su_update) {
+                                      tn_stream_t stream, const TnNextSamplingHost* chain, bool su_update, const float* cond_word, int cond_range) {
   TN_REQUIRE(found_inf && scale && growth_tracker && done_counter && growth_interval >= 1, "tn_adam_step_ranges_amp_update: bad scaler arguments");
   TN_REQUIRE(num_ranges > 0, "tn_adam_step_ranges_amp_update: the fused scale update needs at least one range (use tn_grad_scaler_update otherwise)");
   ScalerUpdate su{scale, growth_tracker, done_counter, (float)growth_factor, (float)backoff_factor, (int32_t)growth_interval};
   return adam_ranges_amp_impl(params, grads, exp_avg, exp_avg_sq, num_ranges, offsets, counts, steps, lrs, lr_finals, sched_max_steps, sched_step, beta1, beta2,
                               eps, inv_scale, found_inf, flag_index, num_flags, skipped, lag_index, count_skip, zero_grads, su_update ? su : ScalerUpdate{}, stream,
-                              next, next_taken, chain);
+                              next, next_taken, chain, cond_word, cond_range);
 }
 
 __global__ void k_grad_scaler_update(float* scale, int32_t* growth_tracker, float* found_inf, int num_flags, int32_t* lag, float growth_factor,
diff --git a/nerfstudio-thermal_amd/csrc/tn_pipeline.hip b/nerfstudio-thermal_amd/csrc/tn_pipeline.hip
--- a/nerfstudio-thermal_amd/csrc/tn_pipeline.hip
+++ b/nerfstudio-thermal_amd/csrc/tn_pipeline.hip
@@ -1,5 +1,6 @@
 #include "tn_common.h"
 #include "tn_pose_finish.h"
+#include "tn_adam.h"
 
 namespace {
 struct EvalWs {
@@ -176,7 +177,8 @@
                                       const float* d_weights1, const float* d_weights2, const float* d_density_extra, void* field_workspace,
                                       int64_t field_workspace_bytes, void* prop_workspace0, int64_t prop_workspace_bytes0, void* prop_workspace1,
                                       int64_t prop_workspace_bytes1, float* tmp, float* d_origins, float* d_directions, int32_t prop_enc_saved,
-                                      bool render_bwd_done, const PoseFinishArgs* fold_cowork, bool* fold_cowork_taken, tn_stream_t stream) {
+                                      bool render_bwd_done, const PoseFinishArgs* fold_cowork, bool* fold_cowork_taken, tn_stream_t stream,
+                                      const FoldAdamHost* fold_adam = nullptr) {
   if (fold_cowork_taken) *fold_cowork_taken = false;
   if (N == 0) return TN_OK;
   TN_REQUIRE(field && origins && directions && camera_indices && fwd_out && d_comp && d_weights2 && field_workspace && tmp,
@@ -222,7 +224,7 @@
   }
   rc = tn_field_bwd_phase_ex(field, o, d, camera_indices, at(TRO_E2), d_dens, d_rgb, N, S2, field_workspace, field_workspace_bytes, d_origins, d_directions,
                              TN_BWD_MLP | TN_BWD_SCATTER | TN_BWD_JOIN | (prop_grad ? TN_BWD_FORK_DPOS : 0), 0, field->grid.num_levels,
-                             prop_grad ? nullptr : fold_cowork, fold_cowork_taken, stream);
+                             prop_grad ? nullptr : fold_cowork, fold_cowork_taken, stream, fold_adam);
   if (prop_grad) { tn_join_n(st, 1); tn_join_n(st, 2); }
   return rc ? rc : (rc0 ? rc0 : rc1);
 }
@@ -320,6 +322,67 @@
                                         stream))) {
     return rc;
   }
+  int nr = a->num_ranges, fa_range = -1;
+  int64_t r_off[TN_TRAIN_STEP_MAX_RANGES + 2], r_cnt[TN_TRAIN_STEP_MAX_RANGES + 2];
+  int32_t r_step[TN_TRAIN_STEP_MAX_RANGES + 2], r_ms[TN_TRAIN_STEP_MAX_RANGES + 2], r_fl[TN_TRAIN_STEP_MAX_RANGES + 2];
+  double r_lr[TN_TRAIN_STEP_MAX_RANGES + 2], r_lf[TN_TRAIN_STEP_MAX_RANGES + 2];
+  for (int k = 0; k < nr; ++k) {
+    r_off[k] = a->offsets[k]; r_cnt[k] = a->counts[k]; r_step[k] = a->steps[k]; r_ms[k] = a->sched_max_steps[k]; r_fl[k] = a->flag_index[k];
+    r_lr[k] = a->lrs[k]; r_lf[k] = a->lr_finals[k];
+  }
+  FoldAdamHost fad{};
+  static const bool fold_adam_on = [] { const char* e = getenv("TN_FOLD_ADAM"); return !(e && e[0] == '0'); }();
+  if (fold_adam_on && nr > 0 && tn_fold_adam_takes(a->field->grid, a->N * (int64_t)a->S2, a->field_workspace)) {
+    const TnGrid& g = a->field->grid;
+    const int64_t tfl = (int64_t)g.num_levels * (2ll << g.log2_hashmap_size);
+    const int64_t tlo = g.table - a->params, thi = tlo + tfl;
+    int holder = -1, touching = 0;
+    for (int k = 0; k < nr; ++k) {
+      const int64_t lo = a->offsets[k], hi = lo + a->counts[k];
+      if (lo < thi && tlo < hi) { ++touching; if (lo <= tlo && thi <= hi) holder = k; }
+    }
+    bool holds_chain_read = false;
+    if (holder >= 0) {
+      const float *lo = a->params + a->offsets[holder], *hi = lo + a->counts[holder];
+      const float* reads[] = {a->prop0->grid.table, a->prop0->w0, a->prop0->b0, a->prop0->w1, a->prop0->b1, a->prop1->grid.table, a->prop1->w0,
+                              a->prop1->b0, a->prop1->w1, a->prop1->b1, a->pose_adjustment};
+      for (const float* q : reads) holds_chain_read = holds_chain_read || (q >= lo && q < hi);
+    }
+    int pieces = 0;
+    if (holder >= 0) pieces = (a->offsets[holder] < tlo ? 1 : 0) + (thi < a->offsets[holder] + a->counts[holder] ? 1 : 0);
+    const bool ok = holder >= 0 && touching == 1 && !holds_chain_read && tlo % 4 == 0 && g.table_grad == a->grads + tlo && a->flag_index[holder] >= 0 &&
+                    a->flag_index[holder] < a->num_flags && g.nonfinite_flag == a->found_inf + a->flag_index[holder] && nr + pieces <= TN_TRAIN_STEP_MAX_RANGES &&
+                    a->steps[holder] >= 1;
+    if (ok) {
+      const int h = holder;
+      const int64_t lo = a->offsets[h], hi = lo + a->counts[h];
+      int n = 0;
+      auto put = [&](int src, int64_t o, int64_t c) {
+        r_off[n] = o; r_cnt[n] = c; r_step[n] = a->steps[src]; r_ms[n] = a->sched_max_steps[src]; r_fl[n] = a->flag_index[src];
+        r_lr[n] = a->lrs[src]; r_lf[n] = a->lr_finals[src];
+        ++n;
+      };
+      for (int k = 0; k < a->num_ranges; ++k) {
+        if (k != h) { put(k, a->offsets[k], a->counts[k]); continue; }
+        if (lo < tlo) put(k, lo, tlo - lo);
+        fa_range = n;
+        put(k, tlo, tfl);
+        if (thi < hi) put(k, thi, hi - thi);
+      }
+      nr = n;
+      fad.p = a->params + tlo; fad.m = a->exp_avg + tlo; fad.v = a->exp_avg_sq + tlo;
+      fad.state = a->losses16 + TN_FOLD_ADAM_STATE_SLOT;
+      fad.found_inf = a->found_inf; fad.flag = a->flag_index[h];
+      fad.skipped = a->skipped; fad.lag_index = a->lag_index;
+      fad.step = a->steps[h]; fad.max_steps = a->sched_max_steps[h]; fad.sched_step = a->sched_step;
+      fad.lr = a->lrs[h]; fad.lr_final = a->lr_finals[h]; fad.beta1 = a->beta1; fad.beta2 = a->beta2; fad.eps = (float)a->eps;
+      fad.grads = a->grads;
+      for (int k = 0; k < a->num_check; ++k)
+        if (a->check_flags[k] == fad.flag && a->check_counts[k] > 0) { fad.check_off[fad.ncheck] = a->check_offsets[k]; fad.check_cnt[fad.ncheck] = a->check_counts[k]; ++fad.ncheck; }
+    }
+  }
+  const FoldAdamHost* fold_adam = fa_range >= 0 ? &fad : nullptr;
+  const float* cond_word = fold_adam ? fad.state + 1 : nullptr;
   PoseFinishArgs pf;
   bool pf_taken = false;
   const char* pfe = getenv("TN_POSE_FINISH_COWORK");
@@ -335,7 +398,7 @@
                                        a->field_workspace, a->field_workspace_bytes, a->prop_grad ? a->prop_workspace0 : nullptr,
                                        a->prop_grad ? a->prop_workspace_bytes0 : 0, a->prop_grad ? a->prop_workspace1 : nullptr,
                                        a->prop_grad ? a->prop_workspace_bytes1 : 0, a->bwd_tmp, a->d_origins, a->d_directions, a->prop_grad ? 1 : 0,
-                                       fuse_render, pf_cowork ? &pf : nullptr, &pf_taken, stream)))
+                                       fuse_render, pf_cowork ? &pf : nullptr, &pf_taken, stream, fold_adam)))
     return rc;
   if (!pf_taken) {
     if ((rc = tn_pose_bwd_finish_check(a->pose_adjustment, a->frozen, a->camera_indices, a->directions_in, a->d_origins, a->d_directions, a->N,
@@ -350,38 +413,42 @@
   const char* nse = getenv("TN_NEXT_SAMPLING");
   bool chain = nx != nullptr && a->next_sample != nullptr && a->next_sample->num_rays == a->N && a->next_sample->camera_indices != nullptr && a->N % 4 == 0 &&
                tn_next_sampling_supported(a->S0, a->S1, a->S2) && !(nse && nse[0] == '0');
-  int first[TN_TRAIN_STEP_MAX_RANGES], nfirst = 0, rest[TN_TRAIN_STEP_MAX_RANGES], nrest = 0;
+  int first[TN_TRAIN_STEP_MAX_RANGES + 2], nfirst = 0, rest[TN_TRAIN_STEP_MAX_RANGES + 2], nrest = 0;
   if (chain) {
     const float* reads[] = {a->prop0->grid.table, a->prop0->w0, a->prop0->b0, a->prop0->w1, a->prop0->b1, a->prop1->grid.table, a->prop1->w0,
                             a->prop1->b0, a->prop1->w1, a->prop1->b1, a->pose_adjustment};
-    for (int k = 0; k < a->num_ranges; ++k) {
-      const float *lo = a->params + a->offsets[k], *hi = lo + a->counts[k];
+    for (int k = 0; k < nr; ++k) {
+      const float *lo = a->params + r_off[k], *hi = lo + r_cnt[k];
       bool hit = false;
       for (const float* q : reads) hit = hit || (q >= lo && q < hi);
-      if (hit) first[nfirst++] = k; else if (a->counts[k] > 0) rest[nrest++] = k;
+      if (hit) first[nfirst++] = k; else if (r_cnt[k] > 0) rest[nrest++] = k;
     }
     chain = nrest > 0 && nfirst > 0;
   }
   if (!chain) {
-    rc = tn_adam_step_ranges_amp_update_cw(a->params, a->grads, a->exp_avg, a->exp_avg_sq, a->num_ranges, a->offsets, a->counts, a->steps, a->lrs, a->lr_finals,
-                                           a->sched_max_steps, a->sched_step, a->beta1, a->beta2, a->eps, nullptr, a->found_inf, a->flag_index, a->num_flags,
-                                           a->skipped, a->lag_index, 1, 1, a->scale, a->growth_tracker, a->done_counter, a->growth_factor, a->backoff_factor,
-                                           a->growth_interval, a->next_sample, &taken, stream);
+    rc = tn_adam_step_ranges_amp_update_cw(a->params, a->grads, a->exp_avg, a->exp_avg_sq, nr, r_off, r_cnt, r_step, r_lr, r_lf, r_ms, a->sched_step, a->beta1,
+                                           a->beta2, a->eps, nullptr, a->found_inf, r_fl, a->num_flags, a->skipped, a->lag_index, 1, 1, a->scale,
+                                           a->growth_tracker, a->done_counter, a->growth_factor, a->backoff_factor, a->growth_interval, a->next_sample, &taken,
+                                           stream, nullptr, true, cond_word, fa_range);
   } else {
+    int cond_at = -1;
     auto sub = [&](const int* idx, int n, int64_t* o, int64_t* c, int32_t* s, double* l, double* lf, int32_t* ms, int32_t* fl) {
+      cond_at = -1;
       for (int i = 0; i < n; ++i) {
         const int k = idx[i];
-        o[i] = a->offsets[k]; c[i] = a->counts[k]; s[i] = a->steps[k]; l[i] = a->lrs[k]; lf[i] = a->lr_finals[k]; ms[i] = a->sched_max_steps[k]; fl[i] = a->flag_index[k];
+        o[i] = r_off[k]; c[i] = r_cnt[k]; s[i] = r_step[k]; l[i] = r_lr[k]; lf[i] = r_lf[k]; ms[i] = r_ms[k]; fl[i] = r_fl[k];
+        if (k == fa_range) cond_at = i;
       }
     };
-    int64_t o[TN_TRAIN_STEP_MAX_RANGES], c[TN_TRAIN_STEP_MAX_RANGES];
-    int32_t s[TN_TRAIN_STEP_MAX_RANGES], ms[TN_TRAIN_STEP_MAX_RANGES], fl[TN_TRAIN_STEP_MAX_RANGES];
-    double l[TN_TRAIN_STEP_MAX_RANGES], lf[TN_TRAIN_STEP_MAX_RANGES];
+    int64_t o[TN_TRAIN_STEP_MAX_RANGES + 2], c[TN_TRAIN_STEP_MAX_RANGES + 2];
+    int32_t s[TN_TRAIN_STEP_MAX_RANGES + 2], ms[TN_TRAIN_STEP_MAX_RANGES + 2], fl[TN_TRAIN_STEP_MAX_RANGES + 2];
+    double l[TN_TRAIN_STEP_MAX_RANGES + 2], lf[TN_TRAIN_STEP_MAX_RANGES + 2];
     rc = TN_OK;
     sub(first, nfirst, o, c, s, l, lf, ms, fl);
     rc = tn_adam_step_ranges_amp_update_cw(a->params, a->grads, a->exp_avg, a->exp_avg_sq, nfirst, o, c, s, l, lf, ms, a->sched_step, a->beta1, a->beta2, a->eps,
                                            nullptr, a->found_inf, fl, a->num_flags, a->skipped, a->lag_index, 1, 1, a->scale, a->growth_tracker, a->done_counter,
-                                           a->growth_factor, a->backoff_factor, a->growth_interval, a->next_sample, &taken, stream, nullptr, false);
+                                           a->growth_factor, a->backoff_factor, a->growth_interval, a->next_sample, &taken, stream, nullptr, false,
+                                           cond_at >= 0 ? cond_word : nullptr, cond_at);
     if (!rc && !taken) rc = tn_sample_rays_args(a->next_sample, stream);
     if (!rc) {
       taken = true;
@@ -399,7 +466,8 @@
       sub(rest, nrest, o, c, s, l, lf, ms, fl);
       rc = tn_adam_step_ranges_amp_update_cw(a->params, a->grads, a->exp_avg, a->exp_avg_sq, nrest, o, c, s, l, lf, ms, a->sched_step, a->beta1, a->beta2, a->eps,
                                              nullptr, a->found_inf, fl, a->num_flags, a->skipped, a->lag_index, 1, 1, a->scale, a->growth_tracker, a->done_counter,
-                                             a->growth_factor, a->backoff_factor, a->growth_interval, nullptr, nullptr, stream, &h, true);
+                                             a->growth_factor, a->backoff_factor, a->growth_interval, nullptr, nullptr, stream, &h, true,
+                                             cond_at >= 0 ? cond_word : nullptr, cond_at);
       if (!rc && a->next_sampling_taken) *a->next_sampling_taken = 1;
     }
   }
diff --git a/nerfstudio-thermal_amd/csrc/tn_scatter.hip b/nerfstudio-thermal_amd/csrc/tn_scatter.hip
--- a/nerfstudio-thermal_amd/csrc/tn_scatter.hip
+++ b/nerfstudio-thermal_amd/csrc/tn_scatter.hip
@@ -1,6 +1,8 @@
 #include "tn_common.h"
 #include "tn_field_dpos.h"
 #include "tn_pose_finish.h"
+#include "tn_adam.h"
+#include <float.h>
 #include <stdlib.h>
 #include <stdio.h>
 #include <vector>
@@ -628,7 +630,31 @@
   uint32_t merge_mask;
   uint32_t segc;
   uint32_t chunks;
+  uint32_t* wmax;
 };
+struct FoldAdamScal {
+  float* state;
+  const int32_t* skipped;
+  int flag, lag_index, step, max_steps, sched_step;
+  double lr, lr_final, beta1, beta2;
+};
+__device__ __forceinline__ void fold_adam_scalars_block(const FoldAdamScal& a, double* s_term ) {
+  if ((threadIdx.x & 63) == 0 && threadIdx.x < 256) {
+    const int w = threadIdx.x >> 6;
+    const int sk = a.skipped ? a.skipped[a.flag] : 0;
+    const int lag = (a.skipped != nullptr && a.lag_index >= 0) ? a.skipped[a.lag_index] : 0;
+    const double t = a.max_steps > 0 ? adam_sched_t(a.max_steps, a.sched_step, lag) : 0.0;
+    if (w < 2) s_term[w] = adam_bias_correction(w == 0 ? a.beta1 : a.beta2, a.step, sk);
+    else if (a.max_steps > 0) s_term[w] = adam_log_lr_term(w == 2 ? a.lr : a.lr_final, w == 2 ? 1.0 - t : t);
+  }
+  __syncthreads();
+  if (threadIdx.x == 0) {
+    float ns, bc;
+    adam_scalars_finish(s_term[0], s_term[1], a.max_steps > 0 ? exp(s_term[2] + s_term[3]) : a.lr, ns, bc);
+    a.state[2] = ns;
+    a.state[3] = bc;
+  }
+}
 #define SEG_CAP (BIN_THREADS * 8)
 #define SEG_REGION (SEG_CAP + TN_BIN_MAX_SLICES)
 #ifndef SEG_FOLD_ABLATE
@@ -639,12 +665,16 @@
 __global__ void __launch_bounds__(BIN_THREADS, 4) k_seg_bin(GridK g, const float* __restrict__ origins, const float* __restrict__ directions,
                                                          const float* __restrict__ e_bins, const float* __restrict__ g_enc, int ld, int64_t N, int S,
                                                          float* __restrict__ d_origins, float* __restrict__ d_directions, int level_groups, SegK sk,
-                                                         DposArgs cw, int cw_blocks) {
+                                                         DposArgs cw, int cw_blocks, FoldAdamScal fs) {
   __shared__ uint32_t s_cnt[TN_BIN_MAX_SLICES];
   __shared__ uint32_t s_off[TN_BIN_MAX_SLICES + 1];
   __shared__ __attribute__((aligned(16))) uint16_t s_i16[SEG_REGION];
   __shared__ __attribute__((aligned(16))) float2 s_val[SEG_REGION];
   const unsigned bx = blockIdx.x;
+  if (!WANT_DPOS && bx >= sk.NB + (unsigned)cw_blocks) {
+    if (blockIdx.y == 0) fold_adam_scalars_block(fs, reinterpret_cast<double*>(s_val));
+    return;
+  }
   if (!WANT_DPOS && bx >= sk.NB) {
     field_dpos_body(cw, blockIdx.y * (unsigned)cw_blocks + (bx - sk.NB), (unsigned)cw_blocks * gridDim.y, reinterpret_cast<float*>(s_val),
                     reinterpret_cast<int*>(s_cnt));
@@ -678,6 +708,7 @@
   __syncthreads();
   const uint32_t smask = (1u << sk.slice_log2) - 1u;
   float dpx = 0.f, dpy = 0.f, dpz = 0.f;
+  uint32_t gmax = 0u;
 #pragma unroll 1
   for (int li = 0; li < nlev; ++li) {
     const int l = blockIdx.y + li * level_groups;
@@ -721,6 +752,7 @@
     } else if (live) {
       gv = *reinterpret_cast<const float2*>(ld > 0 ? g_enc + p * ld + 2 * l : g_enc + (int64_t)l * 2 * P + 2 * p);
     }
+    if (!WANT_DPOS && fs.state != nullptr) gmax = max(gmax, max(__float_as_uint(gv.x) & 0x7fffffffu, __float_as_uint(gv.y) & 0x7fffffffu));
     if (WANT_DPOS) {
       const float2* tb = g.table + (size_t)l * g.tsize;
       float sk8[8];
@@ -771,6 +803,11 @@
       for (uint32_t j = tid; j < (total + 7) / 8; j += BIN_THREADS) di[j] = si[j];
     }
   }
+  if (!WANT_DPOS && fs.state != nullptr) {
+#pragma unroll
+    for (int o2 = 32; o2 >= 1; o2 >>= 1) gmax = max(gmax, (uint32_t)__shfl_xor((int)gmax, o2, 64));
+    if (lane == 0) sk.wmax[((size_t)blockIdx.y * sk.NB + bx) * (BIN_THREADS / 64) + wv] = gmax;
+  }
   if (WANT_DPOS) {
     float wxg, wyg, wzg;
     tn_contract_bwd(c, dpx, dpy, dpz, wxg, wyg, wzg);
@@ -797,13 +834,25 @@
   }
 }
 
+struct FoldAdamK {
+  float2 *p, *m, *v;
+  const float* state;
+  const float* found_inf;
+  float b1, b2, omb1, omb2, eps;
+};
+#ifndef FOLD_ADAM_BATCH
+#define FOLD_ADAM_BATCH 2
+#endif
+template <bool ADAM>
 __global__ void __launch_bounds__(FOLD_THREADS, 8) k_seg_fold(GridK g, SegK sk, uint32_t level_begin, uint32_t grad_zero_promise, PoseFinishArgs pf,
-                                                           uint32_t pf_blocks) {
+                                                           uint32_t pf_blocks, FoldAdamK fa) {
   extern __shared__ __attribute__((aligned(16))) float s_mem[];
   if (blockIdx.x < pf_blocks) {
     if ((int)blockIdx.x < pf.total_blocks) pose_finish_body(pf, (int)blockIdx.x);
     return;
   }
+  const bool fused = ADAM && fa.state[1] == TN_FOLD_ADAM_FUSED;
+  if (fused && *fa.found_inf != 0.0f) return;
   const uint32_t fb = blockIdx.x - pf_blocks;
   const int tid = threadIdx.x, lane = tid & 63, wave = tid >> 6;
   const uint32_t ns = (uint32_t)sk.nslices, per_level = ns * sk.chunks;
@@ -837,10 +886,10 @@
   uint32_t total = 0;
 #pragma unroll
   for (int w = 0; w < FOLD_THREADS / 64; ++w) total += s_tot[w];
-  if (total == 0) return;
+  if (total == 0 && !fused) return;
   const bool split = sk.chunks > 1;
   const bool store = grad_zero_promise && !split;
-  const uint32_t avg = 2u * total / nseg;
+  const uint32_t avg = 2u * total / max(nseg, 1u);
   const int gw_log2 = avg >= 256 ? 6 : (avg >= 96 ? 5 : 4);
   const uint32_t gw = 1u << gw_log2, ngroups = FOLD_THREADS >> gw_log2;
   const uint32_t share = (((total + ngroups - 1) / ngroups) + gw - 1) & ~(gw - 1);
@@ -924,6 +973,47 @@
 #if SEG_FOLD_ABLATE & 4
   if (total != 0xffffffffu) return;
 #endif
+  if (fused) {
+    typedef float v4f __attribute__((ext_vector_type(4)));
+    typedef uint32_t v4u __attribute__((ext_vector_type(4)));
+    const AdamCoef coef{fa.state[2], fa.state[3], fa.b1, fa.b2, fa.omb1, fa.omb2, fa.eps};
+    const size_t tb = (size_t)l * g.tsize + ((size_t)sl << sk.slice_log2);
+    float4* p4 = reinterpret_cast<float4*>(fa.p + tb);
+    v4f* m4 = reinterpret_cast<v4f*>(fa.m + tb);
+    v4f* v4 = reinterpret_cast<v4f*>(fa.v + tb);
+    const uint32_t pairs = slots >> 1;
+    for (uint32_t q0 = 0; q0 < pairs; q0 += FOLD_THREADS * FOLD_ADAM_BATCH) {
+      v4f gg[FOLD_ADAM_BATCH], mm[FOLD_ADAM_BATCH], vv[FOLD_ADAM_BATCH];
+      float4 pq[FOLD_ADAM_BATCH];
+#pragma unroll
+      for (int u = 0; u < FOLD_ADAM_BATCH; ++u) {
+        const uint32_t q = q0 + u * FOLD_THREADS + tid;
+        if (q < pairs) {
+          pq[u] = p4[q];
+          mm[u] = __builtin_nontemporal_load(m4 + q);
+          vv[u] = __builtin_nontemporal_load(v4 + q);
+          gg[u] = v4f{(float)ax[2 * q], (float)ay[2 * q], (float)ax[2 * q + 1], (float)ay[2 * q + 1]};
+        }
+      }
+#pragma unroll
+      for (int u = 0; u < FOLD_ADAM_BATCH; ++u) {
+        const uint32_t q = q0 + u * FOLD_THREADS + tid;
+        if (q >= pairs) continue;
+        const v4u zb = __builtin_bit_cast(v4u, gg[u]) | __builtin_bit_cast(v4u, mm[u]) | __builtin_bit_cast(v4u, vv[u]);
+        if ((zb.x | zb.y | zb.z | zb.w) == 0u) continue;
+        float4 pp = pq[u];
+        float m0 = mm[u].x, m1 = mm[u].y, m2 = mm[u].z, m3 = mm[u].w, v0 = vv[u].x, v1 = vv[u].y, v2 = vv[u].z, v3 = vv[u].w;
+        adam1(pp.x, gg[u].x, m0, v0, coef);
+        adam1(pp.y, gg[u].y, m1, v1, coef);
+        adam1(pp.z, gg[u].z, m2, v2, coef);
+        adam1(pp.w, gg[u].w, m3, v3, coef);
+        p4[q] = pp;
+        __builtin_nontemporal_store(v4f{m0, m1, m2, m3}, m4 + q);
+        __builtin_nontemporal_store(v4f{v0, v1, v2, v3}, v4 + q);
+      }
+    }
+    return;
+  }
   float2* dst = g.grad + (size_t)l * g.tsize + ((size_t)sl << sk.slice_log2);
   for (uint32_t tt = 0; tt < slots; tt += FOLD_THREADS * 8) {
     float2 w[8], cv[8];
@@ -952,6 +1042,59 @@
         if (g.nonfinite != nullptr && ((w[u].x - w[u].x) + (w[u].y - w[u].y)) != 0.0f) *g.nonfinite = 1.0f;
       }
     }
+  }
+}
+
+struct FoldAdamPrep {
+  const float* grads;
+  int ncheck;
+  int64_t off[TN_TRAIN_STEP_MAX_RANGES], cnt[TN_TRAIN_STEP_MAX_RANGES];
+  float* found_inf_flag;
+  float* state;
+  float limit;
+  const uint32_t* wmax;
+  uint32_t row_words, row_stride, rows;
+};
+__global__ void __launch_bounds__(1024) k_fold_adam_prepare(FoldAdamPrep a) {
+  __shared__ int s_bad;
+  __shared__ uint32_t s_max;
+  if (threadIdx.x == 0) { s_bad = 0; s_max = 0u; }
+  __syncthreads();
+  bool bad = false;
+  for (int k = 0; k < a.ncheck; ++k) {
+    const float* base = a.grads + a.off[k];
+    for (int64_t i0 = threadIdx.x; i0 < a.cnt[k]; i0 += 8 * (int64_t)blockDim.x) {
+      float x[8];
+#pragma unroll
+      for (int u = 0; u < 8; ++u) { const int64_t i = i0 + u * (int64_t)blockDim.x; x[u] = i < a.cnt[k] ? base[i] : 0.0f; }
+#pragma unroll
+      for (int u = 0; u < 8; ++u) bad = bad || ((x[u] - x[u]) != 0.0f);
+    }
+  }
+  uint32_t mx = 0u;
+  for (uint32_t r = 0; r < a.rows; ++r) {
+    const uint32_t* row = a.wmax + (size_t)r * a.row_stride;
+    for (uint32_t i0 = threadIdx.x; i0 < a.row_words; i0 += 8 * blockDim.x) {
+      uint32_t w[8];
+#pragma unroll
+      for (int u = 0; u < 8; ++u) { const uint32_t i = i0 + u * blockDim.x; w[u] = i < a.row_words ? row[i] : 0u; }
+#pragma unroll
+      for (int u = 0; u < 8; ++u) mx = max(mx, w[u]);
+    }
+  }
+#pragma unroll
+  for (int o = 32; o >= 1; o >>= 1) mx = max(mx, (uint32_t)__shfl_xor((int)mx, o, 64));
+  const bool wave_bad = __any(bad);
+  if ((threadIdx.x & 63) == 0) {
+    if (wave_bad) s_bad = 1;
+    atomicMax(&s_max, mx);
+  }
+  __syncthreads();
+  if (threadIdx.x == 0) {
+    if (s_bad) *a.found_inf_flag = 1.0f;
+    const float enc_max = __uint_as_float(s_max);
+    a.state[0] = enc_max;
+    a.state[1] = (enc_max <= a.limit) ? TN_FOLD_ADAM_FUSED : TN_FOLD_ADAM_FELL_BACK;
   }
 }
 
@@ -1007,7 +1150,9 @@
   sk.val = reinterpret_cast<float2*>(base);
   sk.idx = reinterpret_cast<uint16_t*>(base + recs * 8);
   sk.hdr = reinterpret_cast<uint32_t*>(base + recs * 10);
-  TN_REQUIRE(256 + recs * 10 + (int64_t)L * sk.nslices * NB * 4 <= tn_scatter_scratch_bytes(P, L), "tn_grid_scatter: segmented layout exceeds the scatter scratch");
+  const int64_t hdr_end = 256 + recs * 10 + (int64_t)L * sk.nslices * NB * 4, wmax_bytes = (int64_t)TN_MAX_LEVELS * NB * (BIN_THREADS / 64) * 4;
+  sk.wmax = reinterpret_cast<uint32_t*>(reinterpret_cast<char*>(scratch) + hdr_end);
+  TN_REQUIRE(hdr_end + wmax_bytes <= tn_scatter_scratch_bytes(P, L), "tn_grid_scatter: segmented layout exceeds the scatter scratch");
   for (int l = 0; l < L; ++l)
     if (grid.res[l] <= (float)merge_res()) sk.merge_mask |= 1u << l;
   int64_t segc = (int64_t)L * sk.nslices >= 1024 ? 1024 : std::max<int64_t>(64, std::min<int64_t>(1024, 8 * sk.nslices));
@@ -1016,6 +1161,11 @@
   sk.segc = (uint32_t)segc;
   sk.chunks = (uint32_t)tn_cdiv(NB, segc);
   return TN_OK;
+}
+static int seg_level_groups(int L, uint32_t NB) {
+  int level_groups = 1;
+  while (level_groups < L && (int64_t)NB * level_groups < 256 * 6) level_groups *= 2;
+  return std::min(level_groups, L);
 }
 static int fold_chunk_sparse() { static int r = env_int("TN_SCATTER_SPARSE_CHUNK", 16384, 1024, 32768) & ~1023; return r; }
 static int merge_res() { static int r = env_int("TN_SCATTER_MERGE_RES", 1 << 20, 0, 1 << 20); return r; }
@@ -1063,30 +1213,35 @@
 }
 
 int tn_grid_scatter_bin(const TnGrid& grid, const float* origins, const float* directions, const float* e_bins, const float* g_enc, int ld, int64_t N,
-                        int S, float* d_origins, float* d_directions, void* scratch, hipStream_t stream, bool counters_zeroed, const DposArgs* cowork) {
+                        int S, float* d_origins, float* d_directions, void* scratch, hipStream_t stream, bool counters_zeroed, const DposArgs* cowork,
+                        const FoldAdamHost* fold_adam) {
   const int64_t P = N * (int64_t)S;
   const int L = grid.num_levels;
+  TN_REQUIRE(fold_adam == nullptr || (d_origins == nullptr && tn_fold_adam_takes(grid, P, scratch)), "tn_grid_scatter: the fold does not step this table (tn_fold_adam_takes)");
   if (seg_mode()) {
     SegK sk;
     int rc = seg_plan(grid, P, scratch, sk);
     if (rc) return rc;
     GridK gk = make_gridk(grid);
     const int blocks = (int)sk.NB;
-    int level_groups = 1;
-    while (level_groups < L && (int64_t)blocks * level_groups < 256 * 6) level_groups *= 2;
-    level_groups = std::min(level_groups, L);
+    const int level_groups = seg_level_groups(L, sk.NB);
     TN_REQUIRE(cowork == nullptr || d_origins == nullptr, "tn_grid_scatter: co-work only beside a bin pass without a d position path of its own");
     if (d_origins != nullptr) {
       hipLaunchKernelGGL(k_seg_bin<true>, dim3(blocks, level_groups), dim3(BIN_THREADS), 0, stream, gk, origins, directions, e_bins, g_enc, ld, N, S, d_origins,
-                         d_directions, level_groups, sk, DposArgs{}, 0);
+                         d_directions, level_groups, sk, DposArgs{}, 0, FoldAdamScal{});
     } else {
       int cw_blocks = 0;
       if (cowork != nullptr) {
         const int64_t tiles = tn_cdiv(cowork->N * (int64_t)cowork->S, 32);
         cw_blocks = (int)std::min<int64_t>(tn_cdiv(tn_cdiv(tiles, BIN_THREADS / 64), level_groups), 2048);
       }
-      hipLaunchKernelGGL(k_seg_bin<false>, dim3(blocks + cw_blocks, level_groups), dim3(BIN_THREADS), 0, stream, gk, origins, directions, e_bins, g_enc, ld, N, S,
-                         d_origins, d_directions, level_groups, sk, cowork ? *cowork : DposArgs{}, cw_blocks);
+      FoldAdamScal fs{};
+      if (fold_adam != nullptr) {
+        const FoldAdamHost& h = *fold_adam;
+        fs = FoldAdamScal{h.state, h.skipped, h.flag, h.lag_index, h.step, h.max_steps, h.sched_step, h.lr, h.lr_final, h.beta1, h.beta2};
+      }
+      hipLaunchKernelGGL(k_seg_bin<false>, dim3(blocks + cw_blocks + (fold_adam ? 1 : 0), level_groups), dim3(BIN_THREADS), 0, stream, gk, origins, directions,
+                         e_bins, g_enc, ld, N, S, d_origins, d_directions, level_groups, sk, cowork ? *cowork : DposArgs{}, cw_blocks, fs);
     }
     TN_CHECK_LAUNCH("tn_grid_scatter(bin, segmented)");
     return TN_OK;
@@ -1119,22 +1274,46 @@
   return TN_OK;
 }
 
-int tn_grid_scatter_fold(const TnGrid& grid, int64_t P, void* scratch, int level_begin, int level_end, hipStream_t stream, const PoseFinishArgs* cowork) {
+int tn_grid_scatter_fold(const TnGrid& grid, int64_t P, void* scratch, int level_begin, int level_end, hipStream_t stream, const PoseFinishArgs* cowork,
+                         const FoldAdamHost* fold_adam) {
   const int L = grid.num_levels;
   TN_REQUIRE(level_begin >= 0 && level_begin < level_end && level_end <= L, "tn_grid_scatter_fold: bad level range");
   TN_REQUIRE(cowork == nullptr || seg_mode(), "tn_grid_scatter_fold: co-work needs the segmented path (tn_grid_scatter_takes_cowork)");
+  TN_REQUIRE(fold_adam == nullptr || (level_begin == 0 && level_end == L && fold_adam->p == grid.table && tn_fold_adam_takes(grid, P, scratch)),
+             "tn_grid_scatter_fold: the fold does not step this table (tn_fold_adam_takes, the whole grid in one launch)");
   if (seg_mode()) {
     SegK sk;
     int rc = seg_plan(grid, P, scratch, sk);
     if (rc) return rc;
     GridK gk = make_gridk(grid);
     const size_t shmem = (size_t)(2u << sk.slice_log2) * sizeof(double) + (size_t)sk.segc * 8 + (FOLD_THREADS / 64) * 4;
-    (void)hipFuncSetAttribute(reinterpret_cast<const void*>(&k_seg_fold), hipFuncAttributeMaxDynamicSharedMemorySize,
-                              (int)((2u << TN_BIN_SLICE_LOG2) * sizeof(double) + 1024 * 8 + (FOLD_THREADS / 64) * 4));
+    const int max_shmem = (int)((2u << TN_BIN_SLICE_LOG2) * sizeof(double) + 1024 * 8 + (FOLD_THREADS / 64) * 4);
     const uint32_t nblk = (uint32_t)(level_end - level_begin) * (uint32_t)sk.nslices * sk.chunks;
     const uint32_t pfb = cowork ? ((uint32_t)cowork->total_blocks + 7u) & ~7u : 0u;
-    hipLaunchKernelGGL(k_seg_fold, dim3(nblk + pfb), dim3(FOLD_THREADS), shmem, stream, gk, sk, (uint32_t)level_begin, (uint32_t)(gk.grad_zero ? 1 : 0),
-                       cowork ? *cowork : PoseFinishArgs{}, pfb);
+    if (fold_adam != nullptr) {
+      const FoldAdamHost& h = *fold_adam;
+      FoldAdamPrep pr{};
+      pr.grads = h.grads;
+      pr.ncheck = h.ncheck;
+      for (int k = 0; k < h.ncheck; ++k) { pr.off[k] = h.check_off[k]; pr.cnt[k] = h.check_cnt[k]; }
+      pr.found_inf_flag = h.found_inf + h.flag;
+      pr.state = h.state;
+      pr.limit = FLT_MAX / (8.0f * (float)P);
+      pr.wmax = sk.wmax;
+      pr.row_words = sk.NB * (BIN_THREADS / 64); pr.row_stride = pr.row_words; pr.rows = (uint32_t)seg_level_groups(L, sk.NB);
+      hipLaunchKernelGGL(k_fold_adam_prepare, dim3(1), dim3(1024), 0, stream, pr);
+      TN_CHECK_LAUNCH("tn_grid_scatter(fold: prepare)");
+      const AdamCoef c = adam_coef(0.f, 0.f, h.beta1, h.beta2, h.eps);
+      FoldAdamK fa{reinterpret_cast<float2*>(h.p), reinterpret_cast<float2*>(h.m), reinterpret_cast<float2*>(h.v), h.state, h.found_inf + h.flag,
+                   c.b1, c.b2, c.omb1, c.omb2, c.eps};
+      (void)hipFuncSetAttribute(reinterpret_cast<const void*>(&k_seg_fold<true>), hipFuncAttributeMaxDynamicSharedMemorySize, max_shmem);
+      hipLaunchKernelGGL(k_seg_fold<true>, dim3(nblk + pfb), dim3(FOLD_THREADS), shmem, stream, gk, sk, (uint32_t)level_begin, (uint32_t)(gk.grad_zero ? 1 : 0),
+                         cowork ? *cowork : PoseFinishArgs{}, pfb, fa);
+    } else {
+      (void)hipFuncSetAttribute(reinterpret_cast<const void*>(&k_seg_fold<false>), hipFuncAttributeMaxDynamicSharedMemorySize, max_shmem);
+      hipLaunchKernelGGL(k_seg_fold<false>, dim3(nblk + pfb), dim3(FOLD_THREADS), shmem, stream, gk, sk, (uint32_t)level_begin, (uint32_t)(gk.grad_zero ? 1 : 0),
+                         cowork ? *cowork : PoseFinishArgs{}, pfb, FoldAdamK{});
+    }
     TN_CHECK_LAUNCH("tn_grid_scatter(fold, segmented)");
     return TN_OK;
   }
@@ -1190,26 +1369,33 @@
 }
 
 bool tn_grid_scatter_takes_cowork(const TnGrid& grid, int64_t P, void* scratch) { return seg_mode() && tn_grid_scatter_is_binned(grid, P, scratch); }
+bool tn_fold_adam_takes(const TnGrid& grid, int64_t P, void* scratch) {
+  if (!tn_grid_scatter_takes_cowork(grid, P, scratch) || !grid.table_grad_is_zero || grid.log2_hashmap_size < 1) return false;
+  SegK sk;
+  if (seg_plan(grid, P, scratch, sk) != TN_OK) return false;
+  return sk.chunks == 1 && ((uintptr_t)grid.table % 16) == 0;
+}
 
 static int grid_scatter_binned(const TnGrid& grid, const float* origins, const float* directions, const float* e_bins, const float* g_enc, int ld,
                                int64_t N, int S, float* d_origins, float* d_directions, void* scratch, hipStream_t stream, bool counters_zeroed,
-                               const DposArgs* cowork, const PoseFinishArgs* fold_cowork) {
-  int rc = tn_grid_scatter_bin(grid, origins, directions, e_bins, g_enc, ld, N, S, d_origins, d_directions, scratch, stream, counters_zeroed, cowork);
+                               const DposArgs* cowork, const PoseFinishArgs* fold_cowork, const FoldAdamHost* fold_adam) {
+  int rc = tn_grid_scatter_bin(grid, origins, directions, e_bins, g_enc, ld, N, S, d_origins, d_directions, scratch, stream, counters_zeroed, cowork, fold_adam);
   if (rc) return rc;
-  return tn_grid_scatter_fold(grid, N * (int64_t)S, scratch, 0, grid.num_levels, stream, fold_cowork);
+  return tn_grid_scatter_fold(grid, N * (int64_t)S, scratch, 0, grid.num_levels, stream, fold_cowork, fold_adam);
 }
 
 int tn_grid_scatter_launch(const TnGrid& grid, const float* origins, const float* directions, const float* e_bins, const float* g_enc, int ld,
                            int64_t N, int S, float* d_origins, float* d_directions, void* scratch, hipStream_t stream, float* dense_sum,
-                           bool counters_zeroed, const DposArgs* cowork, const PoseFinishArgs* fold_cowork) {
+                           bool counters_zeroed, const DposArgs* cowork, const PoseFinishArgs* fold_cowork, const FoldAdamHost* fold_adam) {
   TN_REQUIRE(grid.table && grid.table_grad && origins && directions && e_bins && g_enc, "tn_grid_scatter: null pointer");
   TN_REQUIRE(grid.num_levels >= 1 && grid.num_levels <= TN_MAX_LEVELS && (ld >= 2 * grid.num_levels || ld == TN_LD_LEVEL_MAJOR),
              "tn_grid_scatter: bad level count / row stride");
   int64_t P = N * (int64_t)S;
   if (P == 0) return TN_OK;
   if (dense_sum == nullptr && tn_grid_scatter_is_binned(grid, P, scratch))
-    return grid_scatter_binned(grid, origins, directions, e_bins, g_enc, ld, N, S, d_origins, d_directions, scratch, stream, counters_zeroed, cowork, fold_cowork);
-  TN_REQUIRE(cowork == nullptr && fold_cowork == nullptr, "tn_grid_scatter: co-work needs the segmented path (tn_grid_scatter_takes_cowork)");
+    return grid_scatter_binned(grid, origins, directions, e_bins, g_enc, ld, N, S, d_origins, d_directions, scratch, stream, counters_zeroed, cowork, fold_cowork,
+                               fold_adam);
+  TN_REQUIRE(cowork == nullptr && fold_cowork == nullptr && fold_adam == nullptr, "tn_grid_scatter: co-work needs the segmented path (tn_grid_scatter_takes_cowork)");
   int grid_dim = (int)std::min<int64_t>(tn_cdiv(P, 64), 256 * 32);
   int level_groups = 1;
   if (grid.num_levels >= 8) {
```

Result: faster. 6.128 million rays/s, median of 6 (+2.5%).
